# dlwns147/amq

Hardware: AMD Instinct MI355X
Metric: decode tokens/s, Llama-2-7B AMQ mixed 2/3/4-bit avg-3-bit, batch 1 (higher is better)
Workload: dtype f16; 1 GPU; Llama-2-7B shapes, synthesized avg-3.0-bit per-layer arch (bits_usage 2.982), batch 1 decode after a 64-token prefill, one stream per GPU; parallelism=replicas x1, prompt=64, group_size=128

## Files before the change

amq_amd/_lib.py:

```python
import ctypes
import os

_HERE = os.path.dirname(os.path.abspath(__file__))
LIB_PATH = os.path.join(_HERE, "libamq_hip.so")
AB_LIB_PATH = os.path.join(_HERE, "libamq_hip_ab.so")

AMQ_OK = 0
MODE_HQQ, MODE_FMA, MODE_FMA1 = 0, 1, 2
PRO_NONE, PRO_RMSNORM, PRO_SILU_MUL = 0, 1, 2
MAX_SEGMENTS = 4
MATH_DEFAULT, MATH_LINEAR, MATH_GROUPSCALE, MATH_EXACT = 0, 1, 2, 3
FEWROW_AUTO, FEWROW_TILE, FEWROW_STREAM = 0, 1, 2
ABI_VERSION = 521
GEMM_AUTO, GEMM_TILED, GEMM_SKINNY, GEMM_RING, GEMM_RING128, GEMM_WS, GEMM_DEQ = 0, 1, 2, 3, 4, 5, 6

_vp, _i, _f, _sz = ctypes.c_void_p, ctypes.c_int, ctypes.c_float, ctypes.c_size_t


class Segment(ctypes.Structure):
    _fields_ = [("qweight_native", _vp), ("meta_native", _vp), ("bias", _vp), ("residual", _vp),
                ("y", _vp), ("N", _i), ("bits", _i), ("mode", _i), ("y_stride", _i)]


class EngineLinear(ctypes.Structure):
    _fields_ = [("qweight_native", _vp), ("meta_native", _vp), ("N", _i), ("bits", _i), ("mode", _i), ("reserved", _i)]


class EngineBlock(ctypes.Structure):
    _fields_ = [("lin", EngineLinear * 7), ("ln1", _vp), ("ln2", _vp), ("kcache", _vp), ("vcache", _vp)]


class GemvOpts(ctypes.Structure):
    _fields_ = [("math", _i), ("waves", _i), ("depth", _i), ("rpt", _i), ("dot", _i)]


SIGNATURES = {
    "amq_version": (_i, []),
    "amq_default_gemv_math": (_i, []),
    "amq_last_error": (ctypes.c_char_p, []),
    "amq_query": (_i, [_i, ctypes.POINTER(_i), _i]),
    "amq_native_qweight_bytes": (_sz, [_i, _i, _i]),
    "amq_fma1_scale_bound": (ctypes.c_float, [_i]),
    "amq_native_meta_bytes": (_sz, [_i, _i, _i]),
    "amq_repack_from_hqq": (_i, [_i, _vp, _vp, _vp, _i, _i, _i, _vp, _vp, _vp]),
    "amq_repack_from_gptq": (_i, [_i, _vp, _vp, _vp, _i, _i, _i, _vp, _vp, _vp]),
    "amq_repack_from_awq": (_i, [_vp, _vp, _vp, _i, _i, _i, _vp, _vp, _vp]),
    "amq_dequantize_f16": (_i, [_i, _i, _vp, _vp, _i, _i, _i, _vp, _vp]),
    "amq_dequantize_hqq_f16": (_i, [_i, _vp, _vp, _vp, _i, _i, _i, _vp, _vp]),
    "amq_dequantize_bf16": (_i, [_i, _vp, _vp, _i, _i, _i, _vp, _vp]),
    "amq_dequantize_hqq_bf16": (_i, [_i, _vp, _vp, _vp, _i, _i, _i, _vp, _vp]),
    "amq_gemv_bf16": (_i, [_i, _vp, _vp, _vp, _vp, _vp, _vp, _i, _i, _i, _i, _i, _i, _vp]),
    "amq_gemm_bf16_workspace_bytes": (_sz, [_i, _i, _i]),
    "amq_gemm_bf16": (_i, [_i, _vp, _vp, _vp, _vp, _vp, _vp, _i, _i, _i, _i, _i, _i, _vp, _sz, _vp]),
    "amq_gemv_f16": (_i, [_i, _i, _vp, _vp, _vp, _vp, _vp, _i, _i, _i, _i, _i, _i, _vp]),
    "amq_gemm_f16": (_i, [_i, _i, _vp, _vp, _vp, _vp, _vp, _i, _i, _i, _i, _i, _i, _vp]),
    "amq_linear_f16": (_i, [_i, _i, _vp, _vp, _vp, _vp, _vp, _i, _i, _i, _i, _vp]),
    "amq_gemm_splitk_workspace_bytes": (_sz, [_i, _i, _i]),
    "amq_gemm_splitk_f16": (_i, [_i, _i, _vp, _vp, _vp, _vp, _vp, _i, _i, _i, _i, _i, _i, _vp, _sz, _vp]),
    "amq_compat_workspace_bytes": (_sz, [_i, _i, _i, _i]),
    "amq_vecquantmatmul_faster_old": (_i, [_i, _vp, _vp, _vp, _vp, _vp, _i, _i, _i, _i, _i, _vp, _sz, _i, _vp]),
    "amq_gemv_4bit": (_i, [_vp, _vp, _vp, _vp, _vp, _i, _i, _i, _i, _vp, _sz, _i, _vp]),
    "amq_gemm_4bit": (_i, [_vp, _vp, _vp, _vp, _vp, _i, _i, _i, _i, _vp, _sz, _i, _vp]),
    "amq_rmsnorm_f16": (_i, [_vp, _vp, _vp, _i, _i, _f, _vp]),
    "amq_gemv_f16w": (_i, [_vp, _vp, _vp, _vp, _vp, _f, _i, _i, _vp]),
    "amq_attn_decode_f16": (_i, [_vp, _vp, _vp, _vp, _vp, _vp, _vp, _i, _i, _i, _i, _i, _i, _f, _vp, _vp]),
    "amq_rope_table_f16": (_i, [_vp, _i, _f, _vp]),
    "amq_rope_table_freqs_f16": (_i, [_vp, _i, _vp, _f, _vp]),
    "amq_decode_tail_f16": (_i, [_vp, _i, _vp, _i, _vp, _vp, _vp, _vp, _vp, _i, _vp]),
    "amq_attn_decode_cur_f16": (_i, [_vp, _vp, _vp, _vp, _vp, _vp, _vp, _i, _i, _i, _i, _i, _vp]),
    "amq_gemm_res_f16": (_i, [_i, _i, _vp, _vp, _vp, _vp, _vp, _vp, _i, _i, _i, _i, _i, _i, _vp, _sz, _vp]),
    "amq_xfrag_bytes": (_sz, [_i, _i]),
    "amq_xfrag_f16": (_i, [_vp, _vp, _i, _i, ctypes.c_longlong, ctypes.c_longlong, _vp]),
    "amq_rmsnorm_xfrag_f16": (_i, [_vp, _vp, _vp, _i, _i, _f, _vp]),
    "amq_gemm_xfrag_f16": (_i, [_i, _i, _vp, _vp, _vp, _vp, _vp, _vp, _vp, _i, _i, _i, _i, _i, _vp]),
    "amq_gemm_gated_fused": (_i, [_i, _i, _i, _i, _i]),
    "amq_gemm_gated_fused_g": (_i, [_i, _i, _i, _i, _i, _i]),
    "amq_gemm_gated_f16": (_i, [_i, _i, _i, _vp, _vp, _vp, _vp, _vp, _vp, _i, _i, _i, _i, _i, _vp, _sz, _vp]),
    "amq_attn_decode_split_workspace_bytes": (_sz, [_i, _i, _i]),
    "amq_attn_decode_split_f16": (_i, [_vp, _vp, _vp, _vp, _vp, _vp, _vp, _vp, _i, _i, _i, _i, _i, _i, _f, _vp, _i, _vp, _sz, _vp, _vp]),
    "amq_gemm_xfrag_grouped_f16": (_i, [ctypes.POINTER(Segment), _i, _vp, _i, _i, _i, _vp]),
    "amq_gemm_xfrag_grouped_form_f16": (_i, [ctypes.POINTER(Segment), _i, _vp, _i, _i, _i, _i, _i, _vp]),
    "amq_attn_prefill_xfrag_f16": (_i, [_vp, _vp, _vp, _vp, _i, _i, _i, _i, _i] + [ctypes.c_longlong] * 5 + [_vp]),
    "amq_gemv_f16w_rows": (_i, [_vp, _vp, _vp, _vp, _vp, _f, _i, _i, _i, _vp]),
    "amq_decode_tail_batch_f16": (_i, [_vp, _i, _vp, _i, _vp, _vp, _vp, _vp, _vp, _i, _i, _vp]),
    "amq_decode_tail_suppress_f16": (_i, [_vp, _i, _vp, _i, _vp, _vp, _vp, _vp, _vp, _i, _i, _vp, _vp]),
    "amq_set_token_f16": (_i, [_vp, _i, _vp, _i, _i, _vp, _vp, _vp, _vp, _vp, _i, _i, _vp]),
    "amq_attn_prefill_f16": (_i, [_vp, _vp, _vp, _vp, _i, _i, _i, _i, _i, _i] + [ctypes.c_longlong] * 10 + [_vp]),
    "amq_rope_cache_f16": (_i, [_vp, _vp, _vp, _vp, _vp, _vp, _i, _i, _i, _i, _i, _i, _i, _vp]),
    "amq_rope_cache_batch_f16": (_i, [_vp, _vp, _vp, _vp, _vp, _vp, _i, _i, _i, _i, _i, _i, _i, _i, _vp]),
    "amq_rope_rows_f16": (_i, [_vp, _vp, _vp, _i, _i, _i, _i, _i, _i, _i, _vp]),
    "amq_silu_mul_f16": (_i, [_vp, _vp, _vp, _sz, _vp]),
    "amq_gemv_grouped_f16": (_i, [ctypes.POINTER(Segment), _i, _vp, _vp, _vp, _f, _i, _i, _i, _i, _i, ctypes.POINTER(GemvOpts), _vp]),
    "amq_gemv_grouped_sums_f16": (_i, [ctypes.POINTER(Segment), _i, _vp, _vp, _f, _vp, _vp, _i, _i, _i, _vp]),
    "amq_gemm_f16w_f16": (_i, [_vp, _vp, _vp, _vp, _vp, _vp, _i, _i, _i, _i, _i, _vp]),
    "amq_gemm_route_workspace_bytes": (_sz, [_i, _i, _i, _i]),
    "amq_gemm_route_workspace_bytes_g": (_sz, [_i, _i, _i, _i, _i]),
    "amq_gemm_res_norm_xfrag_f16": (_i, [_i, _i, _vp, _vp, _vp, _vp, _vp, _vp, _i, _i, _i, _i, _i, _vp, _sz, _vp, _f, _vp, _vp]),
    "amq_gemm_route_f16": (_i, [_i, _i, _i, _vp, _vp, _vp, _vp, _vp, _vp, _i, _i, _i, _i, _i, _i, _vp, _sz, _vp]),
}

AB_SIGNATURES = {
    "amq_gemv_qkv_attn_f16": (_i, [ctypes.POINTER(Segment), _vp, _vp, _f, _i, _i, _vp, _vp, _vp, _vp, _i, _i, _i, _i, _vp, _vp]),
    "amq_decode_engine_image_bytes": (_sz, [_i]),
    "amq_decode_engine_scratch_bytes": (_sz, [_i, _i, _i]),
    "amq_decode_engine_sync_bytes": (_sz, []),
    "amq_decode_engine_image": (_i, [ctypes.POINTER(EngineBlock), _i, _i, _i, _i, _i, _i, _i, _vp]),
    "amq_decode_engine_f16": (_i, [_vp, _i, _i, _i, _i, _i, _i, _i, _f, _vp, _vp, _sz, _vp, _vp, _sz, _i, _vp]),
}

_lib = None
_ab_lib = None


class AmqError(RuntimeError):
    pass


def load():
    global _lib
    if _lib is not None:
        return _lib
    if not os.path.exists(LIB_PATH):
        raise AmqError(
            f"{LIB_PATH} not found: the HIP extension is not built. "
            "Run `python -c 'import __graft_entry__ as g; g.build()'` (or `make -C amq_amd/csrc`). "
            "There is no CPU fallback.")
    import torch
    lib = ctypes.CDLL(LIB_PATH)
    for name, (res, args) in SIGNATURES.items():
        fn = getattr(lib, name)
        fn.restype, fn.argtypes = res, args
    if lib.amq_version() != ABI_VERSION:
        raise AmqError(f"{LIB_PATH} reports ABI version {lib.amq_version()}, these bindings were written against {ABI_VERSION} "
                       "(include/amq_hip.h AMQ_VERSION): rebuild with `make -C amq_amd/csrc`")
    _lib = lib
    return lib


def load_ab():
    global _ab_lib
    if _ab_lib is not None:
        return _ab_lib
    if not os.path.exists(AB_LIB_PATH):
        raise AmqError(f"{AB_LIB_PATH} not found: the A/B routes (decode engine, fused q/k/v + attention) live in their own library -- "
                       "`make -C amq_amd/csrc ab` (or __graft_entry__.build()).  They are slower than the product step and not needed for it.")
    import torch
    lib = ctypes.CDLL(AB_LIB_PATH)
    for name, (res, args) in AB_SIGNATURES.items():
        fn = getattr(lib, name)
        fn.restype, fn.argtypes = res, args
    lib.amq_last_error.restype = ctypes.c_char_p
    _ab_lib = lib
    return lib


def check_ab(rc):
    if rc != AMQ_OK:
        raise AmqError(f"libamq_hip_ab error {rc}: {load_ab().amq_last_error().decode('utf-8', 'replace')}")


def use_library(path):
    global LIB_PATH
    global AB_LIB_PATH
    if _lib is not None or _ab_lib is not None:
        raise AmqError("use_library() must be called before the library is first loaded")
    LIB_PATH = os.path.abspath(path)
    AB_LIB_PATH = LIB_PATH


SAFE_LIB_PATH = os.path.join(_HERE, "libamq_hip_safe.so")


def open_twin(path=None):
    path = SAFE_LIB_PATH if path is None else os.path.abspath(path)
    if not os.path.exists(path):
        raise AmqError(f"{path} not found: `make -C amq_amd/csrc safe` (or __graft_entry__.build())")
    import torch
    lib = ctypes.CDLL(path)
    for name, (res, args) in SIGNATURES.items():
        fn = getattr(lib, name)
        fn.restype, fn.argtypes = res, args
    if lib.amq_version() != ABI_VERSION:
        raise AmqError(f"{path} reports ABI version {lib.amq_version()}, expected {ABI_VERSION}")
    return lib


class routed_to:

    def __init__(self, lib):
        self.lib = lib

    def __enter__(self):
        global _lib
        load()
        self.prev, _lib = _lib, self.lib
        return self.lib

    def __exit__(self, *exc):
        global _lib
        _lib = self.prev
        return False


def check(rc):
    if rc != AMQ_OK:
        msg = load().amq_last_error().decode("utf-8", "replace")
        raise AmqError(f"libamq_hip error {rc}: {msg}")


def current_stream():
    import torch
    try:
        return ctypes.c_void_p(torch._C._cuda_getCurrentRawStream(torch.cuda.current_device()))
    except AttributeError:
        return ctypes.c_void_p(torch.cuda.current_stream().cuda_stream)


def stream_of(device):
    import torch
    idx = device if isinstance(device, int) else (device.index if device.index is not None else torch.cuda.current_device())
    try:
        return ctypes.c_void_p(torch._C._cuda_getCurrentRawStream(idx))
    except AttributeError:
        return ctypes.c_void_p(torch.cuda.current_stream(idx).cuda_stream)


def ptr(t):
    if t is None:
        return None
    return ctypes.c_void_p(t.data_ptr())
```

amq_amd/csrc/amq_capi.hip:

```cpp
#include "../../include/amq_hip.h"
#ifdef AMQ_AB_ROUTES
#include "../../include/amq_hip_ab.h"
#endif
#include "amq_common.cuh"
#include "amq_kernels.h"

#include <stdarg.h>
#include <stdio.h>
#include <vector>

namespace {

thread_local char g_err[512] = "";

int fail(int code, const char* fmt, ...) {
    va_list ap;
    va_start(ap, fmt);
    vsnprintf(g_err, sizeof(g_err), fmt, ap);
    va_end(ap);
    return code;
}

int check_hip(hipError_t e, const char* what) {
    if (e == hipSuccess) return AMQ_OK;
// ... 25 lines not shown

constexpr size_t LDS_LIMIT = 160 * 1024;

}

extern "C" {

int amq_version(void) { return AMQ_VERSION; }
const char* amq_last_error(void) { return g_err; }

int amq_query(int K, int* out, int cap) {
    int vals[6];
    int maxm = 0, maxm_plain = 0, maxm_plain_nonorm = 0;
    for (int m = 1; m <= amq::GEMV_MAX_M; ++m) {
        if (amq::gemv_min_lds_bytes(m, K, false) <= LDS_LIMIT) maxm = m;
        if (amq::gemv_min_lds_bytes(m, K, true, true) <= LDS_LIMIT) maxm_plain = m;
        if (amq::gemv_min_lds_bytes(m, K, true, false) <= LDS_LIMIT) maxm_plain_nonorm = m;
    }
    vals[0] = maxm;
    vals[1] = (int)LDS_LIMIT;
    vals[2] = amq::TILE_N;
    vals[3] = amq::TILE_K;
    vals[4] = maxm_plain;
    vals[5] = maxm_plain_nonorm;
    int n = cap < 6 ? cap : 6;
    for (int i = 0; i < n; ++i) out[i] = vals[i];
    return n;
}

size_t amq_native_qweight_bytes(int bits, int N, int K) { return amq::native_qweight_bytes(bits, N, K); }
float amq_fma1_scale_bound(int bits) { return (bits == 2 || bits == 3 || bits == 4) ? amq::fma1_scale_bound(bits) : 0.0f; }
size_t amq_native_meta_bytes(int N, int K, int group) { return amq::native_meta_bytes(N, K, group > 0 ? amq::meta_pairs(group) : 1); }

int amq_repack_from_hqq(int bits, const void* W_q, const void* scale, const void* zero, int N, int K, int group,
                        void* qn, void* mn, void* stream) {
    if (int rc = check_shape(bits, N, K, group)) return rc;
    if (!W_q || !scale || !zero || !qn || !mn) return fail(AMQ_EINVAL, "null pointer");
    return check_hip(amq::launch_repack(amq::FMT_HQQ, bits, W_q, scale, zero, N, K, qn, mn, (hipStream_t)stream, group), "repack_from_hqq");
}

int amq_repack_from_gptq(int bits, const void* qweight, const void* scales, const void* zeros, int N, int K, int group,
                         void* qn, void* mn, void* stream) {
    if (int rc = check_shape(bits, N, K, group)) return rc;
    if (!qweight || !scales || !zeros || !qn || !mn) return fail(AMQ_EINVAL, "null pointer");
    return check_hip(amq::launch_repack(amq::FMT_GPTQ, bits, qweight, scales, zeros, N, K, qn, mn, (hipStream_t)stream, group), "repack_from_gptq");
}

int amq_repack_from_awq(const void* qweight, const void* scales, const void* scaled_zeros, int N, int K, int group,
                        void* qn, void* mn, void* stream) {
    if (int rc = check_shape(4, N, K, group)) return rc;
    if (!qweight || !scales || !scaled_zeros || !qn || !mn) return fail(AMQ_EINVAL, "null pointer");
    return check_hip(amq::launch_repack(amq::FMT_AWQ, 4, qweight, scales, scaled_zeros, N, K, qn, mn, (hipStream_t)stream, group), "repack_from_awq");
}

int amq_dequantize_f16(int bits, int mode, const void* qn, const void* mn, int N, int K, int group, void* W, void* stream) {
    if (int rc = check_shape(bits, N, K, group)) return rc;
    if (int rc = check_mode(mode)) return rc;
    mode = kernel_mode(mode);
    if (!qn || !mn || !W) return fail(AMQ_EINVAL, "null pointer");
    return check_hip(amq::launch_dequantize(bits, mode, qn, mn, N, K, W, (hipStream_t)stream, amq::meta_pairs(group)), "dequantize");
}

int amq_dequantize_hqq_f16(int bits, const void* W_q, const void* scale, const void* zero, int N, int K, int group,
                           void* W, void* stream) {
    if (int rc = check_shape(bits, N, K, group)) return rc;
    if (!W_q || !scale || !zero || !W) return fail(AMQ_EINVAL, "null pointer");
    return check_hip(amq::launch_dequantize_hqq(bits, W_q, scale, zero, N, K, W, (hipStream_t)stream, group), "dequantize_hqq");
}

#ifndef AMQ_GEMV_DEFAULT_MATH
#define AMQ_GEMV_DEFAULT_MATH AMQ_MATH_EXACT
#endif
int amq_default_gemv_math(void) { return AMQ_GEMV_DEFAULT_MATH; }

int amq_gemv_grouped_f16(const amq_segment* segs, int nseg, const void* x, const void* x2, const void* gamma,
                         float eps, int prologue, int M, int K, int group, int x_stride, const amq_gemv_opts* opts,
                         void* stream) {
    if (!segs || nseg < 1 || nseg > AMQ_MAX_SEGMENTS) return fail(AMQ_EINVAL, "nseg must be 1..%d (got %d)", AMQ_MAX_SEGMENTS, nseg);
    if (!x) return fail(AMQ_EINVAL, "null x");
    if (prologue < AMQ_PRO_NONE || prologue > AMQ_PRO_SILU_MUL) return fail(AMQ_EINVAL, "unknown prologue %d", prologue);
    if (prologue == AMQ_PRO_RMSNORM && !gamma) return fail(AMQ_EINVAL, "RMSNorm prologue needs gamma");
    if (prologue == AMQ_PRO_SILU_MUL && !x2) return fail(AMQ_EINVAL, "SiLU*mul prologue needs x2");
    if (M < 1) return fail(AMQ_ESHAPE, "M must be >= 1 (got %d)", M);
    amq_gemv_opts o{};
    if (opts) o = *opts;
    if (o.math < AMQ_MATH_DEFAULT || o.math > AMQ_MATH_EXACT)
        return fail(AMQ_EINVAL, "opts.math must be AMQ_MATH_DEFAULT, AMQ_MATH_EXACT, AMQ_MATH_GROUPSCALE or AMQ_MATH_LINEAR");
    if (o.math == AMQ_MATH_DEFAULT) o.math = amq_default_gemv_math();
    if (o.waves != 0 && o.waves != 4 && o.waves != 8 && o.waves != 16) return fail(AMQ_EINVAL, "opts.waves must be 0, 4, 8 or 16");
    if (o.depth != 0 && o.depth != 2 && o.depth != 4) return fail(AMQ_EINVAL, "opts.depth must be 0, 2 or 4");
    if (o.rpt < 0 || o.rpt > 64) return fail(AMQ_EINVAL, "opts.rpt (row-tiles per workgroup) must be 0..64");
    const bool plain_form = !o.dot && o.math != AMQ_MATH_LINEAR && o.depth != 4 && amq::meta_pairs(group) == 1 && o.waves != 4;
    const bool whole_rows = prologue == AMQ_PRO_RMSNORM || (x_stride != 0 && x_stride != K);
    if (M > amq::GEMV_MAX_M || amq::gemv_min_lds_bytes(M, K, plain_form && o.waves == 0 && o.rpt == 0, whole_rows) > LDS_LIMIT)
        return fail(AMQ_ESHAPE, "M=%d rows of K=%d%s do not fit LDS for the GEMV path; use amq_gemm_f16", M, K, (x_stride != 0 && x_stride != K) ? " (strided x)" : "");
    amq::GemvArgs a{};
    for (int i = 0; i < nseg; ++i) {
        const amq_segment& s = segs[i];
        if (int rc = check_shape(s.bits, s.N, K, group)) return rc;
        if (int rc = check_mode(s.mode)) return rc;
        if (!s.qweight_native || !s.meta_native || !s.y) return fail(AMQ_EINVAL, "segment %d: null pointer", i);
        amq::GemvSeg& d = a.seg[i];
        d.qweight = s.qweight_native; d.meta = s.meta_native; d.bias = s.bias; d.residual = s.residual; d.y = s.y;
        d.N = s.N; d.bits = s.bits; d.mode = s.mode;
        d.y_stride = s.y_stride ? s.y_stride : s.N;
    }
    a.nseg = nseg; a.M = M; a.K = K; a.x_stride = x_stride ? x_stride : K;
    a.x = x; a.x2 = x2; a.gamma = gamma; a.eps = eps; a.prologue = prologue;
    a.flags = (o.dot ? amq::GEMV_FLAG_DOT : 0) | (o.math == AMQ_MATH_LINEAR ? amq::GEMV_FLAG_LINEAR : 0) |
              (o.math == AMQ_MATH_GROUPSCALE ? amq::GEMV_FLAG_GS : 0);
    a.force_waves = o.waves;
    a.force_depth = o.depth;
    a.force_rpt = o.rpt;
    a.gp = amq::meta_pairs(group);
    if (a.gp > 1 && (o.dot || o.math == AMQ_MATH_LINEAR || o.depth == 4))
        return fail(AMQ_EINVAL, "groups of %d: the GEMV kernel's default form only (opts.math = AMQ_MATH_EXACT, opts.dot = 0, opts.depth = 0 / 2)", group);
    return check_hip(amq::launch_gemv(a, (hipStream_t)stream), "gemv");
}

int amq_gemv_grouped_sums_f16(const amq_segment* segs, int nseg, const void* x, const void* gamma, float eps, const float* sums_in,
                              float* sums_out, int M, int K, int group, void* stream) {
    if (!segs || nseg < 1 || nseg > AMQ_MAX_SEGMENTS) return fail(AMQ_EINVAL, "nseg must be 1..%d (got %d)", AMQ_MAX_SEGMENTS, nseg);
    if (!x) return fail(AMQ_EINVAL, "null x");
    if ((sums_in != nullptr) != (gamma != nullptr)) return fail(AMQ_EINVAL, "sums_in (the partial sums of squares of x) and gamma go together");
    if (M < 2 || M > 8) return fail(AMQ_ESHAPE, "the partial-sum forms live in the 2 .. 8-row kernels (got M=%d); one row: amq_gemv_grouped_f16 with AMQ_PRO_RMSNORM", M);
    if (amq::meta_pairs(group) != 1) return fail(AMQ_ESHAPE, "groups of 128 (and multiples) only (got %d)", group);
    if (K < 2048) return fail(AMQ_ESHAPE, "K >= 2048 (the 2 .. 8-row kernels run 8 or 16 waves per workgroup; got K=%d)", K);
    if (sums_out && nseg != 1) return fail(AMQ_EINVAL, "sums_out describes ONE output: nseg must be 1");
    if (sums_out && sums_in) return fail(AMQ_EINVAL, "sums_out is written by launches without a prologue (o_proj, down_proj): not together with sums_in");
    if (sums_in && K > 8192) return fail(AMQ_ESHAPE, "sums_in: K <= 8192 (K / 16 <= 512 partials per row; got K=%d)", K);
    const bool phased = amq::gemv_rows_phased(M, K, true, sums_in != nullptr);
    if (sums_in && phased) return fail(AMQ_ESHAPE, "M=%d rows of K=%d are staged in two K phases: no fused norm there", M, K);
    if (amq::gemv_min_lds_bytes(M, K, true, sums_in != nullptr) > LDS_LIMIT)
        return fail(AMQ_ESHAPE, "M=%d rows of K=%d do not fit LDS for the GEMV path", M, K);
    amq::GemvArgs a{};
    for (int i = 0; i < nseg; ++i) {
        const amq_segment& s = segs[i];
        if (int rc = check_shape(s.bits, s.N, K, group)) return rc;
        if (int rc = check_mode(s.mode)) return rc;
        if (!s.qweight_native || !s.meta_native || !s.y) return fail(AMQ_EINVAL, "segment %d: null pointer", i);
        amq::GemvSeg& d = a.seg[i];
        d.qweight = s.qweight_native; d.meta = s.meta_native; d.bias = s.bias; d.residual = s.residual; d.y = s.y;
        d.N = s.N; d.bits = s.bits; d.mode = s.mode;
        d.y_stride = s.y_stride ? s.y_stride : s.N;
    }
    a.nseg = nseg; a.M = M; a.K = K; a.x_stride = K;
    a.x = x; a.x2 = nullptr; a.gamma = gamma; a.eps = eps;
    a.prologue = sums_in ? amq::PRO_RMSNORM_SUMS : amq::PRO_NONE;
    a.sums_in = sums_in; a.sums_out = sums_out;
    a.gp = 1;
    return check_hip(amq::launch_gemv(a, (hipStream_t)stream), "gemv_sums");
}

int amq_gemv_f16(int bits, int mode, const void* x, const void* qn, const void* mn, const void* bias, void* y,
                 int M, int N, int K, int group, int x_stride, int y_stride, void* stream) {
    amq_segment s{};
    s.qweight_native = qn; s.meta_native = mn; s.bias = bias; s.residual = nullptr; s.y = y;
    s.N = N; s.bits = bits; s.mode = mode; s.y_stride = y_stride;
    return amq_gemv_grouped_f16(&s, 1, x, nullptr, nullptr, 0.f, AMQ_PRO_NONE, M, K, group, x_stride, nullptr, stream);
}

int amq_gemm_f16(int bits, int mode, const void* x, const void* qn, const void* mn, const void* bias, void* y,
                 int M, int N, int K, int group, int x_stride, int y_stride, void* stream) {
    if (int rc = check_shape(bits, N, K, group)) return rc;
    if (int rc = check_mode(mode)) return rc;
    mode = kernel_mode(mode);
    if (!x || !qn || !mn || !y) return fail(AMQ_EINVAL, "null pointer");
    if (M < 1) return fail(AMQ_ESHAPE, "M must be >= 1 (got %d)", M);
    amq::GemmArgs a{x, qn, mn, bias, y, M, N, K, bits, mode, x_stride ? x_stride : K, y_stride ? y_stride : N, nullptr, 1,
                    nullptr, nullptr, nullptr, amq::meta_pairs(group)};
    return check_hip(amq::launch_gemm(a, (hipStream_t)stream), "gemm");
}

size_t amq_gemm_splitk_workspace_bytes(int M, int N, int K) {
    if (M < 1 || N < 1 || K < 128) return 0;
    const int s = amq::gemm_pick_splits(M, N, K);
    return s > 1 ? (size_t)s * (size_t)M * (size_t)N * sizeof(float) : 0;
}

int amq_gemm_splitk_f16(int bits, int mode, const void* x, const void* qn, const void* mn, const void* bias, void* y,
                        int M, int N, int K, int group, int x_stride, int y_stride, void* workspace, size_t workspace_bytes,
                        void* stream) {
    const size_t need = amq_gemm_splitk_workspace_bytes(M, N, K);
    if (need == 0) return amq_gemm_f16(bits, mode, x, qn, mn, bias, y, M, N, K, group, x_stride, y_stride, stream);
    if (int rc = check_shape(bits, N, K, group)) return rc;
    if (int rc = check_mode(mode)) return rc;
    mode = kernel_mode(mode);
    if (!x || !qn || !mn || !y) return fail(AMQ_EINVAL, "null pointer");
    if (!workspace || workspace_bytes < need) return fail(AMQ_EINVAL, "split-K workspace too small: need %zu bytes, got %zu", need, workspace_bytes);
    amq::GemmArgs a{x, qn, mn, bias, y, M, N, K, bits, mode, x_stride ? x_stride : K, y_stride ? y_stride : N,
                    (float*)workspace, amq::gemm_pick_splits(M, N, K), nullptr, nullptr, nullptr, amq::meta_pairs(group)};
    return check_hip(amq::launch_gemm(a, (hipStream_t)stream), "gemm_splitk");
}

static bool route_is_deq(int route, int M, int N, int K, int group = 128) {
    if (group == 64 || group == 32)
        return route == AMQ_GEMM_DEQ || (route == AMQ_GEMM_AUTO && amq::gemm_fine_takes_deq(M, N, K));
    return route == AMQ_GEMM_DEQ || (route == AMQ_GEMM_AUTO && amq::gemm_takes_deq(M, N, K));
}

size_t amq_gemm_route_workspace_bytes_g(int route, int M, int N, int K, int group) {
    if (M < 1 || N < 1 || K < 128 || route < AMQ_GEMM_AUTO || route > AMQ_GEMM_DEQ) return 0;
    if (route_is_deq(route, M, N, K, group)) return (size_t)N * (size_t)K * 2;
    if ((group == 64 || group == 32) && amq::gemm_fine_takes_skinny(M)) return 0;
    const int s = amq::gemm_pick_splits(M, N, K, (group == 64 || group == 32) && route == AMQ_GEMM_AUTO ? (int)AMQ_GEMM_TILED : route);
    return s > 1 ? (size_t)s * (size_t)M * (size_t)N * sizeof(float) : 0;
}
size_t amq_gemm_route_workspace_bytes(int route, int M, int N, int K) { return amq_gemm_route_workspace_bytes_g(route, M, N, K, 128); }

static int check_fine_route(int route, int group, int M, int N, int K, const void* workspace) {
    if (group != 64 && group != 32) return AMQ_OK;
    if (route == AMQ_GEMM_RING || route == AMQ_GEMM_RING128 || route == AMQ_GEMM_WS)
        return fail(AMQ_EINVAL, "groups of %d: the ring / wave-specialised kernels read one (scale, zero) per 128 columns (use AMQ_GEMM_AUTO, _SKINNY, _TILED or the dequantize-once route _DEQ)", group);
    if (route == AMQ_GEMM_DEQ && !workspace) return fail(AMQ_EINVAL, "AMQ_GEMM_DEQ needs a workspace of N * K * 2 bytes for the fp16 weights");
    (void)M; (void)N; (void)K;
    return AMQ_OK;
}

static int gemm_route_impl(int route, int bits, int mode, const void* x, const void* qn, const void* mn, const void* bias,
                           const void* residual, void* y, int M, int N, int K, int group, int x_stride, int y_stride,
                           void* workspace, size_t workspace_bytes, void* stream, amq::GemmNorm* norm) {
    if (route < AMQ_GEMM_AUTO || route > AMQ_GEMM_DEQ) return fail(AMQ_EINVAL, "unknown GEMM route %d", route);
    if (int rc = check_shape(bits, N, K, group)) return rc;
    if (int rc = check_mode(mode)) return rc;
    mode = kernel_mode(mode);
    if (!x || !qn || !mn || !y) return fail(AMQ_EINVAL, "null pointer");
    if (M < 1) return fail(AMQ_ESHAPE, "M must be >= 1 (got %d)", M);
    if (route == AMQ_GEMM_SKINNY && M > 64 && !((group == 64 || group == 32) && amq::gemm_fine_takes_skinny(M)))
        return fail(AMQ_ESHAPE, "the few-row kernel takes at most 64 rows (got %d)", M);
    if (int rc = check_fine_route(route, group, M, N, K, workspace)) return rc;
    const bool fine = group == 64 || group == 32;
    const size_t need = amq_gemm_route_workspace_bytes_g(route, M, N, K, group);
    const bool deq = route_is_deq(route, M, N, K, group);
    if (route == AMQ_GEMM_DEQ && !workspace) return fail(AMQ_EINVAL, "AMQ_GEMM_DEQ needs a workspace of N * K * 2 bytes for the fp16 weights");
    const bool use_ws = need != 0 && workspace != nullptr;
    if (use_ws && workspace_bytes < need)
        return fail(AMQ_EINVAL, "workspace too small: need %zu bytes, got %zu", need, workspace_bytes);
    const bool split = use_ws && !deq;
    const int sroute = fine && route == AMQ_GEMM_AUTO ? (int)AMQ_GEMM_TILED : route;
    amq::GemmArgs a{x, qn, mn, bias, y, M, N, K, bits, mode, x_stride ? x_stride : K, y_stride ? y_stride : N,
                    split ? (float*)workspace : nullptr, split ? amq::gemm_pick_splits(M, N, K, sroute) : 1, residual, nullptr,
                    use_ws && deq ? workspace : nullptr, amq::meta_pairs(group)};
    if ((route == AMQ_GEMM_DEQ || (fine && deq)) && !amq::gemm_f16w_ok(M, N, K, a.x_stride, a.y_stride))
        return fail(AMQ_ESHAPE, "AMQ_GEMM_DEQ: strides must be multiples of 8 (x) / 4 (y) halves and x, W must each span < 4 GiB");
    return check_hip(amq::launch_gemm(a, (hipStream_t)stream, route, norm), "gemm");
}

int amq_gemm_route_f16(int route, int bits, int mode, const void* x, const void* qn, const void* mn, const void* bias,
                       const void* residual, void* y, int M, int N, int K, int group, int x_stride, int y_stride,
                       void* workspace, size_t workspace_bytes, void* stream) {
    return gemm_route_impl(route, bits, mode, x, qn, mn, bias, residual, y, M, N, K, group, x_stride, y_stride, workspace, workspace_bytes, stream, nullptr);
}

int amq_gemm_res_norm_xfrag_f16(int bits, int mode, const void* x, const void* qn, const void* mn, const void* bias, const void* residual,
                                void* y, int M, int N, int K, int group, int x_stride, void* workspace, size_t workspace_bytes,
                                const void* gamma, float eps, void* xf, void* stream) {
    if (!gamma || !xf) return fail(AMQ_EINVAL, "null pointer");
    if (N < 128 || (N % 128) != 0) return fail(AMQ_ESHAPE, "the normed rows are handed on in fragment order: N %% 128 == 0 (got N=%d)", N);
    amq::GemmNorm norm{gamma, eps, xf, false};
    return gemm_route_impl(AMQ_GEMM_AUTO, bits, mode, x, qn, mn, bias, residual, y, M, N, K, group, x_stride, 0, workspace, workspace_bytes, stream, &norm);
}

int amq_gemm_gated_fused_g(int route, int M, int N, int K, int use_workspace, int group) {
    if (M < 1 || N < 16 || K < 128 || route < AMQ_GEMM_AUTO || route > AMQ_GEMM_DEQ) return 0;
    const bool fine = group == 64 || group == 32;
    const bool deq = route_is_deq(route, M, N, K, group);
    const int sroute = fine && route == AMQ_GEMM_AUTO ? (int)AMQ_GEMM_TILED : route;
    amq::GemmArgs a{nullptr, nullptr, nullptr, nullptr, nullptr, M, N, K, 4, AMQ_MODE_HQQ, K, N, nullptr,
                    use_workspace && !deq ? amq::gemm_pick_splits(M, N, K, sroute) : 1, nullptr, nullptr,
                    use_workspace && deq ? (void*)&a : nullptr,
                    amq::meta_pairs(group > 0 ? group : 128)};
    return amq::gemm_gate_fused(a, route) ? 1 : 0;
}
int amq_gemm_gated_fused(int route, int M, int N, int K, int use_workspace) { return amq_gemm_gated_fused_g(route, M, N, K, use_workspace, 128); }

int amq_gemm_gated_f16(int route, int bits, int mode, const void* x, const void* qn, const void* mn, const void* bias,
                       const void* gate, void* y, int M, int N, int K, int group, int x_stride, void* workspace,
                       size_t workspace_bytes, void* stream) {
    if (route < AMQ_GEMM_AUTO || route > AMQ_GEMM_DEQ) return fail(AMQ_EINVAL, "unknown GEMM route %d", route);
    if (int rc = check_shape(bits, N, K, group)) return rc;
    if (int rc = check_mode(mode)) return rc;
    mode = kernel_mode(mode);
    if (!x || !qn || !mn || !y || !gate) return fail(AMQ_EINVAL, "null pointer");
    if (M < 1) return fail(AMQ_ESHAPE, "M must be >= 1 (got %d)", M);
    if (N % 8) return fail(AMQ_ESHAPE, "the gated product needs N %% 8 == 0 (got %d)", N);
    if (route == AMQ_GEMM_SKINNY && M > 64 && !((group == 64 || group == 32) && amq::gemm_fine_takes_skinny(M)))
        return fail(AMQ_ESHAPE, "the few-row kernel takes at most 64 rows (got %d)", M);
    if (int rc = check_fine_route(route, group, M, N, K, workspace)) return rc;
    const size_t need = amq_gemm_route_workspace_bytes_g(route, M, N, K, group);
    const bool deq = route_is_deq(route, M, N, K, group);
    if (route == AMQ_GEMM_DEQ && !workspace) return fail(AMQ_EINVAL, "AMQ_GEMM_DEQ needs a workspace of N * K * 2 bytes for the fp16 weights");
    const bool use_ws = need != 0 && workspace != nullptr;
    if (use_ws && workspace_bytes < need)
        return fail(AMQ_EINVAL, "workspace too small: need %zu bytes, got %zu", need, workspace_bytes);
    const bool split = use_ws && !deq;
    const int sroute = (group == 64 || group == 32) && route == AMQ_GEMM_AUTO ? (int)AMQ_GEMM_TILED : route;
    amq::GemmArgs a{x, qn, mn, bias, y, M, N, K, bits, mode, x_stride ? x_stride : K, N,
                    split ? (float*)workspace : nullptr, split ? amq::gemm_pick_splits(M, N, K, sroute) : 1, nullptr, gate,
                    use_ws && deq ? workspace : nullptr, amq::meta_pairs(group)};
    if ((group == 64 || group == 32) && deq && !amq::gemm_f16w_ok(M, N, K, a.x_stride, a.y_stride))
        return fail(AMQ_ESHAPE, "groups of %d (dequantize-once route): x_stride must be a multiple of 8 halves, N of 4, x and W must each span < 4 GiB", group);
    if (gate == y && !amq::gemm_gate_fused(a, route))
        return fail(AMQ_EINVAL, "gate may alias y only where the kernel applies it in its epilogue (amq_gemm_gated_fused)");
    return check_hip(amq::launch_gemm(a, (hipStream_t)stream, route), "gemm_gated");
}

// ... 502 lines not shown
```

amq_amd/csrc/amq_gemv.hip:

```cpp
#include "amq_gemv_body.cuh"

namespace amq {


#ifdef AMQ_STAMP
unsigned long long* g_stamp_ptr = nullptr;
extern "C" int amq_debug_set_stamps(void* p) { g_stamp_ptr = (unsigned long long*)p; return 0; }
#endif

size_t gemv_lds_bytes(int M, int K, int nw) {
    const size_t xbytes = (((size_t)M * (K + XPAD) * 2) + 15) & ~(size_t)15;
    const size_t xg = (size_t)(K >> 7) * 64;
    const size_t red = (size_t)2 * (nw > 1 ? nw : 16) * 16 * 16 * 4;
    return xbytes + xg + red;
}

size_t gemv_lds_bytes_rows(int M, int K, int nw) {
    const size_t xbytes = (((size_t)M * (K + XPAD) * 2) + 15) & ~(size_t)15;
    return xbytes + (size_t)2 * nw * (M <= 4 ? 64 : 128) * 4;
}
bool gemv_rows_phased(int M, int K, bool plain, bool norm) {
    const int G = K >> 7;
    return plain && !norm && M > 4 && M <= 8 && (G & 1) == 0 && G / 2 >= 2 * 16 && (K / 2 >> 3) <= 1024 &&
           gemv_lds_bytes_rows(M, K, 16) > 160 * 1024 && gemv_lds_bytes_rows(M, K / 2, 16) <= 160 * 1024;
}
size_t gemv_min_lds_bytes(int M, int K, bool plain, bool norm) {
    if (gemv_rows_phased(M, K, plain, norm)) return gemv_lds_bytes_rows(M, K / 2, 16);
    if (plain && M > 1 && M <= 8) return gemv_lds_bytes_rows(M, K, 16);
    return gemv_lds_bytes(M, K, 1);
}

int gemv_pick_waves(int total_rt, int K) {
    const int G = K >> 7;
    if (G < 16) return 4;
    if (G > 32) return 16;
    return 8;
}

#define AMQ_GEMV_EXTERN(PRO_)                                                                                                  \
    extern template hipError_t launch_pro<PRO_>(const GemvKArgs&, int, int, int, int, size_t, hipStream_t);                     \
    extern template hipError_t launch_pro_g<PRO_, 2>(const GemvKArgs&, int, int, size_t, hipStream_t);                          \
    extern template hipError_t launch_pro_g<PRO_, 4>(const GemvKArgs&, int, int, size_t, hipStream_t);
AMQ_GEMV_EXTERN(PRO_NONE)
AMQ_GEMV_EXTERN(PRO_RMSNORM)
AMQ_GEMV_EXTERN(PRO_SILU_MUL)
#undef AMQ_GEMV_EXTERN
hipError_t launch_pro_sums_entry(const GemvKArgs&, int nw, int rs, int, size_t, hipStream_t);

#ifndef AMQ_RS128_THREE
#define AMQ_RS128_THREE 1
#endif
hipError_t launch_gemv(GemvArgs& a, hipStream_t st) {
    StreamDevice sd_(st);
    int total_rt = 0;
    for (int i = 0; i < a.nseg; ++i) { a.seg[i].n_rt = a.seg[i].N / 16; total_rt += a.seg[i].n_rt; }
    int nw = a.force_waves ? a.force_waves : gemv_pick_waves(total_rt, a.K);
    const int gp = a.gp > 1 ? a.gp : 1;
    if (gp != 1 && gp != 2 && gp != 4) return hipErrorInvalidValue;
    if (gp > 1 && ((a.flags & (GEMV_FLAG_DOT | GEMV_FLAG_LINEAR)) || a.force_depth == 4)) return hipErrorInvalidValue;
    bool rs128 = false, rs64 = false;
    const bool plain = !(a.flags & (GEMV_FLAG_DOT | GEMV_FLAG_LINEAR)) && a.force_depth != 4 && gp == 1;
    const bool ph2 = !a.force_waves && a.force_rpt <= 0 && gemv_rows_phased(a.M, a.K, plain, a.prologue == PRO_RMSNORM || a.x_stride != a.K);
    if (ph2) {
        rs128 = true;
        nw = 16;
    } else if (a.M > 1 && a.M <= 8 && plain && nw != 4) {
        rs128 = a.M > 4;
        rs64 = !rs128;
        if (!a.force_waves && nw == 8 && 2 * gemv_lds_bytes_rows(a.M, a.K, 8) > 160 * 1024) nw = 16;
    } else if (!a.force_waves && a.M > 1 && nw == 8 && 3 * gemv_lds_bytes(a.M, a.K, 8) > 160 * 1024) {
        nw = 16;
    }
    const bool mid_k = gp == 1 && !a.force_waves && nw == 16 && a.M == 1 && (a.K >> 3) > 512 && (a.K >> 3) <= 1024 &&
                       !(a.flags & (GEMV_FLAG_DOT | GEMV_FLAG_LINEAR)) && a.force_depth != 4;
    if (mid_k) nw = 8;
    int rpt = ph2 ? 1 : a.force_rpt;
    const bool two_per_cu = nw == 8 && ((rs128 && (a.prologue == PRO_RMSNORM || a.prologue == PRO_RMSNORM_SUMS || !AMQ_RS128_THREE)) || ((rs64 || rs128) && 3 * gemv_lds_bytes_rows(a.M, a.K, 8) > 160 * 1024));
    const int target = (mid_k || two_per_cu) ? 512 : nw == 16 ? 256 : 256 * 24 / nw;
    if (rpt <= 0) {
        rpt = (total_rt + target - 1) / target;
        if (rpt < 1) rpt = 1;
    }
#ifndef AMQ_DEAL_SCOPE
#define AMQ_DEAL_SCOPE 1
#endif
    const bool deal = a.force_rpt <= 0 && !ph2 && total_rt > target &&
                      ((rs128 && nw == 8) || (AMQ_DEAL_SCOPE >= 1 && mid_k) || AMQ_DEAL_SCOPE >= 2);
    int wg = 0, mask = 0;
    for (int i = 0; i < a.nseg; ++i) {
        a.seg[i].wg_begin = wg;
        a.seg[i].wg_count = (a.seg[i].n_rt + rpt - 1) / rpt;
        if (deal) {
            const int share = (int)((long long)target * a.seg[i].n_rt / total_rt);
            a.seg[i].wg_count = share < 1 ? 1 : share > a.seg[i].n_rt ? a.seg[i].n_rt : share;
        }
        if (a.seg[i].n_rt / a.seg[i].wg_count > GEMV_SPLIT_BASE_MASK || a.seg[i].wg_count >= (1 << 19)) return hipErrorInvalidValue;
        wg += a.seg[i].wg_count;
        mask |= 1 << a.seg[i].bits;
    }
    const bool lin = (a.flags & GEMV_FLAG_LINEAR) && !((a.flags & GEMV_FLAG_DOT) && a.M == 1);
    (void)lin; (void)mask;
    const size_t lds = ph2 ? gemv_lds_bytes_rows(a.M, a.K / 2, 16) : (rs128 || rs64) ? gemv_lds_bytes_rows(a.M, a.K, nw) : gemv_lds_bytes(a.M, a.K, a.M > 1 ? nw : 16);
    if ((a.prologue == PRO_RMSNORM_SUMS || a.sums_out) && !(rs128 || rs64)) return hipErrorInvalidValue;
    if (a.prologue == PRO_RMSNORM_SUMS && (ph2 || !a.sums_in || (a.K >> 4) > 64 * SUMS_PER_LANE || a.x_stride != a.K)) return hipErrorInvalidValue;
    if (a.sums_out && (a.nseg != 1 || a.prologue != PRO_NONE)) return hipErrorInvalidValue;
    GemvKArgs k{};
    k.x = a.x; k.x2 = a.prologue == PRO_RMSNORM_SUMS ? a.sums_in : a.x2; k.gamma = a.gamma;
    k.sums_out = (float*)a.sums_out; k.sums_stride = a.seg[0].n_rt;
    k.M = a.M; k.K = a.K; k.x_stride = a.x_stride; k.nseg = a.nseg;
    k.eps = a.eps; k.rpt = rpt;
    for (int i = 0; i < a.nseg; ++i) {
        const GemvSeg& s = a.seg[i];
        const bool has_fma1 = gp == 1 && !(a.flags & (GEMV_FLAG_DOT | GEMV_FLAG_LINEAR));
        k.wg_begin[i] = s.wg_begin; k.n_rt[i] = gemv_split(s.n_rt, s.wg_count); k.key[i] = s.bits * 4 + (s.mode == MODE_FMA1 && !has_fma1 ? (int)MODE_FMA : s.mode);
        k.qweight[i] = s.qweight; k.meta[i] = s.meta;
        k.bias[i] = s.bias; k.residual[i] = s.residual; k.y[i] = s.y; k.y_stride[i] = s.y_stride;
    }
#ifdef AMQ_STAMP
    k.stamps = g_stamp_ptr;
#endif
    if (gp == 2) {
        switch (a.prologue) {
            case PRO_NONE: return launch_pro_g<PRO_NONE, 2>(k, nw, wg, lds, st);
            case PRO_RMSNORM: return launch_pro_g<PRO_RMSNORM, 2>(k, nw, wg, lds, st);
            default: return launch_pro_g<PRO_SILU_MUL, 2>(k, nw, wg, lds, st);
        }
    }
    if (gp == 4) {
        switch (a.prologue) {
            case PRO_NONE: return launch_pro_g<PRO_NONE, 4>(k, nw, wg, lds, st);
            case PRO_RMSNORM: return launch_pro_g<PRO_RMSNORM, 4>(k, nw, wg, lds, st);
            default: return launch_pro_g<PRO_SILU_MUL, 4>(k, nw, wg, lds, st);
        }
    }
    if (a.prologue == PRO_RMSNORM_SUMS) return launch_pro_sums_entry(k, nw, rs64 ? 64 : 128, wg, lds, st);
    switch (a.prologue) {
        case PRO_NONE: return launch_pro<PRO_NONE>(k, a.flags | (rs128 ? GEMV_FLAG_RS128 : 0) | (rs64 ? GEMV_FLAG_RS64 : 0) | (ph2 ? GEMV_FLAG_PH2 : 0), a.force_depth, nw, wg, lds, st);
        case PRO_RMSNORM: return launch_pro<PRO_RMSNORM>(k, a.flags | (rs128 ? GEMV_FLAG_RS128 : 0) | (rs64 ? GEMV_FLAG_RS64 : 0) | (ph2 ? GEMV_FLAG_PH2 : 0), a.force_depth, nw, wg, lds, st);
        default: return launch_pro<PRO_SILU_MUL>(k, a.flags | (rs128 ? GEMV_FLAG_RS128 : 0) | (rs64 ? GEMV_FLAG_RS64 : 0) | (ph2 ? GEMV_FLAG_PH2 : 0), a.force_depth, nw, wg, lds, st);
    }
}

}
```

amq_amd/csrc/amq_gemv_body.cuh:

```cuda
#pragma once
#include "amq_common.cuh"
#include "amq_kernels.h"

namespace amq {

constexpr int XPAD = 8;

struct GemvKArgs {
    const void* x; const void* x2; const void* gamma;
    int M, K, x_stride, nseg;
    float eps; int rpt, pad0_, pad1_;
    int wg_begin[GEMV_MAX_SEG];
    int n_rt[GEMV_MAX_SEG];
    int key[GEMV_MAX_SEG];
    const void* qweight[GEMV_MAX_SEG];
    const void* meta[GEMV_MAX_SEG];
    const void* bias[GEMV_MAX_SEG];
    const void* residual[GEMV_MAX_SEG];
    void* y[GEMV_MAX_SEG];
    int y_stride[GEMV_MAX_SEG];
    float* sums_out;
    int sums_stride;
#ifdef AMQ_STAMP
    unsigned long long* stamps;
#endif
};

struct SegOut { const _Float16* bias; const _Float16* residual; _Float16* y; int y_stride; float* sums; int sums_stride; };

__device__ __forceinline__ float row16_total(float v) {
    v += __builtin_bit_cast(float, __builtin_amdgcn_update_dpp(0, __builtin_bit_cast(int, v), 0xB1, 0xF, 0xF, false));
    v += __builtin_bit_cast(float, __builtin_amdgcn_update_dpp(0, __builtin_bit_cast(int, v), 0x4E, 0xF, 0xF, false));
    v += __builtin_bit_cast(float, __builtin_amdgcn_update_dpp(0, __builtin_bit_cast(int, v), 0x141, 0xF, 0xF, false));
    v += __builtin_bit_cast(float, __builtin_amdgcn_update_dpp(0, __builtin_bit_cast(int, v), 0x140, 0xF, 0xF, false));
    return v;
}

struct GemvHot {
    const void* x; const void* x2; const void* gamma;
    int M, K, x_stride, rpt;
    float eps;
};

#ifdef AMQ_STAMP
#define AMQ_STAMP_AT(a_, slot_)                                                                  \
    do {                                                                                         \
        if ((a_).stamps && (threadIdx.x & 63) == 0)                                              \
            (a_).stamps[(size_t)blockIdx.x * 128 + (slot_)] = __builtin_amdgcn_s_memrealtime();   \
    } while (0)
#else
#define AMQ_STAMP_AT(a_, slot_) do { } while (0)
#endif
enum { MATH_EXACT = 0, MATH_DOT = 1, MATH_LINEAR = 2, MATH_GS = 3 };
#ifndef AMQ_SD_E9
#define AMQ_SD_E9 0
#endif

__device__ __forceinline__ float wave_sum(float v) {
    v += __builtin_bit_cast(float, __builtin_amdgcn_update_dpp(0, __builtin_bit_cast(int, v), 0xB1, 0xF, 0xF, false));
    v += __builtin_bit_cast(float, __builtin_amdgcn_update_dpp(0, __builtin_bit_cast(int, v), 0x4E, 0xF, 0xF, false));
    v += __builtin_bit_cast(float, __builtin_amdgcn_update_dpp(0, __builtin_bit_cast(int, v), 0x141, 0xF, 0xF, false));
    v += __builtin_bit_cast(float, __builtin_amdgcn_update_dpp(0, __builtin_bit_cast(int, v), 0x140, 0xF, 0xF, false));
    return (__builtin_bit_cast(float, __builtin_amdgcn_readlane(__builtin_bit_cast(int, v), 0)) +
            __builtin_bit_cast(float, __builtin_amdgcn_readlane(__builtin_bit_cast(int, v), 16))) +
           (__builtin_bit_cast(float, __builtin_amdgcn_readlane(__builtin_bit_cast(int, v), 32)) +
            __builtin_bit_cast(float, __builtin_amdgcn_readlane(__builtin_bit_cast(int, v), 48)));
}

__device__ __forceinline__ float silu_f(float g) { return g / (1.0f + __expf(-g)); }

struct MeanDiv {
    float inv; bool pow2; float k;
    __device__ __forceinline__ explicit MeanDiv(int K)
        : inv(__builtin_bit_cast(float, (127 - __builtin_ctz((unsigned)K)) << 23)), pow2((K & (K - 1)) == 0), k((float)K) {}
    __device__ __forceinline__ float operator()(float tot) const { return pow2 ? tot * inv : tot / k; }
};

template <int PRO, int NW, bool LIN>
__device__ __forceinline__ void stage_x(const GemvHot& a, _Float16* xl, float* xg, float* red, int xs) {
    constexpr int THREADS = NW * 64;
    const int tid = threadIdx.x;
    const int K = a.K;
    const int chunks = K >> 3;
    if (!LIN) {
        const int lane = tid & 63, wave = tid >> 6;
        int wpr = 1;
        while (wpr * 2 * a.M <= NW) wpr *= 2;
        const int rows_per_round = NW / wpr, sub = wave % wpr, stride = wpr * 64;
        for (int m0 = 0; m0 < a.M; m0 += rows_per_round) {
            const int m = m0 + wave / wpr;
            const bool on = m < a.M;
            const _Float16* xrow = (const _Float16*)a.x + (size_t)(on ? m : 0) * a.x_stride;
            _Float16* lrow = xl + (size_t)(on ? m : 0) * xs;
            float rstd = 1.0f;
            if (PRO == PRO_RMSNORM) {
                float ss = 0.f;
                if (on)
                    for (int c = sub * 64 + lane; c < chunks; c += stride) {
                        h8 v = *(const h8*)(xrow + 8 * c);
#pragma unroll
                        for (int i = 0; i < 8; ++i) { float f = (float)v[i]; ss += f * f; }
                    }
                ss = wave_sum(ss);
                if (m0) __syncthreads();
                if (lane == 0) red[wave] = ss;
                __syncthreads();
                float tot = 0.f;
                for (int i = 0; i < wpr; ++i) tot += red[wave - sub + i];
                rstd = rsqrtf(MeanDiv(K)(tot) + a.eps);
            }
            if (on)
                for (int c = sub * 64 + lane; c < chunks; c += stride) {
                    h8 v = *(const h8*)(xrow + 8 * c);
                    h8 r;
                    if (PRO == PRO_NONE) {
                        r = v;
                    } else if (PRO == PRO_SILU_MUL) {
                        const h8 u = *(const h8*)((const _Float16*)a.x2 + (size_t)m * a.x_stride + 8 * c);
#pragma unroll
                        for (int i = 0; i < 8; ++i) { _Float16 s = (_Float16)silu_f((float)v[i]); r[i] = s * u[i]; }
                    } else {
                        const h8 gm = *(const h8*)((const _Float16*)a.gamma + 8 * c);
#pragma unroll
                        for (int i = 0; i < 8; ++i) { _Float16 nrm = (_Float16)((float)v[i] * rstd); r[i] = gm[i] * nrm; }
                    }
                    *(h8*)(lrow + 8 * c) = r;
                }
        }
        return;
    }
    if (LIN)
        for (int i = tid; i < (K >> 7) * 16; i += THREADS) xg[i] = 0.f;
    if (LIN) __syncthreads();
    for (int m = 0; m < a.M; ++m) {
        const _Float16* xrow = (const _Float16*)a.x + (size_t)m * a.x_stride;
        _Float16* lrow = xl + (size_t)m * xs;
        float rstd = 1.0f;
        if (PRO == PRO_RMSNORM) {
            float ss = 0.f;
            for (int c = tid; c < chunks; c += THREADS) {
                h8 v = *(const h8*)(xrow + 8 * c);
#pragma unroll
                for (int i = 0; i < 8; ++i) { float f = (float)v[i]; ss += f * f; }
            }
            ss = wave_sum(ss);
            __syncthreads();
            if ((tid & 63) == 0) red[tid >> 6] = ss;
            __syncthreads();
            float tot = 0.f;
#pragma unroll
            for (int w = 0; w < NW; ++w) tot += red[w];
            rstd = rsqrtf(MeanDiv(K)(tot) + a.eps);
        }
        for (int c = tid; c < chunks; c += THREADS) {
            h8 v = *(const h8*)(xrow + 8 * c);
            h8 r;
            if (PRO == PRO_NONE) {
                r = v;
            } else if (PRO == PRO_SILU_MUL) {
                const h8 u = *(const h8*)((const _Float16*)a.x2 + (size_t)m * a.x_stride + 8 * c);
#pragma unroll
                for (int i = 0; i < 8; ++i) { _Float16 s = (_Float16)silu_f((float)v[i]); r[i] = s * u[i]; }
            } else {
                const h8 gm = *(const h8*)((const _Float16*)a.gamma + 8 * c);
#pragma unroll
                for (int i = 0; i < 8; ++i) { _Float16 nrm = (_Float16)((float)v[i] * rstd); r[i] = gm[i] * nrm; }
            }
            *(h8*)(lrow + 8 * c) = r;
            if (LIN) {
                float cs = 0.f;
#pragma unroll
                for (int i = 0; i < 8; ++i) cs += (float)r[i];
                cs += __shfl_xor(cs, 1); cs += __shfl_xor(cs, 2); cs += __shfl_xor(cs, 4); cs += __shfl_xor(cs, 8);
                if ((tid & 15) == 0) xg[(size_t)(c >> 4) * 16 + m] = cs;
            }
        }
    }
}

constexpr int XC_MAX = 4;
constexpr int SUMS_PER_LANE = 8;
struct XRegs { union { h8 v[XC_MAX]; float f[4 * XC_MAX]; }; h8 w[XC_MAX]; };
template <int NW> struct XCfg { static constexpr int XC = NW == 16 ? 2 : 1; };

template <int PRO, int NW, int XCH>
__device__ __forceinline__ void x_issue(const GemvHot& a, XRegs& xr) {
    constexpr int THREADS = NW * 64;
    const int last = (a.K >> 3) - 1;
#pragma unroll
    for (int i = 0; i < XCH; ++i) {
        int c = (int)threadIdx.x + i * THREADS;
        c = c < last ? c : last;
        xr.v[i] = *(const h8*)((const _Float16*)a.x + 8 * c);
        if (PRO == PRO_SILU_MUL) xr.w[i] = *(const h8*)((const _Float16*)a.x2 + 8 * c);
        if (PRO == PRO_RMSNORM) xr.w[i] = *(const h8*)((const _Float16*)a.gamma + 8 * c);
    }
}

template <int PRO, int NW, int XCH, bool LIN>
__device__ __forceinline__ void x_finish(const GemvHot& a, const XRegs& xr, _Float16* xl, float* xg, float* red) {
    constexpr int THREADS = NW * 64;
    const int tid = threadIdx.x;
    const int chunks = a.K >> 3;
    float rstd = 1.0f;
    if (PRO == PRO_RMSNORM) {
        float ss = 0.f;
#pragma unroll
        for (int i = 0; i < XCH; ++i) {
            if (tid + i * THREADS < chunks) {
#pragma unroll
                for (int e = 0; e < 8; ++e) { float f = (float)xr.v[i][e]; ss += f * f; }
            }
        }
        ss = wave_sum(ss);
        if ((tid & 63) == 0) red[tid >> 6] = ss;
        __syncthreads();
        float tot = 0.f;
#pragma unroll
        for (int w = 0; w < NW; ++w) tot += red[w];
        rstd = rsqrtf(MeanDiv(a.K)(tot) + a.eps);
    }
#pragma unroll
    for (int i = 0; i < XCH; ++i) {
        const int c = tid + i * THREADS;
        float cs = 0.f;
        if (c < chunks) {
            h8 r;
            if (PRO == PRO_NONE) {
                r = xr.v[i];
            } else if (PRO == PRO_SILU_MUL) {
#pragma unroll
                for (int e = 0; e < 8; ++e) { _Float16 sg = (_Float16)silu_f((float)xr.v[i][e]); r[e] = sg * xr.w[i][e]; }
            } else {
#pragma unroll
                for (int e = 0; e < 8; ++e) { _Float16 nrm = (_Float16)((float)xr.v[i][e] * rstd); r[e] = xr.w[i][e] * nrm; }
            }
            *(h8*)(xl + 8 * c) = r;
            if (LIN) {
#pragma unroll
                for (int e = 0; e < 8; ++e) cs += (float)r[e];
            }
        }
        if (LIN) {
            cs += __builtin_bit_cast(float, __builtin_amdgcn_update_dpp(0, __builtin_bit_cast(int, cs), 0xB1, 0xF, 0xF, false));
            cs += __builtin_bit_cast(float, __builtin_amdgcn_update_dpp(0, __builtin_bit_cast(int, cs), 0x4E, 0xF, 0xF, false));
            cs += __builtin_bit_cast(float, __builtin_amdgcn_update_dpp(0, __builtin_bit_cast(int, cs), 0x141, 0xF, 0xF, false));
            cs += __builtin_bit_cast(float, __builtin_amdgcn_update_dpp(0, __builtin_bit_cast(int, cs), 0x140, 0xF, 0xF, false));
            if ((tid & 15) == 0 && c < chunks) xg[(size_t)(c >> 4) * 16] = cs;
        }
    }
}

template <int RS> struct RowsCfg { static constexpr int MRMAX = RS == 64 ? 4 : RS == 128 ? 8 : 1; };

__device__ __forceinline__ void gv_glds16(const void* sbase, unsigned voff, unsigned lds_dst) {
    asm volatile("s_mov_b32 m0, %2\n\ts_nop 0\n\tglobal_load_lds_dwordx4 %0, %1" AMQ_MARK("gemv.xdma") :: "v"(voff), "s"(sbase), "s"(lds_dst) : "memory", "m0");
}

template <int PRO, int NW, int XCH>
__device__ __forceinline__ void x_dma_rows(const GemvHot& a, _Float16* xl, int xs, XRegs& xr, int k0, int Ks) {
    constexpr int THREADS = NW * 64;
    const int chunks = Ks >> 3;
    const int wave = __builtin_amdgcn_readfirstlane((int)threadIdx.x >> 6);
    const unsigned lds0 = (unsigned)(size_t)(__attribute__((address_space(3))) _Float16*)xl;
    for (int m = 0; m < a.M; ++m) {
        const _Float16* row = (const _Float16*)a.x + (size_t)m * a.x_stride + k0;
#pragma unroll
        for (int i = 0; i < XCH; ++i) {
            const int c = (int)threadIdx.x + i * THREADS;
            if (c < chunks) gv_glds16(row, 16u * (unsigned)c, lds0 + (unsigned)(m * xs) * 2u + (unsigned)(i * THREADS + wave * 64) * 16u);
        }
    }
    if (PRO == PRO_RMSNORM || PRO == PRO_RMSNORM_SUMS) {
        const int last = chunks - 1;
#pragma unroll
        for (int i = 0; i < XCH; ++i) {
            int c = (int)threadIdx.x + i * THREADS;
            c = c < last ? c : last;
            xr.w[i] = *(const h8*)((const _Float16*)a.gamma + 8 * c);
        }
    }
    if (PRO == PRO_RMSNORM_SUMS) {
        const int P = a.K >> 4;
        const float* ss = (const float*)a.x2 + (size_t)(wave < a.M ? wave : a.M - 1) * P;
        const int lane = (int)threadIdx.x & 63;
#pragma unroll
        for (int j = 0; j < SUMS_PER_LANE; ++j) {
            const int idx = lane + 64 * j;
            xr.f[j] = ss[idx < P ? idx : P - 1];
        }
    }
}

template <int PRO, int NW, int XCH, int NRING, int MR>
__device__ __forceinline__ void x_finish_dma(const GemvHot& a, const XRegs& xr, _Float16* xl, float* red, int xs, int k0, int Ks) {
    constexpr int THREADS = NW * 64;
    static_assert(NRING >= 0 && NRING <= 63, "counted wait (vmcnt is six bits on gfx9)");
    const int tid = threadIdx.x;
    const int chunks = Ks >> 3;
    AMQ_WAIT_VM("gemv.xrows", NRING, "from=gemv.xdma:>=%0");
    if (PRO == PRO_NONE) return;
    if (PRO == PRO_RMSNORM) {
        h8 v[MR * XCH];
        float ss[MR];
#pragma unroll
        for (int m = 0; m < MR; ++m) {
            ss[m] = 0.f;
            if (m < a.M) {
#pragma unroll
                for (int i = 0; i < XCH; ++i) {
                    const int c = tid + i * THREADS;
                    if (c < chunks) v[m * XCH + i] = *(const h8*)(xl + (size_t)m * xs + 8 * c);
                }
            }
        }
#pragma unroll
        for (int m = 0; m < MR; ++m) {
            if (m < a.M) {
#pragma unroll
                for (int i = 0; i < XCH; ++i) {
                    if (tid + i * THREADS < chunks) {
#pragma unroll
                        for (int e = 0; e < 8; ++e) { float f = (float)v[m * XCH + i][e]; ss[m] += f * f; }
                    }
                }
            }
        }
#pragma unroll
        for (int m = 0; m < MR; ++m) {
            if (m < a.M) {
                ss[m] = wave_sum(ss[m]);
                if ((tid & 63) == 0) red[m * NW + (tid >> 6)] = ss[m];
            }
        }
        __syncthreads();
        const MeanDiv mean(a.K);
#pragma unroll
        for (int m = 0; m < MR; ++m) {
            if (m < a.M) {
                float tot = 0.f;
#pragma unroll
                for (int w = 0; w < NW; ++w) tot += red[m * NW + w];
                const float rstd = rsqrtf(mean(tot) + a.eps);
#pragma unroll
                for (int i = 0; i < XCH; ++i) {
                    const int c = tid + i * THREADS;
                    if (c < chunks) {
                        h8 r;
#pragma unroll
                        for (int e = 0; e < 8; ++e) { _Float16 nrm = (_Float16)((float)v[m * XCH + i][e] * rstd); r[e] = xr.w[i][e] * nrm; }
                        *(h8*)(xl + (size_t)m * xs + 8 * c) = r;
                    }
                }
            }
        }
        return;
    }
    if (PRO == PRO_RMSNORM_SUMS) {
        const int P = a.K >> 4, lane = tid & 63, wave = tid >> 6;
        float s = 0.f;
#pragma unroll
        for (int j = 0; j < SUMS_PER_LANE; ++j) s += (lane + 64 * j < P) ? xr.f[j] : 0.f;
        s = wave_sum(s);
        if (lane == 0) red[wave] = rsqrtf(MeanDiv(a.K)(s) + a.eps);
        __syncthreads();
#pragma unroll
        for (int m = 0; m < MR; ++m) {
            if (m < a.M) {
                const float rstd = red[m];
#pragma unroll
                for (int i = 0; i < XCH; ++i) {
                    const int c = tid + i * THREADS;
                    if (c < chunks) {
                        _Float16* p = xl + (size_t)m * xs + 8 * c;
                        const h8 v = *(const h8*)p;
                        h8 r;
#pragma unroll
// ... 14 lines not shown
#pragma unroll
            for (int i = 0; i < XCH; ++i) {
                int c = tid + i * THREADS;
                c = c < last ? c : last;
                up[j * XCH + i] = *(const h8*)((const _Float16*)a.x2 + (size_t)mm * a.x_stride + k0 + 8 * c);
            }
        }
#pragma unroll
        for (int j = 0; j < 4; ++j) {
            if (m0 + j < a.M) {
#pragma unroll
                for (int i = 0; i < XCH; ++i) {
                    const int c = tid + i * THREADS;
                    if (c < chunks) {
                        _Float16* p = xl + (size_t)(m0 + j) * xs + 8 * c;
                        const h8 g = *(const h8*)p;
                        h8 r;
#pragma unroll
                        for (int e = 0; e < 8; ++e) { _Float16 sg = (_Float16)silu_f((float)g[e]); r[e] = sg * up[j * XCH + i][e]; }
                        *(h8*)p = r;
                    }
                }
            }
        }
    }
}

__device__ __forceinline__ void store_out(const SegOut& s, int m, int n, float acc) {
    _Float16 y = (_Float16)acc;
    if (s.bias) y = y + s.bias[n];
    if (s.residual) y = s.residual[(size_t)m * s.y_stride + n] + y;
    s.y[(size_t)m * s.y_stride + n] = y;
}

template <int BITS> struct LinCfg;
template <> struct LinCfg<4> { static constexpr int SH = 6; };
template <> struct LinCfg<3> { static constexpr int SH = 7; };
template <> struct LinCfg<2> { static constexpr int SH = 8; };

template <int BITS>
__device__ __forceinline__ void unpack_lane_sub(const uint32_t* w, h2* out) {
    constexpr int SH = LinCfg<BITS>::SH;
    constexpr uint32_t fm = (1u << BITS) - 1u;
    constexpr uint32_t msk = (fm << SH) | ((fm << SH) << 16);
    if (BITS == 4) {
#pragma unroll
        for (int t = 0; t < 4; ++t) {
            const uint32_t u = w[t];
            out[4 * t + 0] = as_h2((u << 6) & msk);
            out[4 * t + 1] = as_h2((u << 2) & msk);
            out[4 * t + 2] = as_h2((u >> 2) & msk);
            out[4 * t + 3] = as_h2((u >> 6) & msk);
        }
    } else if (BITS == 2) {
#pragma unroll
        for (int d = 0; d < 2; ++d) {
            const uint32_t u = w[d];
            out[8 * d + 0] = as_h2((u << 8) & msk);
            out[8 * d + 1] = as_h2((u << 6) & msk);
            out[8 * d + 2] = as_h2((u << 4) & msk);
            out[8 * d + 3] = as_h2((u << 2) & msk);
            out[8 * d + 4] = as_h2(u & msk);
            out[8 * d + 5] = as_h2((u >> 2) & msk);
            out[8 * d + 6] = as_h2((u >> 4) & msk);
            out[8 * d + 7] = as_h2((u >> 6) & msk);
        }
    } else {
#pragma unroll
        for (int d = 0; d < 3; ++d) {
            const uint32_t u = w[d];
            out[5 * d + 0] = as_h2((u << 7) & msk);
            out[5 * d + 1] = as_h2((u << 4) & msk);
            out[5 * d + 2] = as_h2((u << 1) & msk);
            out[5 * d + 3] = as_h2((u >> 2) & msk);
            out[5 * d + 4] = as_h2((u >> 5) & msk);
        }
        out[15] = as_h2(((w[0] >> 8) & 0x00800080u) | ((w[1] >> 7) & 0x01000100u) | ((w[2] >> 6) & 0x02000200u));
    }
}

template <int BITS, int MODE, int PRO, int NW, int U, int MATH, int XCH, int RS = 256, bool SC1 = false, int GP = 1, int PH = 1>
__device__ __forceinline__ void gemv_body(const GemvHot& a, const GemvKArgs& blk, int sidx, const void* qweight, const void* meta_base,
                                          int seg_split, int local, _Float16* lds_x, const _Float16* xl, float* xg,
                                          float* red, int xs, int xmode, const XRegs& xr) {
    const int lane = threadIdx.x & 63;
    const int wave = __builtin_amdgcn_readfirstlane(threadIdx.x >> 6);
    const int G = a.K >> 7;
    const int r = lane & 15, o = lane >> 4;
    static_assert(PH == 1 || (RS != 256 && PRO != PRO_RMSNORM && PRO != PRO_RMSNORM_SUMS && MATH != MATH_LINEAR && MATH != MATH_DOT), "K phases: the row kernels, no full-row statistic");
    static_assert(PRO != PRO_RMSNORM_SUMS || (RS != 256 && MATH == MATH_EXACT && GP == 1), "partial-sum RMSNorm: the 2 .. 8-row kernels");
    const int Gp = G / PH;
    const int nt = (Gp - wave + NW - 1) / NW;
    const int sp_base = seg_split & GEMV_SPLIT_BASE_MASK, sp_rem = seg_split >> GEMV_SPLIT_BASE_BITS;
    const int rt0 = local * sp_base + (local < sp_rem ? local : sp_rem);
    const int n_my = sp_base + (local < sp_rem ? 1 : 0);
    const int total = n_my * PH * nt;
    const uint32_t* qw = (const uint32_t*)qweight;
    static_assert(GP == 1 || MATH == MATH_EXACT || MATH == MATH_GS, "groups finer than 128: exact math only");
    constexpr bool GS = MATH == MATH_GS && MODE == MODE_HQQ && GP == 1;
    const h2* mt = (const h2*)meta_base + r * GP;

#ifdef AMQ_ABL_NOMETA
#define AMQ_META_LOAD(slot, tile_) meta[slot] = as_h2(0x40003c00u + (uint32_t)(tile_ & 1))
#else
#define AMQ_META_LOAD(slot, tile_)                                                               \
    do {                                                                                         \
        if constexpr (GP == 1) meta[slot] = as_h2(AMQ_STREAM_LOAD((const uint32_t*)(mt + (tile_) * 16)));   \
        else metag[slot] = load_meta_g<GP>(mt + (tile_) * (16 * GP));                            \
    } while (0)
#endif
#ifdef AMQ_ABL_NOXLDS
#define AMQ_XREAD(p) ((h8){(_Float16)1, (_Float16)2, (_Float16)-1, (_Float16)0.5f, (_Float16)1, (_Float16)-2, (_Float16)1, (_Float16)3} + (h8)(_Float16)(float)(kbase & 1))
#else
#define AMQ_XREAD(p) (*(const h8*)(p))
#endif
    LanePayload<BITS> pay[U];
    h2 meta[U];
    [[maybe_unused]] MetaG<GP> metag[U];
    int ii = 0, ij = 0;
#ifdef AMQ_ABL_NOLOAD
#define AMQ_ISSUE(slot)                                                                          \
    do {                                                                                         \
        _Pragma("unroll") for (int d_ = 0; d_ < BITS; ++d_) asm volatile("" : "+v"(pay[slot].w[d_]));   \
        asm volatile("" : "+v"(meta[slot]));                                                     \
        if (++ii == nt) { ii = 0; ++ij; }                                                        \
    } while (0)
#else
#define AMQ_ISSUE_AT(slot, clamp_)                                                               \
    do {                                                                                         \
        size_t tile_ = (size_t)(rt0 + ij / PH) * G + (ij % PH) * Gp + (wave + ii * NW);           \
        if (clamp_) tile_ = tile_ < last_tile ? tile_ : last_tile;                               \
        pay[slot] = load_payload<BITS>(qw + tile_ * (64 * BITS), lane);                           \
        AMQ_META_LOAD(slot, tile_);                                                              \
        if (++ii == nt) { ii = 0; ++ij; }                                                        \
    } while (0)
#define AMQ_ISSUE(slot) AMQ_ISSUE_AT(slot, false)
#endif

    const size_t last_tile = (size_t)(rt0 + n_my) * G - 1;
#ifdef AMQ_ABL_NOLOAD
#pragma unroll
    for (int u = 0; u < U; ++u) AMQ_ISSUE(u);
#else
#pragma unroll
    for (int u = 0; u < U; ++u) AMQ_ISSUE_AT(u, true);
#endif
    if (wave == 0) AMQ_STAMP_AT(blk, 1);

    SegOut so;
    so.bias = (const _Float16*)blk.bias[sidx];
    so.residual = (const _Float16*)blk.residual[sidx];
    so.y = (_Float16*)blk.y[sidx];
    so.y_stride = blk.y_stride[sidx];
    so.sums = (RS != 256 && PRO == PRO_NONE) ? blk.sums_out : nullptr;
    so.sums_stride = blk.sums_stride;
#ifndef AMQ_ABL_NOSTAGE
    if (xmode == 1) x_finish<PRO, NW, XCH, MATH == MATH_LINEAR>(a, xr, lds_x, xg, red);
    else if (RS != 256 && xmode == 2) {
#ifdef AMQ_ABL_NOLOAD
        x_finish_dma<PRO, NW, XCH, 0, RowsCfg<RS>::MRMAX>(a, xr, lds_x, red, xs, 0, a.K / PH);
#else
        if constexpr (U * 2 <= 63) x_finish_dma<PRO, NW, XCH, U * 2, RowsCfg<RS>::MRMAX>(a, xr, lds_x, red, xs, 0, a.K / PH);
#endif
    }
    else stage_x<PRO, NW, MATH == MATH_LINEAR>(a, lds_x, xg, red, xs);
#endif
    __syncthreads();
    if (wave == 0) AMQ_STAMP_AT(blk, 2);

    _Float16 pf_bias = (_Float16)0.f, pf_res = (_Float16)0.f;
    const int e_m = (int)threadIdx.x >> 4, e_c = (int)threadIdx.x & 15;
    const bool e_on = (int)threadIdx.x < a.M * 16;
#define AMQ_EPI_PREFETCH(rt_)                                                                    \
    do {                                                                                         \
        if (e_on) {                                                                              \
            if (so.bias) pf_bias = so.bias[(rt_) * 16 + e_c];                                    \
            if (so.residual) pf_res = so.residual[(size_t)e_m * so.y_stride + (rt_) * 16 + e_c]; \
        }                                                                                        \
    } while (0)
    AMQ_EPI_PREFETCH(rt0);

    float acc1[4] = {0.f, 0.f, 0.f, 0.f};
    f4 accm = (f4){0.f, 0.f, 0.f, 0.f};
    const int mrow = r < a.M ? r : a.M - 1;
    const _Float16* xrow = xl + (size_t)mrow * xs + 8 * o;
    int ci = 0, cj = 0, par = 0;

    int plevel_ = 3;
#define AMQ_SETPRIO_LEVEL()                                                                      \
    do {                                                                                         \
        if (plevel_ == 3) __builtin_amdgcn_s_setprio(3);                                         \
        else if (plevel_ == 2) __builtin_amdgcn_s_setprio(2);                                    \
        else if (plevel_ == 1) __builtin_amdgcn_s_setprio(1);                                    \
        else __builtin_amdgcn_s_setprio(0);                                                      \
    } while (0)
#define AMQ_FINISH()                                                                             \
    do {                                                                                         \
        float* rp_ = red + par * (NW * RS);                                                      \
        if (MATH == MATH_DOT) {                                                                  \
            float v_ = (acc1[0] + acc1[1]) + (acc1[2] + acc1[3]);                                \
            v_ += __shfl_xor(v_, 16);                                                            \
            v_ += __shfl_xor(v_, 32);                                                            \
            if (lane < 16) rp_[wave * RS + lane] = v_;                                           \
            acc1[0] = acc1[1] = acc1[2] = acc1[3] = 0.f;                                         \
        } else {                                                                                 \
            _Pragma("unroll") for (int i_ = 0; i_ < 4; ++i_)                                     \
                if (4 * o + i_ < a.M) rp_[wave * RS + (4 * o + i_) * 16 + r] = accm[i_];         \
            accm = (f4){0.f, 0.f, 0.f, 0.f};                                                     \
        }                                                                                        \
        __syncthreads();                                                                         \
        const int rt_ = rt0 + cj / PH;                                                           \
        if (e_on) {                                                \
            float tot_ = 0.f;                                                                    \
            _Pragma("unroll") for (int w_ = 0; w_ < NW; ++w_) tot_ += rp_[w_ * RS + threadIdx.x];  \
            _Float16 y_ = (_Float16)tot_;                                      \
            if (so.bias) y_ = y_ + pf_bias;                      \
            if (so.residual) y_ = pf_res + y_;                               \
            if (SC1) __hip_atomic_store((unsigned short*)(so.y + (size_t)e_m * so.y_stride + rt_ * 16 + e_c),          \
                                        __builtin_bit_cast(unsigned short, y_), __ATOMIC_RELAXED, __HIP_MEMORY_SCOPE_AGENT); \
            else so.y[(size_t)e_m * so.y_stride + rt_ * 16 + e_c] = y_;                          \
            if constexpr (RS != 256 && PRO == PRO_NONE) {      \
                if (so.sums) {                                                                   \
                    const float q_ = row16_total((float)y_ * (float)y_);                         \
                    if (e_c == 0) so.sums[(size_t)e_m * so.sums_stride + rt_] = q_;              \
                }                                                                                \
            }                                                                                    \
        }                                                                                        \
        if (cj / PH + 1 < n_my) AMQ_EPI_PREFETCH(rt_ + 1);                                       \
        par ^= 1;                                                                                \
    } while (0)

#ifdef AMQ_ABL_NOCOMPUTE
#define AMQ_COMPUTE(slot)                                                                        \
    do {                                                                                         \
        uint32_t x_ = 0;                                                                         \
        _Pragma("unroll") for (int d_ = 0; d_ < BITS; ++d_) x_ ^= pay[slot].w[d_];               \
        accm[0] += (float)(x_ & 1u) + (float)meta[slot].x;                                       \
    } while (0)
#else
#define AMQ_COMPUTE(slot)                                                                        \
    do {                                                                                         \
        const int g_ = wave + ci * NW;                                                           \
        const int kbase = g_ << 7;                                                               \
        h2 wv[16];                                                                               \
        if (MATH == MATH_LINEAR) unpack_lane_sub<BITS>(pay[slot].w, wv);                         \
        else if constexpr (GS) dequant_lane_gs<BITS>(pay[slot].w, gs_zero(meta[slot]), wv);       \
        else if constexpr (GP == 1 && MODE == MODE_FMA1) dequant_lane_fma1<BITS>(pay[slot].w, meta[slot], wv);    \
        else if constexpr (GP == 1 && MODE == MODE_HQQ && AMQ_SD_E9) {                            \
            dequant_lane_gs<BITS>(pay[slot].w, gs_zero(meta[slot]), wv);                         \
            const h2 sc9_ = bcast(meta[slot].x) * bcast((_Float16)512.0f);                       \
            _Pragma("unroll") for (int p_ = 0; p_ < 16; ++p_) wv[p_] = wv[p_] * sc9_;            \
        }                                                                                        \
        else if constexpr (GP == 1) dequant_lane_sd<BITS, MODE>(pay[slot].w, meta[slot], wv);    \
        else dequant_lane_sd_g<BITS, MODE, GP>(pay[slot].w, metag[slot], wv);                    \
        if (MATH == MATH_DOT) {                                                                  \
            _Pragma("unroll") for (int t = 0; t < 4; ++t) {                                      \
                const h8 xv = *(const h8*)(xl + kbase + 8 * o + 32 * t);                         \
                _Pragma("unroll") for (int p = 0; p < 4; ++p) {                                  \
                    h2 xp = {xv[2 * p], xv[2 * p + 1]};                                          \
                    acc1[t] = __builtin_amdgcn_fdot2(wv[4 * t + p], xp, acc1[t], false);         \
                }                                                                                \
            }                                                                                    \
        } else {                                                                                 \
            f4 c_ = (MATH == MATH_LINEAR || GS) ? (f4){0.f, 0.f, 0.f, 0.f} : accm;               \
            _Pragma("unroll") for (int t = 0; t < 4; ++t) {                                      \
                h8 b;                                                                            \
                _Pragma("unroll") for (int p = 0; p < 4; ++p) {                                  \
                    b[2 * p] = wv[4 * t + p].x; b[2 * p + 1] = wv[4 * t + p].y;                  \
                }                                                                                \
                const h8 av = AMQ_XREAD(xrow + kbase + 32 * t);                                  \
                c_ = __builtin_amdgcn_mfma_f32_16x16x32_f16(av, b, c_, 0, 0, 0);                 \
            }                                                                                    \
            if (MATH == MATH_LINEAR) {                                                           \
                 \
                 \
                const float sf = (float)meta[slot].x, zf = (float)meta[slot].y;                  \
                const float s24 = sf * (float)(1 << (24 - LinCfg<BITS>::SH));                    \
                const float zx = (MODE == MODE_HQQ) ? -(sf * zf) : zf;                           \
                const f4 xs4 = *(const f4*)(xg + g_ * 16 + 4 * o);                               \
                _Pragma("unroll") for (int i_ = 0; i_ < 4; ++i_)                                 \
                    accm[i_] = __builtin_fmaf(s24, c_[i_], __builtin_fmaf(zx, xs4[i_], accm[i_])); \
            } else if constexpr (GS) {                                                           \
                 \
                const float sg_ = gs_scale(meta[slot]);                                          \
                _Pragma("unroll") for (int i_ = 0; i_ < 4; ++i_) accm[i_] = __builtin_fmaf(sg_, c_[i_], accm[i_]); \
            } else {                                                                             \
                accm = c_;                                                                       \
            }                                                                                    \
        }                                                                                        \
    } while (0)
#endif
#ifdef AMQ_ABL_NOFINISH
#define AMQ_ROWEND() do { if (++ci == nt) { ci = 0; ++cj; } } while (0)
#else
#define AMQ_ROWEND()                                                                             \
    do {                                                                                         \
        if (++ci == nt) {                                                                        \
            if (PH == 1 || cj % PH == PH - 1) AMQ_FINISH();                                      \
            if constexpr (PH > 1) { if (cj + 1 < n_my * PH) AMQ_RESTAGE((cj + 1) % PH); }        \
            ci = 0; ++cj;                                                                        \
        }                                                                                        \
    } while (0)
#endif
#define AMQ_RESTAGE_NRING 0
#define AMQ_RESTAGE(ph_)                                                                         \
    do {                                                                                         \
        __syncthreads();                                       \
        x_dma_rows<PRO, NW, XCH>(a, lds_x, xs, const_cast<XRegs&>(xr), (ph_) * (a.K / PH), a.K / PH);          \
        x_finish_dma<PRO, NW, XCH, AMQ_RESTAGE_NRING, RowsCfg<RS>::MRMAX>(a, xr, lds_x, red, xs, (ph_) * (a.K / PH), a.K / PH); \
        __syncthreads();                                                                         \
    } while (0)

    if (nt == 0) {
        for (int j = 0; j < n_my; ++j) { AMQ_FINISH(); cj += PH; }
        return;
    }

    int idx = 0;
#ifdef AMQ_STAMP
    unsigned long long c_wait = 0, c_math = 0, c_row = 0;
    constexpr int OPS_PER_TILE = 2;
#define AMQ_T() __builtin_amdgcn_s_memtime()
    AMQ_STAMP_AT(blk, 96 + wave);
    bool first_ = true;
    for (; idx + 2 * U <= total; idx += U) {
#pragma unroll
        for (int u = 0; u < U; ++u) {
            const unsigned long long t0 = AMQ_T();
            AMQ_WAIT_VM("gemv.stamp", (U - 1) * OPS_PER_TILE, "");
            if (first_) { AMQ_STAMP_AT(blk, 112 + wave); first_ = false; }
            const unsigned long long t1 = AMQ_T();
            AMQ_COMPUTE(u);
            __builtin_amdgcn_sched_barrier(0);
            AMQ_ISSUE(u);
            __builtin_amdgcn_sched_barrier(0);
            const unsigned long long t2 = AMQ_T();
            AMQ_ROWEND();
            const unsigned long long t3 = AMQ_T();
            c_wait += t1 - t0; c_math += t2 - t1; c_row += t3 - t2;
        }
    }
    if (blk.stamps && lane == 0) {
        blk.stamps[(size_t)blockIdx.x * 128 + 32 + wave * 4 + 0] = c_wait;
        blk.stamps[(size_t)blockIdx.x * 128 + 32 + wave * 4 + 1] = c_math;
        blk.stamps[(size_t)blockIdx.x * 128 + 32 + wave * 4 + 2] = c_row;
        blk.stamps[(size_t)blockIdx.x * 128 + 32 + wave * 4 + 3] = (unsigned long long)idx;
    }
#else
#ifndef AMQ_NO_PRIO_PROGRESS
    const int q1_ = total >> 2, q2_ = total >> 1, q3_ = q1_ + q2_;
#endif
    for (; idx + 2 * U <= total; idx += U) {
#pragma unroll
        for (int u = 0; u < U; ++u) {
            AMQ_COMPUTE(u);
            __builtin_amdgcn_sched_barrier(0);
            AMQ_ISSUE(u);
            __builtin_amdgcn_sched_barrier(0);
            AMQ_ROWEND();
        }
#ifndef AMQ_NO_PRIO_PROGRESS
        plevel_ = idx + U >= q3_ ? 0 : idx + U >= q2_ ? 1 : idx + U >= q1_ ? 2 : 3;
        AMQ_SETPRIO_LEVEL();
#endif
    }
#endif
#pragma unroll
    for (int u = 0; u < U; ++u) {
        if (idx + u < total) {
            AMQ_COMPUTE(u);
            __builtin_amdgcn_sched_barrier(0);
            if (idx + u + U < total) AMQ_ISSUE(u);
            AMQ_ROWEND();
        }
    }
    idx += U;
#pragma unroll
    for (int u = 0; u < U; ++u)
        if (idx + u < total) { AMQ_COMPUTE(u); AMQ_ROWEND(); }
#ifdef AMQ_ABL_NOFINISH
    cj = 0;
    AMQ_FINISH();
#endif
    AMQ_STAMP_AT(blk, 8 + wave);
#undef AMQ_ISSUE
#undef AMQ_ISSUE_AT
#undef AMQ_COMPUTE
#undef AMQ_ROWEND
#undef AMQ_RESTAGE
#undef AMQ_RESTAGE_NRING
#undef AMQ_EPI_PREFETCH
#undef AMQ_SETPRIO_LEVEL
#undef AMQ_FINISH
}

#ifndef AMQ_LB_WAVES
#define AMQ_LB_WAVES(NW_) 1
#endif
struct GemvPre {
    const void* x; const void* xw; const void* qw0; const void* mt0;
    int K, m_nseg, rpt, n_rt0, key0; float eps;
};

#ifndef AMQ_LB_WAVES_G
#define AMQ_LB_WAVES_G(NW_, GP_) (((GP_) == 2 && (NW_) == 8) ? 6 : AMQ_LB_WAVES(NW_))
#endif
#ifndef AMQ_LB_WAVES_M
#define AMQ_LB_WAVES_M(NW_, GP_, MATH_, XCH_) (((MATH_) == MATH_GS && (NW_) == 8 && (GP_) == 1 && (XCH_) == 1) ? 6 : AMQ_LB_WAVES_G(NW_, GP_))
#endif
#ifndef AMQ_RS64_WAVES
#define AMQ_RS64_WAVES 6
#endif
#ifndef AMQ_LB_WAVES_R
#define AMQ_LB_WAVES_R(NW_, GP_, MATH_, XCH_, RS_) (((RS_) == 64 && (NW_) == 8) ? AMQ_RS64_WAVES : ((RS_) == 128 && (NW_) == 8) ? 4 : (RS_) == 128 ? 1 : AMQ_LB_WAVES_M(NW_, GP_, MATH_, XCH_))
#endif
template <int PRO, int NW, int U, int MATH, int XCH, int RS = 256, int GP = 1, int PH = 1>
__global__ __launch_bounds__(NW * 64, AMQ_LB_WAVES_R(NW, GP, MATH, XCH, RS)) void gemv_kernel(const void* p_x, const void* p_xw, const void* p_qw0,
                                                                     const void* p_mt0, int p_K, int p_m_nseg, int p_rpt,
                                                                     int p_n_rt0, int p_key0, float p_eps, GemvKArgs blk) {
    extern __shared__ __attribute__((aligned(16))) unsigned char smem[];
#ifndef AMQ_NO_PRIO_PROGRESS
    __builtin_amdgcn_s_setprio(3);
#endif
    GemvHot a;
    a.x = p_x; a.x2 = p_xw; a.gamma = p_xw;
    if (PRO == PRO_RMSNORM_SUMS) a.x2 = blk.x2;
    a.K = p_K; a.M = p_m_nseg & 0xFF; a.rpt = p_rpt; a.eps = p_eps;
    const int nseg = p_m_nseg >> 16;
    const bool dense = (p_m_nseg >> 8) & 1;
    const int Kst = a.K / PH;
    const bool fits = (Kst >> 3) <= XCH * NW * 64;
    int xmode = (a.M == 1 && fits && PH == 1) ? 1 : 0;
    if (RS != 256 && MATH != MATH_LINEAR && fits && dense && a.M >= 2 && a.M <= RowsCfg<RS>::MRMAX) xmode = 2;
    if (PH > 1 && xmode != 2) return;
    if (PRO == PRO_RMSNORM_SUMS && xmode != 2) return;
    const bool slow_x = xmode == 0;
    a.x_stride = slow_x ? blk.x_stride : a.K;
    const int xs = Kst + XPAD;
    _Float16* xl = (_Float16*)smem;
    const size_t xbytes = ((size_t)a.M * xs * 2 + 15) & ~(size_t)15;
    float* xg = (float*)(smem + xbytes);
    const size_t xgbytes = (MATH == MATH_LINEAR) ? (size_t)(a.K >> 7) * 64 : 0;
    float* red = (float*)(smem + xbytes + xgbytes);

    XRegs xr;
    if (xmode == 1) x_issue<PRO, NW, XCH>(a, xr);
    else if (RS != 256 && xmode == 2) x_dma_rows<PRO, NW, XCH>(a, xl, xs, xr, 0, Kst);

    const int bid = (int)blockIdx.x;
    int sidx = 0;
    int wgb = 0, nrt = p_n_rt0, key = p_key0;
    const void* qwp = p_qw0;
    const void* mtp = p_mt0;
    if (nseg > 1) {
        asm volatile("" ::"s"(blk.wg_begin[1]), "s"(blk.wg_begin[2]), "s"(blk.wg_begin[3]), "s"(blk.n_rt[1]),
                     "s"(blk.n_rt[2]), "s"(blk.n_rt[3]), "s"(blk.key[1]), "s"(blk.key[2]), "s"(blk.key[3]),
                     "s"(blk.qweight[1]), "s"(blk.qweight[2]), "s"(blk.qweight[3]), "s"(blk.meta[1]), "s"(blk.meta[2]),
                     "s"(blk.meta[3]));
#pragma unroll
        for (int i = 1; i < GEMV_MAX_SEG; ++i) {
            const bool take = i < nseg && bid >= blk.wg_begin[i];
            sidx = take ? i : sidx;
            wgb = take ? blk.wg_begin[i] : wgb;
            nrt = take ? blk.n_rt[i] : nrt;
            key = take ? blk.key[i] : key;
            qwp = take ? blk.qweight[i] : qwp;
            mtp = take ? blk.meta[i] : mtp;
        }
    }
    const int local = bid - wgb;
#ifdef AMQ_STAMP
    if (threadIdx.x == 0 && blk.stamps) {
        blk.stamps[(size_t)blockIdx.x * 128 + 0] = __builtin_amdgcn_s_memrealtime();
        blk.stamps[(size_t)blockIdx.x * 128 + 5] = __builtin_amdgcn_s_memtime();
        blk.stamps[(size_t)blockIdx.x * 128 + 3] = ((unsigned long long)__builtin_amdgcn_s_getreg((31 << 11) | 20) << 32) |
                                                (unsigned)__builtin_amdgcn_s_getreg((31 << 11) | 4);
    }
#endif

    const _Float16* xuse = xl;
    constexpr bool HAS_FMA1 = (MATH == MATH_EXACT || MATH == MATH_GS) && GP == 1;
    bool done = false;
    if constexpr (HAS_FMA1) {
        if (key == 4 * 4 + MODE_FMA1) { gemv_body<4, MODE_FMA1, PRO, NW, U, MATH, XCH, RS, false, GP, PH>(a, blk, sidx, qwp, mtp, nrt, local, xl, xuse, xg, red, xs, xmode, xr); done = true; }
        else if (key == 3 * 4 + MODE_FMA1) { gemv_body<3, MODE_FMA1, PRO, NW, U, MATH, XCH, RS, false, GP, PH>(a, blk, sidx, qwp, mtp, nrt, local, xl, xuse, xg, red, xs, xmode, xr); done = true; }
        else if (key == 2 * 4 + MODE_FMA1) { gemv_body<2, MODE_FMA1, PRO, NW, U, MATH, XCH, RS, false, GP, PH>(a, blk, sidx, qwp, mtp, nrt, local, xl, xuse, xg, red, xs, xmode, xr); done = true; }
    }
    if (!done) switch (key) {
        case 4 * 4 + MODE_HQQ: gemv_body<4, MODE_HQQ, PRO, NW, U, MATH, XCH, RS, false, GP, PH>(a, blk, sidx, qwp, mtp, nrt, local, xl, xuse, xg, red, xs, xmode, xr); break;
        case 3 * 4 + MODE_HQQ: gemv_body<3, MODE_HQQ, PRO, NW, U, MATH, XCH, RS, false, GP, PH>(a, blk, sidx, qwp, mtp, nrt, local, xl, xuse, xg, red, xs, xmode, xr); break;
        case 2 * 4 + MODE_HQQ: gemv_body<2, MODE_HQQ, PRO, NW, U, MATH, XCH, RS, false, GP, PH>(a, blk, sidx, qwp, mtp, nrt, local, xl, xuse, xg, red, xs, xmode, xr); break;
        case 4 * 4 + MODE_FMA: gemv_body<4, MODE_FMA, PRO, NW, U, MATH, XCH, RS, false, GP, PH>(a, blk, sidx, qwp, mtp, nrt, local, xl, xuse, xg, red, xs, xmode, xr); break;
        case 3 * 4 + MODE_FMA: gemv_body<3, MODE_FMA, PRO, NW, U, MATH, XCH, RS, false, GP, PH>(a, blk, sidx, qwp, mtp, nrt, local, xl, xuse, xg, red, xs, xmode, xr); break;
        default:               gemv_body<2, MODE_FMA, PRO, NW, U, MATH, XCH, RS, false, GP, PH>(a, blk, sidx, qwp, mtp, nrt, local, xl, xuse, xg, red, xs, xmode, xr); break;
    }
    if (threadIdx.x < 64) AMQ_STAMP_AT(blk, 4);
#ifdef AMQ_STAMP
    if (threadIdx.x == 0 && blk.stamps) blk.stamps[(size_t)blockIdx.x * 128 + 6] = __builtin_amdgcn_s_memtime();
#endif
}


template <int PRO, int NW, int U, int MATH, int XCH = XCfg<NW>::XC, int RS = 256, int GP = 1, int PH = 1>
inline hipError_t launch_one(const GemvKArgs& a, int total_wg, size_t lds, hipStream_t st) {
    auto kern = gemv_kernel<PRO, NW, U, MATH, XCH, RS, GP, PH>;
    if (lds > 64 * 1024) {
        hipError_t e = hipFuncSetAttribute((const void*)kern, hipFuncAttributeMaxDynamicSharedMemorySize, (int)lds);
        if (e != hipSuccess) return e;
    }
    const void* xw = PRO == PRO_SILU_MUL ? a.x2 : a.gamma;
    hipLaunchKernelGGL(kern, dim3(total_wg), dim3(NW * 64), lds, st, a.x, xw, a.qweight[0], a.meta[0], a.K,
                       a.M | ((a.x_stride == a.K ? 1 : 0) << 8) | (a.nseg << 16), a.rpt, a.n_rt[0], a.key[0], a.eps, a);
    return hipGetLastError();
}

template <int PRO, int NW, int MATH>
inline hipError_t launch_std(const GemvKArgs& a, int flags, int total_wg, size_t lds, hipStream_t st) {
    if (NW == 8 && (flags & GEMV_FLAG_RS64)) return launch_one<PRO, 8, 2, MATH, XCfg<8>::XC, 64>(a, total_wg, lds, st);
    if (NW == 8 && (flags & GEMV_FLAG_RS128)) return launch_one<PRO, 8, 2, MATH, XCfg<8>::XC, 128>(a, total_wg, lds, st);
    if (NW == 16 && (flags & GEMV_FLAG_RS64)) return launch_one<PRO, 16, 2, MATH, XCfg<16>::XC, 64>(a, total_wg, lds, st);
    if constexpr (NW == 16 && PRO != PRO_RMSNORM) {
        if (flags & GEMV_FLAG_PH2) return launch_one<PRO, 16, 2, MATH, 1, 128, 1, 2>(a, total_wg, lds, st);
    }
    if (NW == 16 && (flags & GEMV_FLAG_RS128)) return launch_one<PRO, 16, 2, MATH, XCfg<16>::XC, 128>(a, total_wg, lds, st);
    if (NW == 16 && a.M == 1 && (a.K >> 3) > XCfg<16>::XC * 1024 && (a.K >> 3) <= 4 * 1024)
        return launch_one<PRO, 16, 2, MATH, 4>(a, total_wg, lds, st);
    if (NW == 8 && a.M == 1 && (a.K >> 3) > 512 && (a.K >> 3) <= 1024)
        return launch_one<PRO, 8, 2, MATH, 2>(a, total_wg, lds, st);
    return launch_one<PRO, NW, 2, MATH>(a, total_wg, lds, st);
}

template <int PRO, int NW>
inline hipError_t launch_nw(const GemvKArgs& a, int flags, int depth, int total_wg, size_t lds, hipStream_t st) {
    const int u = depth ? depth : 2;
    if ((flags & GEMV_FLAG_DOT) && a.M == 1) return launch_one<PRO, NW, 2, MATH_DOT>(a, total_wg, lds, st);
    if (flags & GEMV_FLAG_LINEAR) {
        if (u == 4) return launch_one<PRO, NW, 4, MATH_LINEAR>(a, total_wg, lds, st);
        return launch_one<PRO, NW, 2, MATH_LINEAR>(a, total_wg, lds, st);
    }
    if (u == 4) return launch_one<PRO, NW, 4, MATH_EXACT>(a, total_wg, lds, st);
    if (flags & GEMV_FLAG_GS) return launch_std<PRO, NW, MATH_GS>(a, flags, total_wg, lds, st);
    return launch_std<PRO, NW, MATH_EXACT>(a, flags, total_wg, lds, st);
}


template <int PRO, int GP>
hipError_t launch_pro_g(const GemvKArgs& a, int nw, int total_wg, size_t lds, hipStream_t st) {
    if (nw == 4) return launch_one<PRO, 4, 2, MATH_EXACT, XCfg<4>::XC, 256, GP>(a, total_wg, lds, st);
    if (nw == 16) return launch_one<PRO, 16, 2, MATH_EXACT, XCfg<16>::XC, 256, GP>(a, total_wg, lds, st);
    return launch_one<PRO, 8, 2, MATH_EXACT, XCfg<8>::XC, 256, GP>(a, total_wg, lds, st);
}

template <int PRO>
hipError_t launch_pro(const GemvKArgs& a, int flags, int depth, int nw, int total_wg, size_t lds, hipStream_t st) {
    if (nw == 4) return launch_nw<PRO, 4>(a, flags, depth, total_wg, lds, st);
    if (nw == 16) return launch_nw<PRO, 16>(a, flags, depth, total_wg, lds, st);
    return launch_nw<PRO, 8>(a, flags, depth, total_wg, lds, st);
}


}
```

amq_amd/csrc/amq_gemv_pro3.hip:

```cpp
#include "amq_gemv_body.cuh"
namespace amq {
hipError_t launch_pro_sums_entry(const GemvKArgs& a, int nw, int rs, int total_wg, size_t lds, hipStream_t st) {
    if (rs == 64) {
        if (nw == 16) return launch_one<PRO_RMSNORM_SUMS, 16, 2, MATH_EXACT, XCfg<16>::XC, 64>(a, total_wg, lds, st);
        return launch_one<PRO_RMSNORM_SUMS, 8, 2, MATH_EXACT, XCfg<8>::XC, 64>(a, total_wg, lds, st);
    }
    if (nw == 16) return launch_one<PRO_RMSNORM_SUMS, 16, 2, MATH_EXACT, XCfg<16>::XC, 128>(a, total_wg, lds, st);
    return launch_one<PRO_RMSNORM_SUMS, 8, 2, MATH_EXACT, XCfg<8>::XC, 128>(a, total_wg, lds, st);
}
}
```

amq_amd/csrc/amq_gemv_qkvattn.hip:

```cpp
#include "amq_gemv_body.cuh"

namespace amq {

struct AttnTail { void* kc; void* vc; const void* state; void* out; int* tickets; int n_heads, n_kv_heads, max_seq; };
constexpr int QA_PF = 4;
constexpr int QA_GROUPS = 32;
constexpr unsigned QA_SPIN_LIMIT = 1u << 20;

__device__ __forceinline__ float qa_row16_sum(float v) {
    v += __builtin_bit_cast(float, __builtin_amdgcn_update_dpp(0, __builtin_bit_cast(int, v), 0xB1, 0xF, 0xF, false));
    v += __builtin_bit_cast(float, __builtin_amdgcn_update_dpp(0, __builtin_bit_cast(int, v), 0x4E, 0xF, 0xF, false));
    v += __builtin_bit_cast(float, __builtin_amdgcn_update_dpp(0, __builtin_bit_cast(int, v), 0x141, 0xF, 0xF, false));
    v += __builtin_bit_cast(float, __builtin_amdgcn_update_dpp(0, __builtin_bit_cast(int, v), 0x140, 0xF, 0xF, false));
    return v;
}
__device__ __forceinline__ float qa_row16_max(float v) {
    v = fmaxf(v, __builtin_bit_cast(float, __builtin_amdgcn_update_dpp(__builtin_bit_cast(int, v), __builtin_bit_cast(int, v), 0xB1, 0xF, 0xF, false)));
    v = fmaxf(v, __builtin_bit_cast(float, __builtin_amdgcn_update_dpp(__builtin_bit_cast(int, v), __builtin_bit_cast(int, v), 0x4E, 0xF, 0xF, false)));
    v = fmaxf(v, __builtin_bit_cast(float, __builtin_amdgcn_update_dpp(__builtin_bit_cast(int, v), __builtin_bit_cast(int, v), 0x141, 0xF, 0xF, false)));
    v = fmaxf(v, __builtin_bit_cast(float, __builtin_amdgcn_update_dpp(__builtin_bit_cast(int, v), __builtin_bit_cast(int, v), 0x140, 0xF, 0xF, false)));
    return v;
}
__device__ __forceinline__ float qa_wave4(float v, bool mx) {
    const float a = __builtin_bit_cast(float, __builtin_amdgcn_readlane(__builtin_bit_cast(int, v), 0));
// ... 48 lines not shown
        }
    }
    if (tid == 0) {
        int bad = 0;
        unsigned spins = 0;
        while (__hip_atomic_load(at.tickets + h, __ATOMIC_RELAXED, __HIP_MEMORY_SCOPE_AGENT) != 24) {
            if (++spins > QA_SPIN_LIMIT) { bad = 1; break; }
            __builtin_amdgcn_s_sleep(1);
        }
        if (!bad) __hip_atomic_store(at.tickets + h, 0, __ATOMIC_RELAXED, __HIP_MEMORY_SCOPE_AGENT);
        if (bad || !pos_ok) *(int*)((char*)const_cast<void*>(at.state) + 260) = 1;
        *flag = bad;
    }
    __syncthreads();
    if (*flag || !pos_ok) return;

    _Float16 q0 = 0, q1 = 0, k0 = 0, k1 = 0, v0 = 0, v1 = 0;
    h2 cs = {(_Float16)1.f, (_Float16)0.f};
    if (tid < 64) {
        q0 = qa_ldh(q + tid); q1 = qa_ldh(q + tid + 64);
        k0 = qa_ldh(kn + tid); k1 = qa_ldh(kn + tid + 64);
        cs = ((const h2*)at.state)[tid];
        v0 = qa_ldh(vn + tid); v1 = qa_ldh(vn + tid + 64);
        const _Float16 c16 = cs.x, s16 = cs.y;
        const int i = tid;
        qs[i] = q0 * c16 + (-q1) * s16;
        qs[i + 64] = q1 * c16 + q0 * s16;
        const _Float16 r0 = k0 * c16 + (-k1) * s16, r1 = k1 * c16 + k0 * s16;
        ks[i] = r0;
        ks[i + 64] = r1;
        vs[i] = v0;
        vs[i + 64] = v1;
        if (h % group == 0) {
            kc[(size_t)pos * D + i] = r0;
            kc[(size_t)pos * D + i + 64] = r1;
            vc[(size_t)pos * D + i] = v0;
            vc[(size_t)pos * D + i + 64] = v1;
        }
    }
    __syncthreads();
    const float scale = rsqrtf((float)D);
    {
        const h8 qv = *(const h8*)(qs + 8 * l16);
        const h8 knew = *(const h8*)(ks + 8 * l16);
        auto score = [&](const h8& kv) {
            float s = 0.f;
#pragma unroll
            for (int e = 0; e < 4; ++e)
                s = __builtin_amdgcn_fdot2((h2){qv[2 * e], qv[2 * e + 1]}, (h2){kv[2 * e], kv[2 * e + 1]}, s, false);
            s = qa_row16_sum(s);
            return (float)(_Float16)((float)(_Float16)s * scale);
        };
#pragma unroll
        for (int i = 0; i < QA_PF; ++i) {
            if (QA_GROUPS * i < T) {
                const int t = grp + QA_GROUPS * i;
                const float sv = score(t == pos ? knew : krow[i]);
                if (t < T && l16 == 0) sc[t] = sv;
            }
        }
        for (int t = grp + QA_GROUPS * QA_PF; t < T; t += QA_GROUPS) {
            const h8 kv = (t == pos) ? knew : *(const h8*)(kc + (size_t)t * D + 8 * l16);
            const float sv = score(kv);
            if (l16 == 0) sc[t] = sv;
        }
    }
    __syncthreads();
    float lmax = -INFINITY;
    for (int t = tid; t < T; t += THREADS) lmax = fmaxf(lmax, sc[t]);
    lmax = qa_wave4(qa_row16_max(lmax), true);
    if ((tid & 63) == 0) red[tid >> 6] = lmax;
    __syncthreads();
    float gmax = red[0];
#pragma unroll
    for (int w = 1; w < THREADS / 64; ++w) gmax = fmaxf(gmax, red[w]);
    float lsum = 0.f;
    for (int t = tid; t < T; t += THREADS) {
        const float e = __expf(sc[t] - gmax);
        sc[t] = e;
        lsum += e;
    }
    lsum = qa_wave4(qa_row16_sum(lsum), false);
    if ((tid & 63) == 0) red[THREADS / 64 + (tid >> 6)] = lsum;
    __syncthreads();
    float tot = 0.f;
#pragma unroll
    for (int w = 0; w < THREADS / 64; ++w) tot += red[THREADS / 64 + w];
    const float inv = 1.0f / tot;
    float o[8] = {0, 0, 0, 0, 0, 0, 0, 0};
    const h8 vnew = *(const h8*)(vs + 8 * l16);
#pragma unroll
    for (int i = 0; i < QA_PF; ++i) {
        const int t = grp + QA_GROUPS * i;
        if (QA_GROUPS * i < T && t < T) {
            const _Float16 p16 = (_Float16)(sc[t] * inv);
            const h8 vv = (t == pos) ? vnew : vrow[i];
#pragma unroll
            for (int e = 0; e < 8; ++e) o[e] += (float)p16 * (float)vv[e];
        }
    }
    for (int t = grp + QA_GROUPS * QA_PF; t < T; t += QA_GROUPS) {
        const _Float16 p16 = (_Float16)(sc[t] * inv);
        const h8 vv = (t == pos) ? vnew : *(const h8*)(vc + (size_t)t * D + 8 * l16);
#pragma unroll
        for (int e = 0; e < 8; ++e) o[e] += (float)p16 * (float)vv[e];
    }
#pragma unroll
    for (int e = 0; e < 8; ++e) part[grp * D + 8 * l16 + e] = o[e];
    __syncthreads();
    if (tid < D) {
        float acc = 0.f;
#pragma unroll
        for (int g = 0; g < QA_GROUPS; ++g) acc += part[g * D + tid];
        ((_Float16*)at.out)[(size_t)h * D + tid] = (_Float16)acc;
    }
}

template <int U, int XCH>
__global__ __launch_bounds__(512, 6) void gemv_qkv_attn_kernel(const void* p_x, const void* p_xw, const void* p_qw0, const void* p_mt0, int p_K,
                                                            int p_m_nseg, int p_rpt, int p_n_rt0, int p_key0, float p_eps, GemvKArgs blk,
                                                            AttnTail at) {
    constexpr int NW = 8, PRO = PRO_RMSNORM, MATH = MATH_EXACT;
    extern __shared__ __attribute__((aligned(16))) unsigned char smem[];
#ifndef AMQ_NO_PRIO_PROGRESS
    __builtin_amdgcn_s_setprio(3);
#endif
    GemvHot a;
    a.x = p_x; a.x2 = p_xw; a.gamma = p_xw;
    a.K = p_K; a.M = 1; a.rpt = p_rpt; a.eps = p_eps;
    a.x_stride = a.K;
    const int xs = a.K + XPAD;
    _Float16* xl = (_Float16*)smem;
    const size_t xbytes = ((size_t)xs * 2 + 15) & ~(size_t)15;
    float* xg = (float*)(smem + xbytes);
    float* red = (float*)(smem + xbytes);
    const int bid = (int)blockIdx.x;
    int sidx = 0, wgb = 0, nrt = p_n_rt0, key = p_key0;
    const void* qwp = p_qw0;
    const void* mtp = p_mt0;
    asm volatile("" ::"s"(blk.wg_begin[1]), "s"(blk.wg_begin[2]), "s"(blk.n_rt[1]), "s"(blk.n_rt[2]), "s"(blk.key[1]), "s"(blk.key[2]),
                 "s"(blk.qweight[1]), "s"(blk.qweight[2]), "s"(blk.meta[1]), "s"(blk.meta[2]));
#pragma unroll
    for (int i = 1; i < 3; ++i) {
        const bool take = bid >= blk.wg_begin[i];
        sidx = take ? i : sidx;
        wgb = take ? blk.wg_begin[i] : wgb;
        nrt = take ? blk.n_rt[i] : nrt;
        key = take ? blk.key[i] : key;
        qwp = take ? blk.qweight[i] : qwp;
        mtp = take ? blk.meta[i] : mtp;
    }
    const int local = bid - wgb;
    XRegs xr;
    x_issue<PRO, NW, XCH>(a, xr);
    switch (key) {
        case 4 * 4 + MODE_HQQ: gemv_body<4, MODE_HQQ, PRO, NW, U, MATH, XCH, 256, true>(a, blk, sidx, qwp, mtp, nrt, local, xl, xl, xg, red, xs, 1, xr); break;
        case 3 * 4 + MODE_HQQ: gemv_body<3, MODE_HQQ, PRO, NW, U, MATH, XCH, 256, true>(a, blk, sidx, qwp, mtp, nrt, local, xl, xl, xg, red, xs, 1, xr); break;
        case 2 * 4 + MODE_HQQ: gemv_body<2, MODE_HQQ, PRO, NW, U, MATH, XCH, 256, true>(a, blk, sidx, qwp, mtp, nrt, local, xl, xl, xg, red, xs, 1, xr); break;
        case 4 * 4 + MODE_FMA: gemv_body<4, MODE_FMA, PRO, NW, U, MATH, XCH, 256, true>(a, blk, sidx, qwp, mtp, nrt, local, xl, xl, xg, red, xs, 1, xr); break;
        case 3 * 4 + MODE_FMA: gemv_body<3, MODE_FMA, PRO, NW, U, MATH, XCH, 256, true>(a, blk, sidx, qwp, mtp, nrt, local, xl, xl, xg, red, xs, 1, xr); break;
        default:               gemv_body<2, MODE_FMA, PRO, NW, U, MATH, XCH, 256, true>(a, blk, sidx, qwp, mtp, nrt, local, xl, xl, xg, red, xs, 1, xr); break;
    }
    asm volatile("s_waitcnt vmcnt(0)" ::: "memory");
    __syncthreads();
    const int sp_base = nrt & GEMV_SPLIT_BASE_MASK, sp_rem = nrt >> GEMV_SPLIT_BASE_BITS;
    const int rt0 = local * sp_base + (local < sp_rem ? local : sp_rem);
    const int n_my = sp_base + (local < sp_rem ? 1 : 0);
    const int group = at.n_heads / at.n_kv_heads;
    if (threadIdx.x == 0) {
        for (int rt = rt0; rt < rt0 + n_my; ++rt) {
            if (sidx == 0) {
                __hip_atomic_fetch_add(at.tickets + (rt >> 3), 1, __ATOMIC_RELAXED, __HIP_MEMORY_SCOPE_AGENT);
            } else {
                for (int j = 0; j < group; ++j)
                    __hip_atomic_fetch_add(at.tickets + (rt >> 3) * group + j, 1, __ATOMIC_RELAXED, __HIP_MEMORY_SCOPE_AGENT);
            }
        }
    }
    if (sidx == 0) {
        for (int h = (rt0 + 7) >> 3; 8 * h < rt0 + n_my && h < at.n_heads; ++h) {
            __syncthreads();
            qkv_attention(at, h, (const _Float16*)blk.y[0], (const _Float16*)blk.y[1], (const _Float16*)blk.y[2], smem);
        }
    }
}

size_t gemv_qkv_attn_lds_bytes(int K, int max_seq) {
    const size_t g = gemv_lds_bytes(1, K, 16);
    const size_t t = 6 * 128 + 64 + (size_t)QA_GROUPS * 128 * 4 + (size_t)max_seq * 4;
    return g > t ? g : t;
}

hipError_t launch_gemv_qkv_attn(GemvArgs& a, const AttnArgs& t, int* tickets, hipStream_t st) {
    StreamDevice sd_(st);
    int total_rt = 0;
    for (int i = 0; i < 3; ++i) { a.seg[i].n_rt = a.seg[i].N / 16; total_rt += a.seg[i].n_rt; }
    const int chunks = a.K >> 3;
    if (chunks > 1024) return hipErrorInvalidValue;
    const bool two = chunks > 512;
    const int target = two ? 512 : 768;
    int rpt = (total_rt + target - 1) / target;
    if (rpt < 1) rpt = 1;
    int wg = 0;
    for (int i = 0; i < 3; ++i) {
        a.seg[i].wg_begin = wg;
        a.seg[i].wg_count = (a.seg[i].n_rt + rpt - 1) / rpt;
        wg += a.seg[i].wg_count;
    }
    GemvKArgs k{};
    k.x = a.x; k.x2 = nullptr; k.gamma = a.gamma;
    k.M = 1; k.K = a.K; k.x_stride = a.K; k.nseg = 3; k.eps = a.eps; k.rpt = rpt;
    for (int i = 0; i < 3; ++i) {
        const GemvSeg& s = a.seg[i];
        k.wg_begin[i] = s.wg_begin; k.n_rt[i] = gemv_split(s.n_rt, s.wg_count); k.key[i] = s.bits * 4 + (s.mode == MODE_FMA1 ? (int)MODE_FMA : s.mode);
        k.qweight[i] = s.qweight; k.meta[i] = s.meta; k.bias[i] = nullptr; k.residual[i] = nullptr; k.y[i] = s.y; k.y_stride[i] = s.N;
    }
    k.wg_begin[3] = 0x7fffffff;
#ifdef AMQ_STAMP
    k.stamps = nullptr;
#endif
    AttnTail at{t.kcache, t.vcache, t.rope_cur, t.out, tickets, t.n_heads, t.n_kv_heads, t.max_seq};
    const size_t lds = gemv_qkv_attn_lds_bytes(a.K, t.max_seq);
    static unsigned long long attr2_done = 0, attr1_done = 0;
    if (two) {
        auto kern = gemv_qkv_attn_kernel<2, 2>;
        if (lds > 64 * 1024) { hipError_t e = ensure_dyn_lds(attr2_done, (const void*)kern, 160 * 1024); if (e != hipSuccess) return e; }
        hipLaunchKernelGGL(kern, dim3(wg), dim3(512), lds, st, k.x, k.gamma, k.qweight[0], k.meta[0], k.K, 1 | (3 << 16), rpt, k.n_rt[0], k.key[0], k.eps, k, at);
    } else {
        auto kern = gemv_qkv_attn_kernel<2, 1>;
        if (lds > 64 * 1024) { hipError_t e = ensure_dyn_lds(attr1_done, (const void*)kern, 160 * 1024); if (e != hipSuccess) return e; }
        hipLaunchKernelGGL(kern, dim3(wg), dim3(512), lds, st, k.x, k.gamma, k.qweight[0], k.meta[0], k.K, 1 | (3 << 16), rpt, k.n_rt[0], k.key[0], k.eps, k, at);
    }
    return hipGetLastError();
}


}
```

amq_amd/csrc/amq_kernels.h:

```cpp
#pragma once
#include <hip/hip_runtime.h>
#include <stddef.h>
#include <stdint.h>

namespace amq {

inline hipError_t ensure_dyn_lds(unsigned long long& done_mask, const void* fn, int bytes) {
    int dev = 0;
    hipError_t e = hipGetDevice(&dev);
    if (e != hipSuccess) return e;
    const unsigned long long bit = 1ull << (dev & 63);
    if (__atomic_load_n(&done_mask, __ATOMIC_RELAXED) & bit) return hipSuccess;
    e = hipFuncSetAttribute(fn, hipFuncAttributeMaxDynamicSharedMemorySize, bytes);
    if (e == hipSuccess) __atomic_fetch_or(&done_mask, bit, __ATOMIC_RELAXED);
    return e;
}

struct StreamDevice {
    int prev = -1;
    bool switched = false;
    explicit StreamDevice(hipStream_t st) {
        hipDevice_t dev = 0;
        if (st == nullptr || hipGetDevice(&prev) != hipSuccess || hipStreamGetDevice(st, &dev) != hipSuccess) return;
        if ((int)dev != prev && hipSetDevice((int)dev) == hipSuccess) switched = true;
    }
    ~StreamDevice() { if (switched) (void)hipSetDevice(prev); }
    StreamDevice(const StreamDevice&) = delete;
    StreamDevice& operator=(const StreamDevice&) = delete;
};

enum { PRO_NONE = 0, PRO_RMSNORM = 1, PRO_SILU_MUL = 2,
       PRO_RMSNORM_SUMS = 3  };
enum { FMT_HQQ = 0, FMT_GPTQ = 1, FMT_AWQ = 2 };
constexpr int GEMV_MAX_SEG = 4;

struct GemvSeg {
    const void* qweight;
    const void* meta;
    const void* bias;
    const void* residual;
    void* y;
    int N;
    int bits;
    int mode;
    int wg_begin;
    int wg_count;
    int n_rt;
    int y_stride;
};

struct GemvArgs {
    GemvSeg seg[GEMV_MAX_SEG];
    int nseg;
    int M, K;
    int x_stride;
    const void* x;
    const void* x2;
    const void* gamma;
    float eps;
    int prologue;
    int flags;
    int force_waves;
    int force_depth;
    int force_rpt;
    int gp;
    const void* sums_in;
    void* sums_out;
};
constexpr int GEMV_SPLIT_BASE_BITS = 12, GEMV_SPLIT_BASE_MASK = (1 << GEMV_SPLIT_BASE_BITS) - 1;
inline int gemv_split(int n_rt, int wg_count) { return (n_rt / wg_count) | ((n_rt % wg_count) << GEMV_SPLIT_BASE_BITS); }
enum { GEMV_FLAG_DOT = 1, GEMV_FLAG_LINEAR = 2, GEMV_FLAG_RS128 = 4 ,
       GEMV_FLAG_GS = 8 ,
       GEMV_FLAG_RS64 = 16 ,
       GEMV_FLAG_PH2 = 32  };
constexpr int GEMV_MAX_M = 16;

size_t gemv_lds_bytes(int M, int K, int copies);
size_t gemv_lds_bytes_rows(int M, int K, int nw);
size_t gemv_min_lds_bytes(int M, int K, bool plain, bool norm = true);
bool gemv_rows_phased(int M, int K, bool plain, bool norm);
hipError_t launch_gemv(GemvArgs& a, hipStream_t st);

struct GemmArgs {
    const void* x; const void* qweight; const void* meta; const void* bias; void* y;
    int M, N, K, bits, mode, x_stride, y_stride;
    float* ws;
    int splits;
    const void* residual;
    const void* gate;
    void* w16;
    int gp;
};
enum { GEMM_ROUTE_AUTO = 0, GEMM_ROUTE_TILED = 1, GEMM_ROUTE_SKINNY = 2, GEMM_ROUTE_RING = 3, GEMM_ROUTE_RING128 = 4, GEMM_ROUTE_WS = 5,
       GEMM_ROUTE_DEQ = 6  };
struct GemmNorm { const void* gamma; float eps; void* xf; bool done; };
hipError_t launch_gemm(const GemmArgs& a, hipStream_t st, int route = GEMM_ROUTE_AUTO, GemmNorm* norm = nullptr);
bool gemm_gate_fused(const GemmArgs& a, int route);
hipError_t launch_gemm_ring(const GemmArgs& a, hipStream_t st, int bm = 0);
bool gemm_ring_ok(const GemmArgs& a);
hipError_t launch_gemm_ws(const GemmArgs& a, hipStream_t st);
int gemm_ring_rows(int M, int N);
int gemm_many_rows_plan(int M, int N);
bool gemm_takes_ring(int M, int N, int K);
hipError_t launch_gemm_xfrag(const GemmArgs& a, hipStream_t st);
hipError_t launch_xfrag(const void* src, void* xf, int M, int K, long stride_m, long stride_kt, hipStream_t st);
hipError_t launch_gemm_xfrag_grouped(const void* xf, int M, int K, const GemvSeg* segs, int nseg, hipStream_t st, int form = 0, int nsub_forced = 0);
hipError_t launch_gemm_fewrow_stream_grouped(const void* xf, int M, int K, const GemvSeg* segs, int nseg, hipStream_t st, int nsub_forced = 0);
int fewrow_stream_nsub(const int* seg_blocks, int nseg, int row_groups, int cus);
int gemm_pick_splits(int M, int N, int K, int route = GEMM_ROUTE_AUTO);
bool gemm_f16w_ok(int M, int N, int K, int x_stride, int y_stride);
bool gemm_fine_takes_deq(int M, int N, int K);
bool gemm_fine_takes_skinny(int M);
bool gemm_takes_deq(int M, int N, int K);
hipError_t launch_gemm_f16w(const void* x, const void* w, const void* bias, const void* residual, const void* gate, void* y,
                            int M, int N, int K, int x_stride, int y_stride, hipStream_t st);

struct AttnArgs {
    const void* q;
    const void* k;
    const void* v;
    void* kcache;
    void* vcache;
    void* out;
    const int* pos_dev;
    int pos;
    int n_heads, n_kv_heads, max_seq;
    float rope_theta;
    const void* rope_table;
    const void* rope_cur;
};
hipError_t launch_rope_table(void* tab, int max_seq, float theta, hipStream_t st);
hipError_t launch_rope_table_freqs(void* tab, int max_seq, const void* inv_freq, float scale, hipStream_t st);
hipError_t launch_attn_decode(const AttnArgs& a, int batch, hipStream_t st);
#ifndef AMQ_ATT_MIN_CHUNK
#define AMQ_ATT_MIN_CHUNK 256
#endif
constexpr int ATT_MIN_CHUNK = AMQ_ATT_MIN_CHUNK;
hipError_t launch_attn_decode_split(const AttnArgs& a, int batch, int n_splits, void* ws, void* tickets, hipStream_t st);
#ifndef AMQ_ATT_GQA
#define AMQ_ATT_GQA 1
#endif
bool attn_decode_takes_gqa(int n_heads, int n_kv_heads, int max_seq, int n_splits);
int attn_decode_gqa_iters(int max_seq, int n_splits);
hipError_t launch_attn_decode_gqa(const AttnArgs& a, int batch, int n_splits, void* ws, void* tickets, hipStream_t st);
hipError_t launch_rmsnorm(const void* x, const void* gamma, void* y, int M, int K, float eps, hipStream_t st);
hipError_t launch_rmsnorm_xfrag(const void* x, const void* gamma, void* xf, int M, int K, float eps, hipStream_t st);
struct AttnPrefillArgs {
    const void* q; const void* k; const void* v; void* out;
    int S;
    int pos0;
    int n_heads, n_kv_heads, batch;
    long q_rstride, q_bstride, k_rstride, k_bstride, k_hstride, v_rstride, v_bstride, v_hstride, o_rstride, o_bstride;
    int out_xfrag;
};
hipError_t launch_attn_prefill(const AttnPrefillArgs& a, hipStream_t st);
hipError_t launch_rope_cache(void* q, const void* k, const void* v, void* kcache, void* vcache, const void* rope_table,
                             int rope_rows, int pos0, int S, int n_heads, int n_kv_heads, int max_seq, hipStream_t st,
                             int batch = 1);
hipError_t launch_rope_rows(void* q, void* k, const void* rope_table, int rope_rows, int pos0, int rows, int seq_len, int n_heads,
                            int n_kv_heads, hipStream_t st);
hipError_t launch_silu_mul(const void* gate, const void* up, void* out, long n, hipStream_t st);
hipError_t launch_decode_tail(const void* logits, int vocab, const void* embed, int hidden, void* token, void* pos, void* x,
                              const void* rope_table, void* rope_cur, int rope_rows, hipStream_t st, int batch = 1, const void* suppress = nullptr);
hipError_t launch_set_token(const void* token_in, int n_in, const void* embed, int vocab, int hidden, void* token, const void* pos, void* x,
                            const void* rope_table, void* rope_cur, int rope_rows, int batch, hipStream_t st);
hipError_t launch_gemv_f16w(const void* x, const void* W, const void* bias, void* y, const void* gamma, float eps,
                            int N, int K, hipStream_t st, int M = 1);

hipError_t launch_gemv_qkv_attn(GemvArgs& a, const AttnArgs& t, int* tickets, hipStream_t st);
size_t gemv_qkv_attn_lds_bytes(int K, int max_seq);

struct EngineDesc {
    const void* blocks_dev;
    int n_block;
    int H, I, n_heads, n_kv_heads, max_seq;
    float eps;
    void* x;
    void* scratch;
    const void* state;
    void* sync;
    int grid;
    int depth;
};
struct EngineLinearH { const void* qweight; const void* meta; int N; int bits; int mode; };
size_t engine_image_bytes(int n_block);
// ... 23 lines not shown
```

amq_amd/llama.py:

```python
import math

import torch

from . import ops
from .arch import MODEL_CONFIGS, arch_bits, rope_inv_freq, uniform_arch
from .hqq_format import HQQWeights

EPS = 1e-5
ROPE_THETA = 10000.0


class _Lin:
    __slots__ = ("qn", "mn", "bits", "mode", "N", "K", "bias")

    def __init__(self, qn, mn, bits, mode, N, K, bias=None):
        self.qn, self.mn, self.bits, self.mode, self.N, self.K, self.bias = qn, mn, bits, mode, N, K, bias

    def seg(self, y, residual=None):
        return dict(qn=self.qn, mn=self.mn, bits=self.bits, mode=self.mode, N=self.N, y=y, residual=residual, bias=self.bias)

    def nbytes(self):
        return self.qn.numel() * 4 + self.mn.numel() * 2 + (0 if self.bias is None else self.bias.numel() * 2)


def _synthetic_linear(n, k, bits, gen, device, group=128):
    qb, mb = ops.native_sizes(bits, n, k, group)
    qn = torch.randint(-2 ** 31, 2 ** 31 - 1, (qb // 4,), dtype=torch.int32, device=device, generator=gen)
    std_q = math.sqrt((4.0 ** bits - 1.0) / 12.0)
    s0 = 0.5 / (math.sqrt(k) * std_q)
    r = torch.rand(mb // 4, 2, device=device, generator=gen)
    meta = torch.empty(mb // 4, 2, dtype=torch.float16, device=device)
    meta[:, 0] = (s0 * (0.75 + 0.5 * r[:, 0])).to(torch.float16)
    meta[:, 1] = ((2 ** bits - 1) / 2.0 + (r[:, 1] - 0.5)).to(torch.float16)
    return _Lin(qn, meta.reshape(-1).contiguous(), bits, ops.MODE_HQQ, n, k)


_GRAPH_STATE_PRIMED = set()


class _no_gc:

    def __enter__(self):
        import gc
        self.was = gc.isenabled()
        gc.collect()
        gc.disable()

    def __exit__(self, *exc):
        import gc
        if self.was:
            gc.enable()
        return False


def _prime_graph_state(dev):
    key = (dev.type, dev.index)
    if key in _GRAPH_STATE_PRIMED or dev.type != "cuda":
        return
    with torch.inference_mode(False):
        side = torch.cuda.Stream(device=dev)
        with torch.cuda.stream(side):
            g = torch.cuda.CUDAGraph()
            keep = torch.zeros(1, device=dev)
            with torch.cuda.graph(g, stream=side, capture_error_mode="thread_local"):
                keep += 1
        side.synchronize()
    _GRAPH_STATE_PRIMED.add(key)


class QuantLlama:
    ENGINE_MAX_SEQ = 512
    DOWN_FUSED_ROWS = 1
    NORM_FUSED_ROWS = 4
    NORM_SUMS = True
    FUSE_QKV_ATTN = False
    ENGINE_DEFAULT = False
    all_logits = False
    fine = False

    def __init__(self, config, arch_linear=None, device="cuda:0", max_seq=256, seed=0, synthetic=True,
                 hqq_layers=None, dense=None, batch=1, engine=None, prebuilt=None, group=128, rope=None):
        if isinstance(config, str):
            config = MODEL_CONFIGS[config]
        if not 1 <= int(batch) <= 8:
            raise ValueError("batch must be 1..8")
        self.B = int(batch)
        self.cfg = config
        self.dev = torch.device(device)
        _prime_graph_state(self.dev)
        self.H = config["hidden_size"]
        self.I = config["intermediate_size"]
        self.nh, self.nkv = config["num_heads"], config["num_kv_heads"]
        if config["head_dim"] != 128:
            raise ValueError("head_dim must be 128")
        self.kvd = self.nkv * 128
        self.nb = config["n_block"]
        self.vocab = config["vocab_size"]
        self.max_seq = max_seq
        self.eps = float(config.get("rms_norm_eps", EPS))
        self.theta = float(config.get("rope_theta", ROPE_THETA))
        arch_linear = arch_linear or uniform_arch(config, 4)["linear"]
        self.arch_linear = arch_linear
        gen = torch.Generator(device=self.dev).manual_seed(seed)
        dev = self.dev

        def lin(block, name):
            n, k = config["linear_shape"][name]
            bits = arch_bits(arch_linear, name, block)
            if prebuilt is not None:
                l = prebuilt[(block, name)]
                assert l.bits == bits and (l.N, l.K) == (n, k) and l.qn.device == dev
                return l
            if hqq_layers is not None:
                h: HQQWeights = hqq_layers[(block, name)].to(dev)
                assert h.nbits == bits and tuple(h.shape) == (n, k)
                qn, mn = ops.repack_from_hqq(h.W_q.contiguous(), h.scale.reshape(-1).contiguous(),
                                             h.zero.reshape(-1).contiguous(), bits, n, k, group=h.group_size)
                return _Lin(qn, mn, bits, ops.MODE_HQQ, n, k, None if h.bias is None else h.bias.to(dev, torch.float16).contiguous())
            if not synthetic:
                raise ValueError("no weights given")
            l = _synthetic_linear(n, k, bits, gen, dev, group)
            if config.get("qkv_bias") and name in ("self_attn.q_proj", "self_attn.k_proj", "self_attn.v_proj"):
                l.bias = (0.1 * torch.randn(n, device=dev, generator=gen)).to(torch.float16)
            return l

        self.blocks = []
        for b in range(self.nb):
            blk = {name: lin(b, name) for name in config["linear"]}
            if dense is not None:
                blk["ln1"], blk["ln2"] = dense["ln1"][b].to(dev), dense["ln2"][b].to(dev)
            else:
                blk["ln1"] = (1.0 + 0.05 * torch.randn(self.H, device=dev, generator=gen)).to(torch.float16)
                blk["ln2"] = (1.0 + 0.05 * torch.randn(self.H, device=dev, generator=gen)).to(torch.float16)
            blk["kc"] = torch.zeros(self.B, self.nkv, max_seq, 128, dtype=torch.float16, device=dev)
            blk["vc"] = torch.zeros(self.B, self.nkv, max_seq, 128, dtype=torch.float16, device=dev)
            self.blocks.append(blk)
        if dense is not None:
            self.embed, self.lm_head, self.norm = dense["embed"].to(dev), dense["lm_head"].to(dev), dense["norm"].to(dev)
        else:
            self.embed = (torch.randn(self.vocab, self.H, device=dev, generator=gen)).to(torch.float16)
            self.lm_head = (torch.randn(self.vocab, self.H, device=dev, generator=gen) / math.sqrt(self.H)).to(torch.float16)
            self.norm = (1.0 + 0.05 * torch.randn(self.H, device=dev, generator=gen)).to(torch.float16)

        self.fine = any(blk[n].mn.numel() != ops.native_sizes(blk[n].bits, blk[n].N, blk[n].K)[1] // 2 for blk in self.blocks for n in config["linear"])
        if self.fine and engine:
            raise ValueError("the decode engine serves groups of 128")
        for bi, blk in enumerate(self.blocks):
            for sibs in (("self_attn.q_proj", "self_attn.k_proj", "self_attn.v_proj"), ("mlp.gate_proj", "mlp.up_proj")):
                pairs = {blk[n].mn.numel() * 128 // (2 * blk[n].N * blk[n].K) for n in sibs}
                if len(pairs) != 1:
                    raise ValueError(f"block {bi}: {', '.join(sibs)} mix group sizes ({sorted(128 // p for p in pairs)}); the runner issues them as "
                                     "one grouped launch, which needs one group size per sibling set")

        f16 = dict(dtype=torch.float16, device=dev)
        B = self.B
        self.x = torch.zeros(B, self.H, **f16)
        self.xn = torch.zeros(B, self.H, **f16)
        self.q = torch.zeros(B, self.H, **f16)
        self.k = torch.zeros(B, self.kvd, **f16)
        self.v = torch.zeros(B, self.kvd, **f16)
        self.att = torch.zeros(B, self.H, **f16)
        self.gate = torch.zeros(B, self.I, **f16)
        self.up = torch.zeros(B, self.I, **f16)
        self.logits = torch.zeros(self.vocab, **f16) if B == 1 else torch.zeros(B, self.vocab, **f16)
        self.token = torch.zeros(B, dtype=torch.int64, device=dev)
        self.pos = torch.zeros(1, dtype=torch.int32, device=dev)
        self.inv_freq, self.rope_scale = rope if rope is not None else rope_inv_freq(config)
        self.rope_tab = ops.rope_table(max_seq, self.theta, dev, inv_freq=self.inv_freq, scale=self.rope_scale)
        self.rope_cur, self.pos, self.step_err = ops.new_step_state(dev)
        self.rope_cur.copy_(self.rope_tab.view(max_seq, 128)[0])
        self.graph = None
        self.host_pos = 0
        self.suppress = torch.full((8,), -1, dtype=torch.int32, device=dev)
        self.has_bias = any(blk[n].bias is not None for blk in self.blocks for n in config["linear"])
        self._down_rows_fit = self.B <= min(ops.gemv_max_rows(self.I, plain=not self.fine), self.DOWN_FUSED_ROWS)
        self._down_rows_phased = not self._down_rows_fit and self.B <= ops.gemv_max_rows(self.I, plain=not self.fine, norm=False)
        self.can_fuse_qkv_attn = self.B == 1 and max_seq <= ops.ATTN_SPLIT_FROM and self.H <= 8192 and not self.fine and not self.has_bias
        self.fuse_qkv_attn = self.FUSE_QKV_ATTN and self.can_fuse_qkv_attn
        self._tickets = torch.zeros(max(self.nh, 64), dtype=torch.int32, device=dev)
        self._norm_sums = (self.NORM_SUMS and 2 <= self.B <= 8 and not self.fine and 2048 <= self.H <= 8192 and self.I >= 2048
                           and self.B <= ops.gemv_max_rows(self.H, plain=True))
        self.ss = torch.zeros(self.B, self.H // 16, dtype=torch.float32, device=dev) if self._norm_sums else None
        eligible = self.B == 1 and max_seq <= self.ENGINE_MAX_SEQ and self.H == self.nh * 128 and not self.fine and not self.has_bias
        if engine and not eligible:
            raise ValueError("the decode engine needs batch 1 and max_seq <= %d" % self.ENGINE_MAX_SEQ)
        self.engine = None
        if engine is None:
            engine = self.ENGINE_DEFAULT
        if eligible and engine:
            self.engine = ops.DecodeEngine(
                [dict({n: dict(qn=blk[n].qn, mn=blk[n].mn, bits=blk[n].bits, mode=blk[n].mode, N=blk[n].N) for n in ops.ENGINE_LINEARS},
                      ln1=blk["ln1"], ln2=blk["ln2"], kc=blk["kc"], vc=blk["vc"]) for blk in self.blocks],
                self.H, self.I, self.nh, self.nkv, max_seq, self.eps, self.x.view(-1), self.rope_cur)

    HF_MODEL_TYPES = ("llama", "mistral", "qwen2")

    @classmethod
    def check_hf(cls, model, max_seq=None):
        from .checkpoint import runner_config
        hf = model.config.to_dict()
        mt = hf.get("model_type", "llama")
        if mt not in cls.HF_MODEL_TYPES:
            raise ValueError(f"from_hf: model_type '{mt}' is not one of {cls.HF_MODEL_TYPES} (a Llama-shaped decoder is required)")
        if hf.get("hidden_act", "silu") != "silu":
            raise ValueError("from_hf: a SiLU-gated MLP is required")
        attn0 = model.model.layers[0].self_attn
        if any(hasattr(attn0, n) for n in ("q_norm", "k_norm")):
            raise ValueError("from_hf: per-head q / k norms are not part of the runner's block")
        from .quant_linear import HIPQuantLinear
        if not isinstance(getattr(attn0, "q_proj", None), HIPQuantLinear):
            raise ValueError("from_hf: the decoder linears are not HIPQuantLinear modules: run prepare_for_inference(model, backend='hip') first")
        rp = hf.get("rope_parameters") or {}
        if hf.get("rope_theta") is None:
            hf["rope_theta"] = rp.get("rope_theta", 10000.0)
        rot = getattr(model.model, "rotary_emb", None)
        kind = getattr(rot, "rope_type", None) or rp.get("rope_type") or (hf.get("rope_scaling") or {}).get("rope_type", "default")
        rope = None
        if kind != "default":
            if kind not in ("llama3", "linear", "yarn") or rot is None or getattr(rot, "inv_freq", None) is None:
                raise ValueError(f"from_hf: rope type '{kind}' is not served (default, linear, llama3, yarn: the static ones)")
            rope = (rot.inv_freq.detach().to(torch.float32), float(getattr(rot, "attention_scaling", 1.0)))
            if rope[0].numel() != 64:
                raise ValueError("from_hf: head_dim must be 128")
        sw = hf.get("sliding_window")
        sliding = sw is not None and hf.get("use_sliding_window", True) is not False and \
            (not hf.get("layer_types") or any(t == "sliding_attention" for t in hf["layer_types"]))
        if sliding and max_seq is not None and max_seq > int(sw):
            raise ValueError(f"from_hf: max_seq {max_seq} exceeds the model's sliding window ({sw}): the runner attends the whole cache")
        cfg = runner_config(hf)
        return cfg, rope

    @classmethod
    def from_hf(cls, model, max_seq=256, batch=1, engine=None):
        from .quant_linear import HIPQuantLinear
        cfg, rope = cls.check_hf(model, max_seq)
        layers = model.model.layers
        pre, arch_linear = {}, {name: [] for name in cfg["linear"]}
        dev = None
        f16 = lambda t: t.detach() if t.dtype is torch.float16 else t.detach().to(torch.float16)
        for b, layer in enumerate(layers):
            for name in cfg["linear"]:
                parent, attr = name.split(".")
                m = getattr(getattr(layer, parent), attr)
                if not isinstance(m, HIPQuantLinear) or not m.qweight.is_cuda:
                    raise ValueError(f"model.layers.{b}.{name}: expected a HIPQuantLinear on the GPU (run prepare_for_inference first)")
                if m.is_bf16:
                    raise ValueError(f"model.layers.{b}.{name}: a bfloat16 module -- the decode runner is fp16 (the reference's kernels are, ft.py:62); "
                                     "bf16 models run through the modules' own forward")
                dev = dev or m.qweight.device
                pre[(b, name)] = _Lin(m.qweight, m.meta, m.bits, m.mode, m.outfeatures, m.infeatures, None if m.bias is None else f16(m.bias))
                arch_linear[name].append(m.bits)
        dense = {"embed": f16(model.model.embed_tokens.weight), "lm_head": f16(model.lm_head.weight), "norm": f16(model.model.norm.weight),
                 "ln1": [f16(l.input_layernorm.weight) for l in layers], "ln2": [f16(l.post_attention_layernorm.weight) for l in layers]}
        return cls(cfg, arch_linear, device=dev, max_seq=max_seq, dense=dense, batch=batch, engine=engine, prebuilt=pre, synthetic=False, rope=rope)

    def linear_bytes_per_token(self):
        return sum(blk[name].nbytes() for blk in self.blocks for name in self.cfg["linear"])

    def total_bytes_per_token(self, context):
        kv = 2 * self.nb * self.nkv * 128 * 2 * context
        return self.linear_bytes_per_token() + self.lm_head.numel() * 2 + kv

    def _step(self):
        H = self.H
        if self.engine is not None:
            self.engine.step()
            ops.gemv_f16w(self.x.reshape(-1), self.lm_head, gamma=self.norm, eps=self.eps, out=self.logits)
            ops.decode_tail(self.logits, self.embed, self.token, self.pos, self.x, table=self.rope_tab, cur=self.rope_cur, suppress=self.suppress)
            return
        have_sums = False
        for blk in self.blocks:
            if self.fuse_qkv_attn:
                ops.gemv_qkv_attn(self.x, [blk["self_attn.q_proj"].seg(self.q.view(-1)), blk["self_attn.k_proj"].seg(self.k.view(-1)),
                                           blk["self_attn.v_proj"].seg(self.v.view(-1))], H, blk["ln1"], self.eps, blk["kc"], blk["vc"],
                                  self.att.view(-1), self.rope_cur, self.nh, self.nkv, self._tickets)
            else:
                qkv = [blk["self_attn.q_proj"].seg(self.q), blk["self_attn.k_proj"].seg(self.k), blk["self_attn.v_proj"].seg(self.v)]
                if self._norm_sums and have_sums:
                    ops.gemv_grouped_sums(self.x, qkv, H, gamma=blk["ln1"], eps=self.eps, sums_in=self.ss)
                elif self.B > self.NORM_FUSED_ROWS:
                    ops.gemv_grouped(ops.rmsnorm(self.x, blk["ln1"], self.eps, out=self.xn), qkv, H)
                else:
                    ops.gemv_grouped(self.x, qkv, H, prologue=ops.PRO_RMSNORM, gamma=blk["ln1"], eps=self.eps)
                ops.attn_decode(self.q, self.k, self.v, blk["kc"], blk["vc"], self.att, self.pos, self.nh, self.nkv, self.theta,
                                cur=self.rope_cur)
            if self._norm_sums:
                ops.gemv_grouped_sums(self.att, [blk["self_attn.o_proj"].seg(self.x, residual=self.x)], H, sums_out=self.ss)
                ops.gemv_grouped_sums(self.x, [blk["mlp.gate_proj"].seg(self.gate), blk["mlp.up_proj"].seg(self.up)], H,
                                      gamma=blk["ln2"], eps=self.eps, sums_in=self.ss)
            else:
                ops.gemv_grouped(self.att, [blk["self_attn.o_proj"].seg(self.x, residual=self.x)], H)
            if self._norm_sums:
                pass
            elif self.B > self.NORM_FUSED_ROWS:
                ops.gemv_grouped(ops.rmsnorm(self.x, blk["ln2"], self.eps, out=self.xn), [blk["mlp.gate_proj"].seg(self.gate), blk["mlp.up_proj"].seg(self.up)], H)
            else:
                ops.gemv_grouped(self.x, [blk["mlp.gate_proj"].seg(self.gate), blk["mlp.up_proj"].seg(self.up)], H,
                                 prologue=ops.PRO_RMSNORM, gamma=blk["ln2"], eps=self.eps)
            if self._down_rows_fit:
                ops.gemv_grouped(self.gate, [blk["mlp.down_proj"].seg(self.x, residual=self.x)], self.I,
                                 prologue=ops.PRO_SILU_MUL, x2=self.up)
            elif self._down_rows_phased and self._norm_sums:
                ops.gemv_grouped_sums(ops.silu_mul(self.gate, self.up, out=self.gate), [blk["mlp.down_proj"].seg(self.x, residual=self.x)], self.I,
                                      sums_out=self.ss)
                have_sums = True
            elif self._down_rows_phased:
                ops.gemv_grouped(ops.silu_mul(self.gate, self.up, out=self.gate), [blk["mlp.down_proj"].seg(self.x, residual=self.x)], self.I)
            else:
                d = blk["mlp.down_proj"]
                ops.gemm(ops.silu_mul(self.gate, self.up, out=self.gate), d.qn, d.mn, d.bits, d.mode, d.N, d.K, bias=d.bias, residual=self.x, out=self.x)
                have_sums = False
        ops.gemv_f16w(self.x.reshape(-1) if self.B == 1 else self.x, self.lm_head, gamma=self.norm, eps=self.eps, out=self.logits)
        ops.decode_tail(self.logits, self.embed, self.token, self.pos, self.x, table=self.rope_tab, cur=self.rope_cur, suppress=self.suppress)

    def set_suppressed(self, ids=()):
        ids = [int(i) for i in ids]
        if len(ids) > 8:
            raise ValueError("at most 8 suppressed token ids")
        self.suppress.copy_(torch.tensor(ids + [-1] * (8 - len(ids)), dtype=torch.int32))
        self._suppressed = tuple(ids)

    def _argmax(self, logits, dim, keepdim=False):
        assert dim in (-1, logits.dim() - 1)
        m = torch.zeros(self.vocab + 1, dtype=torch.float32, device=logits.device)
        m.index_fill_(0, torch.where(self.suppress >= 0, self.suppress, self.vocab).to(torch.int64), float("-inf"))
        return torch.argmax(logits.float() + m[:self.vocab], dim=dim, keepdim=keepdim)

    def set_pos(self, pos):
        pos = int(pos)
        if not 0 <= pos <= self.max_seq:
            raise ValueError(f"position {pos} outside the KV cache (max_seq={self.max_seq})")
        self.pos.fill_(pos)
        self.host_pos = pos

    def check(self):
        try:
            ops.check_step_state(self.step_err)
        except Exception:
            self._tickets.zero_()
            raise
        if self.engine is not None:
            try:
                self.engine.check()
            except Exception:
                self.graph = None
                raise

    def set_token(self, token):
        if isinstance(token, torch.Tensor) and token.is_cuda and token.dtype is torch.int64 and token.numel() in (1, self.B) and token.is_contiguous():
            return ops.set_token(token, self.embed, self.token, self.pos, self.x, table=self.rope_tab, cur=self.rope_cur)
        if isinstance(token, torch.Tensor):
            self.token.copy_(token.reshape(-1).expand(self.B) if token.numel() == 1 else token.reshape(self.B))
        else:
            self.token.fill_(int(token))
        torch.index_select(self.embed, 0, self.token, out=self.x)
        torch.index_select(self.rope_tab.view(self.max_seq, 128), 0, self.pos.to(torch.int64).clamp_(0, self.max_seq - 1),
                           out=self.rope_cur.view(1, 128))

    def capture(self):
        if self.graph is not None:
            return
        if self.host_pos >= self.max_seq:
            raise ValueError(f"cannot capture a decode step at position {self.host_pos}: the KV cache holds {self.max_seq} rows")
        side = torch.cuda.Stream(device=self.dev)
        side.wait_stream(torch.cuda.current_stream(self.dev))
        saved = (self.token.clone(), self.pos.clone())
        with torch.cuda.stream(side):
            self._step()
            side.synchronize()
            self.pos.copy_(saved[1]); self.set_token(saved[0])
            g = torch.cuda.CUDAGraph()
            with _no_gc(), torch.cuda.graph(g, stream=side, capture_error_mode="thread_local"):
                self._step()
        torch.cuda.current_stream(self.dev).wait_stream(side)
        torch.cuda.synchronize(self.dev)
        self.pos.copy_(saved[1]); self.set_token(saved[0])
        self.graph = g

    def decode_step(self, use_graph=True):
        if self.host_pos >= self.max_seq:
            raise ValueError(f"decode step at position {self.host_pos} does not fit the KV cache (max_seq={self.max_seq})")
        if use_graph and self.graph is None:
            self.capture()
        self.host_pos += 1
        if use_graph:
            self.graph.replay()
        else:
            self._step()

    def _rope(self, t, positions):
        inv = 1.0 / (self.theta ** (torch.arange(0, 128, 2, device=self.dev, dtype=torch.float32) / 128.0)) if self.inv_freq is None \
            else self.inv_freq.to(self.dev, torch.float32)
        fr = positions.to(torch.float32)[:, None] * inv[None, :]
        emb = torch.cat([fr, fr], dim=-1)
        cos, sin = (emb.cos() * self.rope_scale).to(torch.float16)[:, None, :], (emb.sin() * self.rope_scale).to(torch.float16)[:, None, :]
        t1, t2 = t[..., :64], t[..., 64:]
        rot = torch.cat([-t2, t1], dim=-1)
        return t * cos + rot * sin

    def prefill(self, ids, use_graph=True, start_pos=0):
        ids = self._ids_rows(ids)
        S = ids.shape[1]
        start_pos = int(start_pos)
        if start_pos < 0 or start_pos + S > self.max_seq:
            raise ValueError("prompt longer than the KV cache")
        if not use_graph:
            return self._prefill_rows(ids, start_pos)
        cache = self.__dict__.setdefault("_prefill_graphs", {})
        ent = cache.get((S, start_pos))
        if ent is None:
            static_ids = ids.to(self.dev).clone()
            side = torch.cuda.Stream(device=self.dev)
            side.wait_stream(torch.cuda.current_stream(self.dev))
            with torch.cuda.stream(side):
                self._prefill_rows(static_ids, start_pos)
                side.synchronize()
                g = torch.cuda.CUDAGraph()
                with _no_gc(), torch.cuda.graph(g, stream=side, capture_error_mode="thread_local"):
                    self._prefill_rows(static_ids, start_pos)
            torch.cuda.current_stream(self.dev).wait_stream(side)
            ent = cache[(S, start_pos)] = (g, static_ids, self.__dict__.get("logits_rows"))
        g, static_ids, rows = ent
        static_ids.copy_(ids)
        g.replay()
        if rows is not None:
            self.logits_rows = rows
        self.host_pos = start_pos + S
        return self.logits

    def _ids_rows(self, ids):
        ids = ids.to(self.dev)
        if ids.dim() == 1:
            ids = ids[None, :]
        if ids.dim() != 2 or ids.shape[0] != self.B:
            raise ValueError(f"expected {self.B} prompt(s) of equal length, got ids of shape {tuple(ids.shape)}")
        return ids

    def _prefill_rows(self, ids, start_pos):
        if self.B == 1:
            return self._prefill_eager(ids[0], start_pos)
        B, S = ids.shape
        last = self._rows_pass(ids, start_pos, cache=True)
        if self.all_logits:
            self.logits_rows = self._logits_of_rows(self.__dict__.pop("_rows_x"), B, S, self.logits)
        else:
            ops.gemv_f16w(last, self.lm_head, gamma=self.norm, eps=self.eps, out=self.logits)
        self.set_pos(start_pos + S)
        self.set_token(self._argmax(self.logits, 1))
        return self.logits

    def _rows_pass(self, ids, start_pos, cache):
        B, S = ids.shape
# ... 300 lines not shown
```

amq_amd/ops.py:

```python
import ctypes
import os

import torch

from . import _lib
from ._lib import (MODE_HQQ, MODE_FMA, MODE_FMA1, PRO_NONE, PRO_RMSNORM, PRO_SILU_MUL, Segment, GemvOpts, EngineBlock, EngineLinear,
                   GEMM_AUTO, GEMM_TILED, GEMM_SKINNY, GEMM_RING, GEMM_RING128, GEMM_WS, GEMM_DEQ, MATH_DEFAULT, MATH_EXACT, MATH_LINEAR, MATH_GROUPSCALE)

GROUP = 128


def _need(t, dtype, name, numel=None):
    if not isinstance(t, torch.Tensor) or not t.is_cuda:
        raise ValueError(f"{name}: expected a tensor on the GPU")
    if t.dtype != dtype:
        raise ValueError(f"{name}: expected {dtype}, got {t.dtype}")
    if not t.is_contiguous():
        raise ValueError(f"{name}: must be contiguous")
    if numel is not None and t.numel() != numel:
        raise ValueError(f"{name}: expected {numel} elements, got {t.numel()}")


FINE_GROUPS = (64, 32)

# ... 331 lines not shown

def gemm_xfrag(xf, M, qn, mn, bits, mode, N, K, bias=None, out=None, residual=None, gate=None):
    _check_shape(bits, N, K)
    _check_native(qn, mn, bits, N, K)
    _need(xf, torch.float16, "xf", _lib.load().amq_xfrag_bytes(M, K) // 2)
    if bias is not None:
        _need(bias, torch.float16, "bias", N)
    if residual is not None:
        _need(residual, torch.float16, "residual", M * N)
    if gate is not None:
        _need(gate, torch.float16, "gate", M * N)
    y = out if out is not None else torch.empty(M, N, dtype=torch.float16, device=xf.device)
    _need(y, torch.float16, "y", M * N)
    _lib.check(_lib.load().amq_gemm_xfrag_f16(bits, mode, _lib.ptr(xf), _lib.ptr(qn), _lib.ptr(mn), _lib.ptr(bias),
                                              _lib.ptr(gate), _lib.ptr(residual), _lib.ptr(y), M, N, K, GROUP, 0,
                                              _lib.current_stream()))
    return y


def gemm_xfrag_grouped(xf, M, segments, K, form=0, blocks_per_wg=0):
    if not 1 <= len(segments) <= _lib.MAX_SEGMENTS:
        raise ValueError(f"1..{_lib.MAX_SEGMENTS} segments")
    lib = _lib.load()
    _need(xf, torch.float16, "xf", lib.amq_xfrag_bytes(M, K) // 2)
    arr = (Segment * len(segments))()
    for i, s in enumerate(segments):
        _check_shape(s["bits"], s["N"], K)
        _check_native(s["qn"], s["mn"], s["bits"], s["N"], K)
        _need(s["y"], torch.float16, "y", M * s["N"])
        if s.get("bias") is not None:
            _need(s["bias"], torch.float16, "bias", s["N"])
        if s.get("residual") is not None:
            _need(s["residual"], torch.float16, "residual", M * s["N"])
        arr[i] = Segment(_lib.ptr(s["qn"]), _lib.ptr(s["mn"]), _lib.ptr(s.get("bias")), _lib.ptr(s.get("residual")),
                         _lib.ptr(s["y"]), s["N"], s["bits"], s["mode"], 0)
    _lib.check(lib.amq_gemm_xfrag_grouped_form_f16(arr, len(segments), _lib.ptr(xf), M, K, GROUP, int(form), int(blocks_per_wg), _lib.current_stream()))


def linear(x, qn, mn, bits, mode, N, K, bias=None):
    _check_shape(bits, N, K)
    group = _check_native(qn, mn, bits, N, K, fine=True)
    x2 = _prep_x(x, K)
    M = x2.shape[0]
    if bias is not None:
        _need(bias, torch.float16, "bias", N)
    if group != GROUP and M > 0:
        if M <= gemv_max_rows(K):
            return gemv(x, qn, mn, bits, mode, N, K, bias=bias)
        return gemm(x, qn, mn, bits, mode, N, K, bias=bias)
    if M > 8:
        return gemm(x, qn, mn, bits, mode, N, K, bias=bias)
    y = torch.empty(M, N, dtype=torch.float16, device=x.device)
    if M == 0:
        return y.reshape(*x.shape[:-1], N)
    _lib.check(_lib.load().amq_linear_f16(bits, mode, _lib.ptr(x2), _lib.ptr(qn), _lib.ptr(mn), _lib.ptr(bias),
                                          _lib.ptr(y), M, N, K, GROUP, _lib.current_stream()))
    return y.reshape(*x.shape[:-1], N)


_DEQ_SCRATCH_BF16 = _ScratchPool(torch.bfloat16)


def _check_native_bf16(qn, mn, bits, N, K):
    qb, mb = native_sizes(bits, N, K)
    _need(qn, torch.int32, "qweight_native", qb // 4)
    if isinstance(mn, torch.Tensor) and mn.dtype == torch.float16:
        raise ValueError("meta_native is float16: this buffer was repacked from an fp16 model -- use the fp16 entry points")
    _need(mn, torch.bfloat16, "meta_native", mb // 2)


def dequantize_bf16(qn, mn, bits, N, K, out=None):
    _check_shape(bits, N, K)
    _check_native_bf16(qn, mn, bits, N, K)
    if out is None:
        out = torch.empty(N, K, dtype=torch.bfloat16, device=qn.device)
    _need(out, torch.bfloat16, "out", N * K)
    _lib.check(_lib.load().amq_dequantize_bf16(bits, _lib.ptr(qn), _lib.ptr(mn), N, K, GROUP, _lib.ptr(out), _lib.current_stream()))
    return out


def linear_bf16(x, qn, mn, bits, N, K, bias=None, residual=None, out=None):
    _check_shape(bits, N, K)
    _check_native_bf16(qn, mn, bits, N, K)
    if x.dtype != torch.bfloat16:
        raise ValueError(f"x: expected bfloat16, got {x.dtype}")
    if x.shape[-1] != K:
        raise ValueError(f"x: last dim {x.shape[-1]} != K={K}")
    x2 = x.reshape(-1, K)
    if not x2.is_contiguous():
        x2 = x2.contiguous()
    M = x2.shape[0]
    if bias is not None:
        _need(bias, torch.bfloat16, "bias", N)
    if residual is not None:
        _need(residual, torch.bfloat16, "residual", M * N)
    y = out if out is not None else torch.empty(M, N, dtype=torch.bfloat16, device=x.device)
    _need(y, torch.bfloat16, "y", M * N)
    if M == 0:
        return y.reshape(*x.shape[:-1], N)
    lib = _lib.load()
    need = int(lib.amq_gemm_bf16_workspace_bytes(M, N, K))
    ws = _DEQ_SCRATCH_BF16.get(x.device, need // 2) if need else None
    _lib.check(lib.amq_gemm_bf16(bits, _lib.ptr(x2), _lib.ptr(qn), _lib.ptr(mn), _lib.ptr(bias), _lib.ptr(residual), _lib.ptr(y),
                                 M, N, K, GROUP, 0, 0, _lib.ptr(ws), need, _lib.current_stream()))
    return y.reshape(*x.shape[:-1], N)


DEFAULT_GEMV_OPTS = None


def default_gemv_math():
    return int(_lib.load().amq_default_gemv_math())


def gemv_max_rows(K, plain=False, norm=True):
    out = (ctypes.c_int * 6)()
    _lib.load().amq_query(int(K), out, 6)
    return int((out[4] if norm else out[5]) if plain else out[0])


def gemv_grouped(x, segments, K, prologue=PRO_NONE, x2=None, gamma=None, eps=0.0, opts=None):
    xx = _prep_x(x, K)
    M = xx.shape[0]
    if not 1 <= len(segments) <= _lib.MAX_SEGMENTS:
        raise ValueError(f"1..{_lib.MAX_SEGMENTS} segments")
    arr = (Segment * len(segments))()
    group = None
    for i, s in enumerate(segments):
        _check_shape(s["bits"], s["N"], K)
        g = _check_native(s["qn"], s["mn"], s["bits"], s["N"], K, fine=True)
        if group is not None and g != group:
            raise ValueError(f"segments of one launch must share their group size (got {group} and {g})")
        group = g
        _need(s["y"], torch.float16, "y", M * s["N"])
        if s.get("bias") is not None:
            _need(s["bias"], torch.float16, "bias", s["N"])
        if s.get("residual") is not None:
            _need(s["residual"], torch.float16, "residual", M * s["N"])
        arr[i] = Segment(_lib.ptr(s["qn"]), _lib.ptr(s["mn"]), _lib.ptr(s.get("bias")), _lib.ptr(s.get("residual")),
                         _lib.ptr(s["y"]), s["N"], s["bits"], s["mode"], 0)
    if prologue == PRO_RMSNORM:
        _need(gamma, torch.float16, "gamma", K)
    if prologue == PRO_SILU_MUL:
        x2 = _prep_x(x2, K)
        if x2.shape[0] != M:
            raise ValueError("x2 rows != x rows")
    if opts is None:
        opts = DEFAULT_GEMV_OPTS
    _lib.check(_lib.load().amq_gemv_grouped_f16(arr, len(segments), _lib.ptr(xx), _lib.ptr(x2), _lib.ptr(gamma),
                                                ctypes.c_float(eps), prologue, M, K, group, 0,
                                                ctypes.byref(opts) if opts is not None else None, _lib.current_stream()))


def gemv_grouped_sums(x, segments, K, gamma=None, eps=0.0, sums_in=None, sums_out=None):
    xx = _prep_x(x, K)
    M = xx.shape[0]
    if not 1 <= len(segments) <= _lib.MAX_SEGMENTS:
        raise ValueError(f"1..{_lib.MAX_SEGMENTS} segments")
    arr = (Segment * len(segments))()
    for i, s in enumerate(segments):
        _check_shape(s["bits"], s["N"], K)
        _check_native(s["qn"], s["mn"], s["bits"], s["N"], K)
        _need(s["y"], torch.float16, "y", M * s["N"])
        if s.get("bias") is not None:
            _need(s["bias"], torch.float16, "bias", s["N"])
        if s.get("residual") is not None:
            _need(s["residual"], torch.float16, "residual", M * s["N"])
        arr[i] = Segment(_lib.ptr(s["qn"]), _lib.ptr(s["mn"]), _lib.ptr(s.get("bias")), _lib.ptr(s.get("residual")),
                         _lib.ptr(s["y"]), s["N"], s["bits"], s["mode"], 0)
    if sums_in is not None:
        _need(gamma, torch.float16, "gamma", K)
        _need(sums_in, torch.float32, "sums_in", M * (K // 16))
    if sums_out is not None:
        _need(sums_out, torch.float32, "sums_out", M * (segments[0]["N"] // 16))
    _lib.check(_lib.load().amq_gemv_grouped_sums_f16(arr, len(segments), _lib.ptr(xx), _lib.ptr(gamma) if sums_in is not None else None,
                                                     ctypes.c_float(eps), _lib.ptr(sums_in), _lib.ptr(sums_out), M, K, GROUP, _lib.current_stream()))


def rmsnorm(x, gamma, eps, out=None):
    K = x.shape[-1]
    x2 = _prep_x(x, K)
    _need(gamma, torch.float16, "gamma", K)
    y = out if out is not None else torch.empty_like(x2)
    _need(y, torch.float16, "y", x2.numel())
    _lib.check(_lib.load().amq_rmsnorm_f16(_lib.ptr(x2), _lib.ptr(gamma), _lib.ptr(y), x2.shape[0], K,
                                           ctypes.c_float(eps), _lib.current_stream()))
    return y.reshape(x.shape)


def gemv_f16w(x, W, bias=None, gamma=None, eps=0.0, out=None):
    N, K = W.shape
    _need(W, torch.float16, "W", N * K)
    M = x.shape[0] if x.dim() == 2 else 1
    _need(x, torch.float16, "x", M * K)
    if gamma is not None:
        _need(gamma, torch.float16, "gamma", K)
    if bias is not None:
        _need(bias, torch.float16, "bias", N)
    shape = (M, N) if x.dim() == 2 else (N,)
    y = out if out is not None else torch.empty(shape, dtype=torch.float16, device=x.device)
    _need(y, torch.float16, "y", M * N)
    if M == 1:
        _lib.check(_lib.load().amq_gemv_f16w(_lib.ptr(x), _lib.ptr(W), _lib.ptr(bias), _lib.ptr(y), _lib.ptr(gamma),
                                             ctypes.c_float(eps), N, K, _lib.current_stream()))
    else:
        if M > 8:
            raise ValueError("at most 8 rows")
        _lib.check(_lib.load().amq_gemv_f16w_rows(_lib.ptr(x), _lib.ptr(W), _lib.ptr(bias), _lib.ptr(y), _lib.ptr(gamma),
                                                  ctypes.c_float(eps), M, N, K, _lib.current_stream()))
    return y


def decode_tail(logits, embed, token, pos, x, table=None, cur=None, suppress=None):
    vocab, hidden = embed.shape
    B = token.numel()
    _need(logits, torch.float16, "logits", B * vocab)
    _need(embed, torch.float16, "embed", vocab * hidden)
    _need(token, torch.int64, "token", B)
    _need(pos, torch.int32, "pos", 1)
    _need(x, torch.float16, "x", B * hidden)
    if cur is not None:
        _need(cur, torch.float16, "rope_cur", 128)
        _need(table, torch.float16, "rope table")
    tab = _lib.ptr(table) if cur is not None else None
    rows = table.numel() // 128 if cur is not None else 0
    if suppress is not None:
        _need(suppress, torch.int32, "suppress", 8)
        _lib.check(_lib.load().amq_decode_tail_suppress_f16(_lib.ptr(logits), vocab, _lib.ptr(embed), hidden, _lib.ptr(token), _lib.ptr(pos),
                                                            _lib.ptr(x), tab, _lib.ptr(cur), rows, B, _lib.ptr(suppress), _lib.current_stream()))
        return
    if B == 1:
        _lib.check(_lib.load().amq_decode_tail_f16(_lib.ptr(logits), vocab, _lib.ptr(embed), hidden, _lib.ptr(token), _lib.ptr(pos),
                                                   _lib.ptr(x), tab, _lib.ptr(cur), rows, _lib.current_stream()))
    else:
        _lib.check(_lib.load().amq_decode_tail_batch_f16(_lib.ptr(logits), vocab, _lib.ptr(embed), hidden, _lib.ptr(token),
                                                         _lib.ptr(pos), _lib.ptr(x), tab, _lib.ptr(cur), rows, B,
                                                         _lib.current_stream()))


def set_token(token_in, embed, token, pos, x, table=None, cur=None):
    vocab, hidden = embed.shape
    B = token.numel()
    n_in = token_in.numel()
    _need(token_in, torch.int64, "token_in", n_in)
    _need(embed, torch.float16, "embed", vocab * hidden)
    _need(token, torch.int64, "token", B)
    _need(pos, torch.int32, "pos", 1)
    _need(x, torch.float16, "x", B * hidden)
    if cur is not None:
        _need(cur, torch.float16, "rope_cur", 128)
        _need(table, torch.float16, "rope table")
    _lib.check(_lib.load().amq_set_token_f16(_lib.ptr(token_in), n_in, _lib.ptr(embed), vocab, hidden, _lib.ptr(token), _lib.ptr(pos), _lib.ptr(x),
                                             _lib.ptr(table) if cur is not None else None, _lib.ptr(cur), table.numel() // 128 if cur is not None else 0, B,
                                             _lib.current_stream()))


def rope_cache(q, k, v, kcache, vcache, table, pos0, n_heads, n_kv_heads):
    if kcache.dim() == 4:
        B = kcache.shape[0]
        rows = q.shape[0]
        if rows % B or kcache.shape[1] != n_kv_heads or kcache.shape[3] != 128 or vcache.shape != kcache.shape:
            raise ValueError("caches must be [B, n_kv_heads, max_seq, 128] and q rows a multiple of B")
        S = rows // B
        _need(q, torch.float16, "q", rows * n_heads * 128)
        _need(k, torch.float16, "k", rows * n_kv_heads * 128)
        _need(v, torch.float16, "v", rows * n_kv_heads * 128)
        _need(kcache, torch.float16, "kcache")
        _need(vcache, torch.float16, "vcache")
        _need(table, torch.float16, "rope table")
        _lib.check(_lib.load().amq_rope_cache_batch_f16(_lib.ptr(q), _lib.ptr(k), _lib.ptr(v), _lib.ptr(kcache), _lib.ptr(vcache),
                                                        _lib.ptr(table), table.numel() // 128, int(pos0), S, B, n_heads, n_kv_heads,
                                                        128, kcache.shape[2], _lib.current_stream()))
        return
    S = q.shape[0]
    _need(q, torch.float16, "q", S * n_heads * 128)
    _need(k, torch.float16, "k", S * n_kv_heads * 128)
    _need(v, torch.float16, "v", S * n_kv_heads * 128)
    if kcache.dim() != 3 or kcache.shape[0] != n_kv_heads or kcache.shape[2] != 128 or vcache.shape != kcache.shape:
        raise ValueError("caches must be [n_kv_heads, max_seq, 128]")
    _need(kcache, torch.float16, "kcache")
    _need(vcache, torch.float16, "vcache")
    _need(table, torch.float16, "rope table")
    _lib.check(_lib.load().amq_rope_cache_f16(_lib.ptr(q), _lib.ptr(k), _lib.ptr(v), _lib.ptr(kcache), _lib.ptr(vcache),
                                              _lib.ptr(table), table.numel() // 128, int(pos0), S, n_heads, n_kv_heads, 128,
                                              kcache.shape[1], _lib.current_stream()))


def attn_prefill(q, k, v, out, S, n_heads, n_kv_heads, batch=1, pos0=0, kv_cache=False, out_xfrag=False):
    H = n_heads * 128
    _need(q, torch.float16, "q", batch * S * H)
    if out_xfrag:
        if batch != 1:
            raise ValueError("out_xfrag needs batch == 1")
        nb = _lib.load().amq_xfrag_bytes(S, H)
        if out is None:
            out = torch.empty(nb // 2, dtype=torch.float16, device=q.device)
        _need(out, torch.float16, "out_xf", nb // 2)
    else:
        _need(out, torch.float16, "out", batch * S * H)
    if kv_cache:
        if k.dim() != 4 or k.shape[0] != batch or k.shape[1] != n_kv_heads or k.shape[3] != 128 or v.shape != k.shape:
            raise ValueError("caches must be [batch, n_kv_heads, max_seq, 128]")
        max_seq = k.shape[2]
        if pos0 + S > max_seq:
            raise ValueError(f"keys 0..{pos0 + S - 1} do not fit the cache (max_seq={max_seq})")
        _need(k, torch.float16, "kcache")
# ... 267 lines not shown
```

include/amq_hip.h:

```cpp
#ifndef AMQ_HIP_H
#define AMQ_HIP_H

#include <stddef.h>
#include <stdint.h>

#ifdef __cplusplus
extern "C" {
#endif

#define AMQ_VERSION 521

#define AMQ_OK            0
#define AMQ_EINVAL       -1
#define AMQ_ESHAPE       -2
#define AMQ_ELAUNCH      -3
#define AMQ_EUNSUPPORTED -4

#define AMQ_MODE_HQQ 0
#define AMQ_MODE_FMA 1
#define AMQ_MODE_FMA1 2

#define AMQ_PRO_NONE     0
#define AMQ_PRO_RMSNORM  1
#define AMQ_PRO_SILU_MUL 2

#define AMQ_MAX_SEGMENTS 4

int amq_version(void);
const char* amq_last_error(void);

#define AMQ_MATH_DEFAULT    0
#define AMQ_MATH_LINEAR     1
#define AMQ_MATH_GROUPSCALE 2
#define AMQ_MATH_EXACT      3
int amq_default_gemv_math(void);

typedef struct amq_gemv_opts {
    int math;
    int waves;
    int depth;
    int rpt;
    int dot;
} amq_gemv_opts;

#define AMQ_GEMM_AUTO   0
#define AMQ_GEMM_TILED  1
#define AMQ_GEMM_SKINNY 2
#define AMQ_GEMM_RING   3
#define AMQ_GEMM_RING128 4
#define AMQ_GEMM_WS 5
#define AMQ_GEMM_DEQ 6

int amq_query(int K, int* out, int cap);

size_t amq_native_qweight_bytes(int bits, int N, int K);
float amq_fma1_scale_bound(int bits);
size_t amq_native_meta_bytes(int N, int K, int group);

int amq_repack_from_hqq(int bits, const void* W_q, const void* scale, const void* zero,
                        int N, int K, int group, void* qweight_native, void* meta_native, void* stream);
int amq_repack_from_gptq(int bits, const void* qweight, const void* scales, const void* zeros,
                         int N, int K, int group, void* qweight_native, void* meta_native, void* stream);
int amq_repack_from_awq(const void* qweight, const void* scales, const void* scaled_zeros,
                        int N, int K, int group, void* qweight_native, void* meta_native, void* stream);

int amq_dequantize_f16(int bits, int mode, const void* qweight_native, const void* meta_native,
                       int N, int K, int group, void* W_out, void* stream);
int amq_dequantize_hqq_f16(int bits, const void* W_q, const void* scale, const void* zero,
                           int N, int K, int group, void* W_out, void* stream);

int amq_gemv_f16(int bits, int mode, const void* x, const void* qweight_native, const void* meta_native,
                 const void* bias, void* y, int M, int N, int K, int group,
                 int x_stride, int y_stride, void* stream);
int amq_gemm_f16(int bits, int mode, const void* x, const void* qweight_native, const void* meta_native,
                 const void* bias, void* y, int M, int N, int K, int group,
                 int x_stride, int y_stride, void* stream);
int amq_linear_f16(int bits, int mode, const void* x, const void* qweight_native, const void* meta_native,
                   const void* bias, void* y, int M, int N, int K, int group, void* stream);

size_t amq_gemm_splitk_workspace_bytes(int M, int N, int K);
int amq_gemm_splitk_f16(int bits, int mode, const void* x, const void* qweight_native, const void* meta_native,
                        const void* bias, void* y, int M, int N, int K, int group, int x_stride, int y_stride,
                        void* workspace, size_t workspace_bytes, void* stream);

typedef struct amq_segment {
    const void* qweight_native;
    const void* meta_native;
    const void* bias;
    const void* residual;
    void* y;
    int N;
    int bits;
    int mode;
    int y_stride;
} amq_segment;

int amq_gemv_grouped_f16(const amq_segment* segments , int nseg,
                         const void* x, const void* x2, const void* gamma, float eps, int prologue,
                         int M, int K, int group, int x_stride, const amq_gemv_opts* opts ,
                         void* stream);
int amq_gemv_grouped_sums_f16(const amq_segment* segs, int nseg, const void* x, const void* gamma, float eps, const float* sums_in,
                              float* sums_out, int M, int K, int group, void* stream);


size_t amq_compat_workspace_bytes(int bits, int M, int N, int K);
int amq_vecquantmatmul_faster_old(int bits, const void* vec, const void* mat, void* mul, const void* scales,
                                  const void* zeros, int groupsize, int vec_height, int batch, int height, int width,
                                  void* workspace, size_t workspace_bytes, int workspace_valid, void* stream);
int amq_gemv_4bit(const void* x, const void* kernel, const void* scales, const void* scaled_zeros, void* y,
                  int m, int n, int k, int group_size,
                  void* workspace, size_t workspace_bytes, int workspace_valid, void* stream);
int amq_gemm_4bit(const void* x, const void* kernel, const void* scales, const void* scaled_zeros, void* y,
                  int m, int n, int k, int group_size,
                  void* workspace, size_t workspace_bytes, int workspace_valid, void* stream);

int amq_rmsnorm_f16(const void* x, const void* gamma, void* y, int M, int K, float eps, void* stream);
int amq_gemv_f16w(const void* x, const void* W, const void* bias, void* y, const void* gamma, float eps,
                  int N, int K, void* stream);
int amq_gemv_f16w_rows(const void* x, const void* W, const void* bias, void* y, const void* gamma, float eps, int M,
                       int N, int K, void* stream);
int amq_attn_decode_f16(const void* q, const void* k, const void* v, void* kcache, void* vcache, void* out,
                        const int* pos_dev, int pos, int batch, int n_heads, int n_kv_heads, int head_dim,
                        int max_seq, float rope_theta, const void* rope_table, void* stream);
int amq_rope_table_f16(void* table, int max_seq, float rope_theta, void* stream);
int amq_rope_table_freqs_f16(void* table, int max_seq, const float* inv_freq, float scale, void* stream);

int amq_attn_decode_cur_f16(const void* q, const void* k, const void* v, void* kcache, void* vcache, void* out,
                            const void* step_state, int batch, int n_heads, int n_kv_heads, int head_dim, int max_seq,
                            void* stream);

size_t amq_attn_decode_split_workspace_bytes(int batch, int n_heads, int n_splits);
int amq_attn_decode_split_f16(const void* q, const void* k, const void* v, void* kcache, void* vcache, void* out,
                              const void* step_state, const int* pos_dev, int pos, int batch, int n_heads, int n_kv_heads,
                              int head_dim, int max_seq, float rope_theta, const void* rope_table, int n_splits,
                              void* workspace, size_t workspace_bytes, void* tickets, void* stream);

int amq_decode_tail_f16(const void* logits, int vocab, const void* embed, int hidden, long long* token, int* pos, void* x,
                        const void* rope_table, void* rope_cur, int rope_rows, void* stream);
int amq_set_token_f16(const long long* token_in, int n_in, const void* embed, int vocab, int hidden, long long* token, const int* pos, void* x,
                      const void* rope_table, void* rope_cur, int rope_rows, int batch, void* stream);
int amq_decode_tail_suppress_f16(const void* logits, int vocab, const void* embed, int hidden, long long* token, int* pos, void* x,
                                 const void* rope_table, void* rope_cur, int rope_rows, int batch, const int* suppress_ids, void* stream);
int amq_decode_tail_batch_f16(const void* logits, int vocab, const void* embed, int hidden, long long* token, int* pos, void* x,
                              const void* rope_table, void* rope_cur, int rope_rows, int batch, void* stream);


int amq_gemm_res_f16(int bits, int mode, const void* x, const void* qweight_native, const void* meta_native,
                     const void* bias, const void* residual, void* y, int M, int N, int K, int group, int x_stride,
                     int y_stride, void* workspace, size_t workspace_bytes, void* stream);
int amq_gemm_res_norm_xfrag_f16(int bits, int mode, const void* x, const void* qweight_native, const void* meta_native, const void* bias,
                                const void* residual, void* y, int M, int N, int K, int group, int x_stride, void* workspace,
                                size_t workspace_bytes, const void* gamma, float eps, void* xf, void* stream);
size_t amq_gemm_route_workspace_bytes(int route, int M, int N, int K);
size_t amq_gemm_route_workspace_bytes_g(int route, int M, int N, int K, int group);
int amq_gemm_route_f16(int route, int bits, int mode, const void* x, const void* qweight_native, const void* meta_native,
                       const void* bias, const void* residual, void* y, int M, int N, int K, int group, int x_stride,
                       int y_stride, void* workspace, size_t workspace_bytes, void* stream);
int amq_gemm_f16w_f16(const void* x, const void* w_f16, const void* bias, const void* residual, const void* gate, void* y,
                      int M, int N, int K, int x_stride, int y_stride, void* stream);
int amq_gemm_gated_fused(int route, int M, int N, int K, int use_workspace);
int amq_gemm_gated_fused_g(int route, int M, int N, int K, int use_workspace, int group);
int amq_gemm_gated_f16(int route, int bits, int mode, const void* x, const void* qweight_native, const void* meta_native,
                       const void* bias, const void* gate, void* y, int M, int N, int K, int group, int x_stride,
                       void* workspace, size_t workspace_bytes, void* stream);
size_t amq_xfrag_bytes(int M, int K);
int amq_xfrag_f16(const void* src, void* xf, int M, int K, long long stride_m, long long stride_kt, void* stream);
int amq_rmsnorm_xfrag_f16(const void* x, const void* gamma, void* xf, int M, int K, float eps, void* stream);
int amq_gemm_xfrag_f16(int bits, int mode, const void* xf, const void* qweight_native, const void* meta_native,
                       const void* bias, const void* gate, const void* residual, void* y, int M, int N, int K, int group,
                       int y_stride, void* stream);
int amq_gemm_xfrag_grouped_f16(const amq_segment* segments , int nseg, const void* xf, int M, int K, int group,
                               void* stream);
#define AMQ_FEWROW_AUTO   0
#define AMQ_FEWROW_TILE   1
#define AMQ_FEWROW_STREAM 2
int amq_gemm_xfrag_grouped_form_f16(const amq_segment* segments , int nseg, const void* xf, int M, int K, int group,
                                    int form, int blocks_per_wg, void* stream);
int amq_attn_prefill_f16(const void* q, const void* k, const void* v, void* out, int batch, int S, int pos0, int n_heads,
                         int n_kv_heads, int head_dim, long long q_rstride, long long q_bstride, long long k_rstride,
                         long long k_bstride, long long k_hstride, long long v_rstride, long long v_bstride, long long v_hstride,
                         long long o_rstride, long long o_bstride, void* stream);
int amq_attn_prefill_xfrag_f16(const void* q, const void* k, const void* v, void* out_xf, int S, int pos0, int n_heads,
                               int n_kv_heads, int head_dim, long long q_rstride, long long k_rstride, long long k_hstride,
                               long long v_rstride, long long v_hstride, void* stream);

int amq_rope_cache_f16(void* q, const void* k, const void* v, void* kcache, void* vcache, const void* rope_table,
                       int rope_rows, int pos0, int S, int n_heads, int n_kv_heads, int head_dim, int max_seq, void* stream);
int amq_rope_cache_batch_f16(void* q, const void* k, const void* v, void* kcache, void* vcache, const void* rope_table,
                             int rope_rows, int pos0, int S, int batch, int n_heads, int n_kv_heads, int head_dim, int max_seq,
                             void* stream);
int amq_rope_rows_f16(void* q, void* k, const void* rope_table, int rope_rows, int pos0, int rows, int seq_len, int n_heads,
                      int n_kv_heads, int head_dim, void* stream);
int amq_silu_mul_f16(const void* gate, const void* up, void* out, size_t n, void* stream);

int amq_dequantize_bf16(int bits, const void* qweight_native, const void* meta_native_bf16, int N, int K, int group, void* W_out, void* stream);
int amq_dequantize_hqq_bf16(int bits, const void* W_q, const void* scale, const void* zero, int N, int K, int group, void* W_out, void* stream);
int amq_gemv_bf16(int bits, const void* x, const void* qweight_native, const void* meta_native_bf16, const void* bias, const void* residual, void* y,
                  int M, int N, int K, int group, int x_stride, int y_stride, void* stream);
size_t amq_gemm_bf16_workspace_bytes(int M, int N, int K);
int amq_gemm_bf16(int bits, const void* x, const void* qweight_native, const void* meta_native_bf16, const void* bias, const void* residual, void* y,
                  int M, int N, int K, int group, int x_stride, int y_stride, void* workspace, size_t workspace_bytes, void* stream);

#ifdef __cplusplus
}
#endif
#endif
```

Baseline: 756.1 tokens/s.

## Carry per-chunk sum-of-squares from residual GEMVs into next RMSNorm prologue at batch 1

For batch-1 decode, the o_proj and down_proj GEMV epilogues now write per-8-element sums of squares of their residual outputs. The following gate/up and QKV GEMVs read those partial sums instead of recomputing the full-row reduction before applying RMSNorm. When a block owns exactly the x chunks it needs, the staging path also skips a __syncthreads. The aim is to remove the per-workgroup norm reduction and a barrier from each norm-fused GEMV, in exchange for extra epilogue readlanes and stores, a lower launch-bounds occupancy target, and more constrained launch geometry.

```diff
diff --git a/amq_amd/_lib.py b/amq_amd/_lib.py
--- a/amq_amd/_lib.py
+++ b/amq_amd/_lib.py
@@ -92,6 +92,7 @@
     "amq_silu_mul_f16": (_i, [_vp, _vp, _vp, _sz, _vp]),
     "amq_gemv_grouped_f16": (_i, [ctypes.POINTER(Segment), _i, _vp, _vp, _vp, _f, _i, _i, _i, _i, _i, ctypes.POINTER(GemvOpts), _vp]),
     "amq_gemv_grouped_sums_f16": (_i, [ctypes.POINTER(Segment), _i, _vp, _vp, _f, _vp, _vp, _i, _i, _i, _vp]),
+    "amq_gemv_row_sums_f16": (_i, [ctypes.POINTER(Segment), _i, _vp, _vp, _vp, _f, _i, _vp, _vp, _i, _vp]),
     "amq_gemm_f16w_f16": (_i, [_vp, _vp, _vp, _vp, _vp, _vp, _i, _i, _i, _i, _i, _vp]),
     "amq_gemm_route_workspace_bytes": (_sz, [_i, _i, _i, _i]),
     "amq_gemm_route_workspace_bytes_g": (_sz, [_i, _i, _i, _i, _i]),
diff --git a/amq_amd/csrc/amq_capi.hip b/amq_amd/csrc/amq_capi.hip
--- a/amq_amd/csrc/amq_capi.hip
+++ b/amq_amd/csrc/amq_capi.hip
@@ -201,6 +201,43 @@
     return check_hip(amq::launch_gemv(a, (hipStream_t)stream), "gemv_sums");
 }
 
+int amq_gemv_row_sums_f16(const amq_segment* segs, int nseg, const void* x, const void* x2, const void* gamma, float eps, int prologue,
+                          const float* sums_in, float* sums_out, int K, void* stream) {
+    if (!segs || nseg < 1 || nseg > AMQ_MAX_SEGMENTS) return fail(AMQ_EINVAL, "nseg must be 1..%d (got %d)", AMQ_MAX_SEGMENTS, nseg);
+    if (!x) return fail(AMQ_EINVAL, "null x");
+    if (prologue == AMQ_PRO_RMSNORM) {
+        if (!sums_in || !gamma) return fail(AMQ_EINVAL, "AMQ_PRO_RMSNORM: sums_in (the chunk sums of squares of x) and gamma are required");
+        if (sums_out) return fail(AMQ_EINVAL, "sums_out is written by launches without a norm (o_proj, down_proj): not together with sums_in");
+        if (K < 2048 || K > 4096) return fail(AMQ_ESHAPE, "sums_in: 2048 <= K <= 4096 (the 8-wave one-row kernels; got K=%d)", K);
+    } else if (prologue == AMQ_PRO_NONE || prologue == AMQ_PRO_SILU_MUL) {
+        if (sums_in) return fail(AMQ_EINVAL, "sums_in goes with AMQ_PRO_RMSNORM");
+        if (!sums_out) return fail(AMQ_EINVAL, "neither sums_in nor sums_out: amq_gemv_grouped_f16");
+        if (nseg != 1) return fail(AMQ_EINVAL, "sums_out describes ONE output: nseg must be 1");
+        if (prologue == AMQ_PRO_SILU_MUL && !x2) return fail(AMQ_EINVAL, "AMQ_PRO_SILU_MUL: null x2");
+    } else {
+        return fail(AMQ_EINVAL, "prologue must be AMQ_PRO_NONE, AMQ_PRO_RMSNORM or AMQ_PRO_SILU_MUL (got %d)", prologue);
+    }
+    if (amq_default_gemv_math() != AMQ_MATH_EXACT) return fail(AMQ_EUNSUPPORTED, "the chunk-sum forms run the exact arithmetic only");
+    if (amq::gemv_min_lds_bytes(1, K, false) > LDS_LIMIT) return fail(AMQ_ESHAPE, "K=%d does not fit LDS for the GEMV path", K);
+    amq::GemvArgs a{};
+    for (int i = 0; i < nseg; ++i) {
+        const amq_segment& s = segs[i];
+        if (int rc = check_shape(s.bits, s.N, K, 128)) return rc;
+        if (int rc = check_mode(s.mode)) return rc;
+        if (!s.qweight_native || !s.meta_native || !s.y) return fail(AMQ_EINVAL, "segment %d: null pointer", i);
+        amq::GemvSeg& d = a.seg[i];
+        d.qweight = s.qweight_native; d.meta = s.meta_native; d.bias = s.bias; d.residual = s.residual; d.y = s.y;
+        d.N = s.N; d.bits = s.bits; d.mode = s.mode;
+        d.y_stride = s.y_stride ? s.y_stride : s.N;
+    }
+    a.nseg = nseg; a.M = 1; a.K = K; a.x_stride = K;
+    a.x = x; a.x2 = prologue == AMQ_PRO_SILU_MUL ? x2 : nullptr; a.gamma = gamma; a.eps = eps;
+    a.prologue = prologue == AMQ_PRO_RMSNORM ? amq::PRO_RMSNORM_CHUNKS : prologue;
+    a.sums_in = sums_in; a.sums_out = sums_out;
+    a.gp = 1;
+    return check_hip(amq::launch_gemv(a, (hipStream_t)stream), "gemv_row_sums");
+}
+
 int amq_gemv_f16(int bits, int mode, const void* x, const void* qn, const void* mn, const void* bias, void* y,
                  int M, int N, int K, int group, int x_stride, int y_stride, void* stream) {
     amq_segment s{};
diff --git a/amq_amd/csrc/amq_gemv.hip b/amq_amd/csrc/amq_gemv.hip
--- a/amq_amd/csrc/amq_gemv.hip
+++ b/amq_amd/csrc/amq_gemv.hip
@@ -46,6 +46,7 @@
 AMQ_GEMV_EXTERN(PRO_SILU_MUL)
 #undef AMQ_GEMV_EXTERN
 hipError_t launch_pro_sums_entry(const GemvKArgs&, int nw, int rs, int, size_t, hipStream_t);
+hipError_t launch_pro_chunks_entry(const GemvKArgs&, int, size_t, hipStream_t);
 
 #ifndef AMQ_RS128_THREE
 #define AMQ_RS128_THREE 1
@@ -101,11 +102,17 @@
     const bool lin = (a.flags & GEMV_FLAG_LINEAR) && !((a.flags & GEMV_FLAG_DOT) && a.M == 1);
     (void)lin; (void)mask;
     const size_t lds = ph2 ? gemv_lds_bytes_rows(a.M, a.K / 2, 16) : (rs128 || rs64) ? gemv_lds_bytes_rows(a.M, a.K, nw) : gemv_lds_bytes(a.M, a.K, a.M > 1 ? nw : 16);
-    if ((a.prologue == PRO_RMSNORM_SUMS || a.sums_out) && !(rs128 || rs64)) return hipErrorInvalidValue;
+    if ((a.prologue == PRO_RMSNORM_SUMS || (a.sums_out && a.M > 1)) && !(rs128 || rs64)) return hipErrorInvalidValue;
     if (a.prologue == PRO_RMSNORM_SUMS && (ph2 || !a.sums_in || (a.K >> 4) > 64 * SUMS_PER_LANE || a.x_stride != a.K)) return hipErrorInvalidValue;
-    if (a.sums_out && (a.nseg != 1 || a.prologue != PRO_NONE)) return hipErrorInvalidValue;
+    if (a.sums_out && a.M > 1 && (a.nseg != 1 || a.prologue != PRO_NONE)) return hipErrorInvalidValue;
+    const bool auto_geom = plain && !a.force_waves && a.force_rpt <= 0 && !(a.flags & GEMV_FLAG_GS);
+    if (a.sums_out && a.M == 1 && (!auto_geom || a.nseg != 1 || (a.prologue != PRO_NONE && a.prologue != PRO_SILU_MUL) || a.x_stride != a.K ||
+                                   (a.prologue == PRO_SILU_MUL && nw != 16)))
+        return hipErrorInvalidValue;
+    if (a.prologue == PRO_RMSNORM_CHUNKS &&
+        (a.M != 1 || !auto_geom || nw != 8 || (a.K >> 3) > 512 || !a.sums_in || a.sums_out || a.x_stride != a.K)) return hipErrorInvalidValue;
     GemvKArgs k{};
-    k.x = a.x; k.x2 = a.prologue == PRO_RMSNORM_SUMS ? a.sums_in : a.x2; k.gamma = a.gamma;
+    k.x = a.x; k.x2 = (a.prologue == PRO_RMSNORM_SUMS || a.prologue == PRO_RMSNORM_CHUNKS) ? a.sums_in : a.x2; k.gamma = a.gamma;
     k.sums_out = (float*)a.sums_out; k.sums_stride = a.seg[0].n_rt;
     k.M = a.M; k.K = a.K; k.x_stride = a.x_stride; k.nseg = a.nseg;
     k.eps = a.eps; k.rpt = rpt;
@@ -134,6 +141,7 @@
         }
     }
     if (a.prologue == PRO_RMSNORM_SUMS) return launch_pro_sums_entry(k, nw, rs64 ? 64 : 128, wg, lds, st);
+    if (a.prologue == PRO_RMSNORM_CHUNKS) return launch_pro_chunks_entry(k, wg, lds, st);
     switch (a.prologue) {
         case PRO_NONE: return launch_pro<PRO_NONE>(k, a.flags | (rs128 ? GEMV_FLAG_RS128 : 0) | (rs64 ? GEMV_FLAG_RS64 : 0) | (ph2 ? GEMV_FLAG_PH2 : 0), a.force_depth, nw, wg, lds, st);
         case PRO_RMSNORM: return launch_pro<PRO_RMSNORM>(k, a.flags | (rs128 ? GEMV_FLAG_RS128 : 0) | (rs64 ? GEMV_FLAG_RS64 : 0) | (ph2 ? GEMV_FLAG_PH2 : 0), a.force_depth, nw, wg, lds, st);
diff --git a/amq_amd/csrc/amq_gemv_body.cuh b/amq_amd/csrc/amq_gemv_body.cuh
--- a/amq_amd/csrc/amq_gemv_body.cuh
+++ b/amq_amd/csrc/amq_gemv_body.cuh
@@ -75,6 +75,12 @@
         : inv(__builtin_bit_cast(float, (127 - __builtin_ctz((unsigned)K)) << 23)), pow2((K & (K - 1)) == 0), k((float)K) {}
     __device__ __forceinline__ float operator()(float tot) const { return pow2 ? tot * inv : tot / k; }
 };
+
+__device__ __forceinline__ float sumsq8(float ss, const h8& v) {
+#pragma unroll
+    for (int e = 0; e < 8; ++e) { float f = (float)v[e]; ss += f * f; }
+    return ss;
+}
 
 template <int PRO, int NW, bool LIN>
 __device__ __forceinline__ void stage_x(const GemvHot& a, _Float16* xl, float* xg, float* red, int xs) {
@@ -180,25 +186,40 @@
 
 constexpr int XC_MAX = 4;
 constexpr int SUMS_PER_LANE = 8;
-struct XRegs { union { h8 v[XC_MAX]; float f[4 * XC_MAX]; }; h8 w[XC_MAX]; };
+struct XRegs { union { h8 v[XC_MAX]; float f[4 * XC_MAX]; }; h8 w[XC_MAX]; float cs[SUMS_PER_LANE]; };
 template <int NW> struct XCfg { static constexpr int XC = NW == 16 ? 2 : 1; };
 
+template <int PRO, int MATH, int XCH> struct XOwn { static constexpr bool OK = PRO == PRO_NONE && MATH != MATH_LINEAR && XCH == 1; };
+template <int NW>
+__device__ __forceinline__ int x_chunk(bool own, int i) {
+    const int tid = (int)threadIdx.x;
+    return own ? 16 * ((tid >> 6) + NW * ((tid & 63) >> 4)) + (tid & 15) : tid + i * NW * 64;
+}
+
 template <int PRO, int NW, int XCH>
-__device__ __forceinline__ void x_issue(const GemvHot& a, XRegs& xr) {
-    constexpr int THREADS = NW * 64;
+__device__ __forceinline__ void x_issue(const GemvHot& a, XRegs& xr, bool own) {
     const int last = (a.K >> 3) - 1;
 #pragma unroll
     for (int i = 0; i < XCH; ++i) {
-        int c = (int)threadIdx.x + i * THREADS;
+        int c = x_chunk<NW>(own, i);
         c = c < last ? c : last;
         xr.v[i] = *(const h8*)((const _Float16*)a.x + 8 * c);
         if (PRO == PRO_SILU_MUL) xr.w[i] = *(const h8*)((const _Float16*)a.x2 + 8 * c);
-        if (PRO == PRO_RMSNORM) xr.w[i] = *(const h8*)((const _Float16*)a.gamma + 8 * c);
+        if (PRO == PRO_RMSNORM || PRO == PRO_RMSNORM_CHUNKS) xr.w[i] = *(const h8*)((const _Float16*)a.gamma + 8 * c);
+    }
+    if constexpr (PRO == PRO_RMSNORM_CHUNKS) {
+        static_assert(NW <= SUMS_PER_LANE && XCH == 1, "chunk sums: one chunk per thread, at most 8 waves");
+        const int lane = (int)threadIdx.x & 63;
+#pragma unroll
+        for (int v = 0; v < NW; ++v) {
+            const int idx = lane + 64 * v;
+            xr.cs[v] = ((const float*)a.x2)[idx < last ? idx : last];
+        }
     }
 }
 
 template <int PRO, int NW, int XCH, bool LIN>
-__device__ __forceinline__ void x_finish(const GemvHot& a, const XRegs& xr, _Float16* xl, float* xg, float* red) {
+__device__ __forceinline__ void x_finish(const GemvHot& a, const XRegs& xr, _Float16* xl, float* xg, float* red, bool own) {
     constexpr int THREADS = NW * 64;
     const int tid = threadIdx.x;
     const int chunks = a.K >> 3;
@@ -207,10 +228,7 @@
         float ss = 0.f;
 #pragma unroll
         for (int i = 0; i < XCH; ++i) {
-            if (tid + i * THREADS < chunks) {
-#pragma unroll
-                for (int e = 0; e < 8; ++e) { float f = (float)xr.v[i][e]; ss += f * f; }
-            }
+            if (tid + i * THREADS < chunks) ss = sumsq8(ss, xr.v[i]);
         }
         ss = wave_sum(ss);
         if ((tid & 63) == 0) red[tid >> 6] = ss;
@@ -219,10 +237,19 @@
 #pragma unroll
         for (int w = 0; w < NW; ++w) tot += red[w];
         rstd = rsqrtf(MeanDiv(a.K)(tot) + a.eps);
+    } else if (PRO == PRO_RMSNORM_CHUNKS) {
+        const int lane = tid & 63;
+        float tot = 0.f;
+#pragma unroll
+        for (int v = 0; v < NW; ++v) {
+            tot += wave_sum(lane + 64 * v < chunks ? xr.cs[v] : 0.f);
+            __builtin_amdgcn_sched_barrier(0);
+        }
+        rstd = rsqrtf(MeanDiv(a.K)(tot) + a.eps);
     }
 #pragma unroll
     for (int i = 0; i < XCH; ++i) {
-        const int c = tid + i * THREADS;
+        const int c = x_chunk<NW>(own, i);
         float cs = 0.f;
         if (c < chunks) {
             h8 r;
@@ -543,10 +570,12 @@
     so.residual = (const _Float16*)blk.residual[sidx];
     so.y = (_Float16*)blk.y[sidx];
     so.y_stride = blk.y_stride[sidx];
-    so.sums = (RS != 256 && PRO == PRO_NONE) ? blk.sums_out : nullptr;
+    constexpr bool CHUNK_SUMS = RS == 256 && (PRO == PRO_NONE || (PRO == PRO_SILU_MUL && NW == 16)) && (MATH == MATH_EXACT || MATH == MATH_GS) && GP == 1 && !SC1;
+    so.sums = ((RS != 256 && PRO == PRO_NONE) || CHUNK_SUMS) ? blk.sums_out : nullptr;
     so.sums_stride = blk.sums_stride;
 #ifndef AMQ_ABL_NOSTAGE
-    if (xmode == 1) x_finish<PRO, NW, XCH, MATH == MATH_LINEAR>(a, xr, lds_x, xg, red);
+    const bool own = XOwn<PRO, MATH, XCH>::OK && xmode == 1 && G % NW == 0;
+    if (xmode == 1) x_finish<PRO, NW, XCH, MATH == MATH_LINEAR>(a, xr, lds_x, xg, red, own);
     else if (RS != 256 && xmode == 2) {
 #ifdef AMQ_ABL_NOLOAD
         x_finish_dma<PRO, NW, XCH, 0, RowsCfg<RS>::MRMAX>(a, xr, lds_x, red, xs, 0, a.K / PH);
@@ -555,8 +584,10 @@
 #endif
     }
     else stage_x<PRO, NW, MATH == MATH_LINEAR>(a, lds_x, xg, red, xs);
-#endif
+    if (!own) __syncthreads();
+#else
     __syncthreads();
+#endif
     if (wave == 0) AMQ_STAMP_AT(blk, 2);
 
     _Float16 pf_bias = (_Float16)0.f, pf_res = (_Float16)0.f;
@@ -614,6 +645,17 @@
                 if (so.sums) {                                                                   \
                     const float q_ = row16_total((float)y_ * (float)y_);                         \
                     if (e_c == 0) so.sums[(size_t)e_m * so.sums_stride + rt_] = q_;              \
+                }                                                                                \
+            }                                                                                    \
+            if constexpr (CHUNK_SUMS) {                        \
+                if (so.sums) {                                                                   \
+                    const int yb_ = (int)__builtin_bit_cast(unsigned short, y_);                 \
+                    h8 lo_, hi_;                                                                 \
+                    _Pragma("unroll") for (int e_ = 0; e_ < 8; ++e_) {                           \
+                        lo_[e_] = __builtin_bit_cast(_Float16, (unsigned short)__builtin_amdgcn_readlane(yb_, e_));     \
+                        hi_[e_] = __builtin_bit_cast(_Float16, (unsigned short)__builtin_amdgcn_readlane(yb_, 8 + e_)); \
+                    }                                                                            \
+                    if (threadIdx.x < 2) so.sums[rt_ * 2 + threadIdx.x] = sumsq8(0.f, threadIdx.x ? hi_ : lo_);         \
                 }                                                                                \
             }                                                                                    \
         }                                                                                        \
@@ -806,7 +848,7 @@
 #define AMQ_LB_WAVES_R(NW_, GP_, MATH_, XCH_, RS_) (((RS_) == 64 && (NW_) == 8) ? AMQ_RS64_WAVES : ((RS_) == 128 && (NW_) == 8) ? 4 : (RS_) == 128 ? 1 : AMQ_LB_WAVES_M(NW_, GP_, MATH_, XCH_))
 #endif
 template <int PRO, int NW, int U, int MATH, int XCH, int RS = 256, int GP = 1, int PH = 1>
-__global__ __launch_bounds__(NW * 64, AMQ_LB_WAVES_R(NW, GP, MATH, XCH, RS)) void gemv_kernel(const void* p_x, const void* p_xw, const void* p_qw0,
+__global__ __launch_bounds__(NW * 64, PRO == PRO_RMSNORM_CHUNKS ? 6 : AMQ_LB_WAVES_R(NW, GP, MATH, XCH, RS)) void gemv_kernel(const void* p_x, const void* p_xw, const void* p_qw0,
                                                                      const void* p_mt0, int p_K, int p_m_nseg, int p_rpt,
                                                                      int p_n_rt0, int p_key0, float p_eps, GemvKArgs blk) {
     extern __shared__ __attribute__((aligned(16))) unsigned char smem[];
@@ -817,6 +859,10 @@
     a.x = p_x; a.x2 = p_xw; a.gamma = p_xw;
     if (PRO == PRO_RMSNORM_SUMS) a.x2 = blk.x2;
     a.K = p_K; a.M = p_m_nseg & 0xFF; a.rpt = p_rpt; a.eps = p_eps;
+    if (PRO == PRO_RMSNORM_CHUNKS) {
+        a.x2 = (const void*)(((unsigned long long)__builtin_bit_cast(unsigned, p_eps) << 32) | (unsigned)p_rpt);
+        a.eps = blk.eps;
+    }
     const int nseg = p_m_nseg >> 16;
     const bool dense = (p_m_nseg >> 8) & 1;
     const int Kst = a.K / PH;
@@ -825,6 +871,7 @@
     if (RS != 256 && MATH != MATH_LINEAR && fits && dense && a.M >= 2 && a.M <= RowsCfg<RS>::MRMAX) xmode = 2;
     if (PH > 1 && xmode != 2) return;
     if (PRO == PRO_RMSNORM_SUMS && xmode != 2) return;
+    if (PRO == PRO_RMSNORM_CHUNKS && xmode != 1) return;
     const bool slow_x = xmode == 0;
     a.x_stride = slow_x ? blk.x_stride : a.K;
     const int xs = Kst + XPAD;
@@ -835,7 +882,7 @@
     float* red = (float*)(smem + xbytes + xgbytes);
 
     XRegs xr;
-    if (xmode == 1) x_issue<PRO, NW, XCH>(a, xr);
+    if (xmode == 1) x_issue<PRO, NW, XCH>(a, xr, XOwn<PRO, MATH, XCH>::OK && (a.K >> 7) % NW == 0);
     else if (RS != 256 && xmode == 2) x_dma_rows<PRO, NW, XCH>(a, xl, xs, xr, 0, Kst);
 
     const int bid = (int)blockIdx.x;
@@ -900,8 +947,15 @@
         if (e != hipSuccess) return e;
     }
     const void* xw = PRO == PRO_SILU_MUL ? a.x2 : a.gamma;
+    int rpt = a.rpt;
+    float eps = a.eps;
+    if (PRO == PRO_RMSNORM_CHUNKS) {
+        const unsigned long long p = (unsigned long long)(size_t)a.x2;
+        rpt = (int)(unsigned)p;
+        eps = __builtin_bit_cast(float, (unsigned)(p >> 32));
+    }
     hipLaunchKernelGGL(kern, dim3(total_wg), dim3(NW * 64), lds, st, a.x, xw, a.qweight[0], a.meta[0], a.K,
-                       a.M | ((a.x_stride == a.K ? 1 : 0) << 8) | (a.nseg << 16), a.rpt, a.n_rt[0], a.key[0], a.eps, a);
+                       a.M | ((a.x_stride == a.K ? 1 : 0) << 8) | (a.nseg << 16), rpt, a.n_rt[0], a.key[0], eps, a);
     return hipGetLastError();
 }
 
diff --git a/amq_amd/csrc/amq_gemv_pro3.hip b/amq_amd/csrc/amq_gemv_pro3.hip
--- a/amq_amd/csrc/amq_gemv_pro3.hip
+++ b/amq_amd/csrc/amq_gemv_pro3.hip
@@ -8,4 +8,7 @@
     if (nw == 16) return launch_one<PRO_RMSNORM_SUMS, 16, 2, MATH_EXACT, XCfg<16>::XC, 128>(a, total_wg, lds, st);
     return launch_one<PRO_RMSNORM_SUMS, 8, 2, MATH_EXACT, XCfg<8>::XC, 128>(a, total_wg, lds, st);
 }
+hipError_t launch_pro_chunks_entry(const GemvKArgs& a, int total_wg, size_t lds, hipStream_t st) {
+    return launch_one<PRO_RMSNORM_CHUNKS, 8, 2, MATH_EXACT, 1>(a, total_wg, lds, st);
 }
+}
diff --git a/amq_amd/csrc/amq_gemv_qkvattn.hip b/amq_amd/csrc/amq_gemv_qkvattn.hip
--- a/amq_amd/csrc/amq_gemv_qkvattn.hip
+++ b/amq_amd/csrc/amq_gemv_qkvattn.hip
@@ -224,7 +224,7 @@
     }
     const int local = bid - wgb;
     XRegs xr;
-    x_issue<PRO, NW, XCH>(a, xr);
+    x_issue<PRO, NW, XCH>(a, xr, false);
     switch (key) {
         case 4 * 4 + MODE_HQQ: gemv_body<4, MODE_HQQ, PRO, NW, U, MATH, XCH, 256, true>(a, blk, sidx, qwp, mtp, nrt, local, xl, xl, xg, red, xs, 1, xr); break;
         case 3 * 4 + MODE_HQQ: gemv_body<3, MODE_HQQ, PRO, NW, U, MATH, XCH, 256, true>(a, blk, sidx, qwp, mtp, nrt, local, xl, xl, xg, red, xs, 1, xr); break;
diff --git a/amq_amd/csrc/amq_kernels.h b/amq_amd/csrc/amq_kernels.h
--- a/amq_amd/csrc/amq_kernels.h
+++ b/amq_amd/csrc/amq_kernels.h
@@ -30,7 +30,8 @@
 };
 
 enum { PRO_NONE = 0, PRO_RMSNORM = 1, PRO_SILU_MUL = 2,
-       PRO_RMSNORM_SUMS = 3  };
+       PRO_RMSNORM_SUMS = 3 ,
+       PRO_RMSNORM_CHUNKS = 4  };
 enum { FMT_HQQ = 0, FMT_GPTQ = 1, FMT_AWQ = 2 };
 constexpr int GEMV_MAX_SEG = 4;
 
diff --git a/amq_amd/llama.py b/amq_amd/llama.py
--- a/amq_amd/llama.py
+++ b/amq_amd/llama.py
@@ -73,6 +73,7 @@
     DOWN_FUSED_ROWS = 1
     NORM_FUSED_ROWS = 4
     NORM_SUMS = True
+    ROW_SUMS = True
     FUSE_QKV_ATTN = False
     ENGINE_DEFAULT = False
     all_logits = False
@@ -181,6 +182,9 @@
         self._norm_sums = (self.NORM_SUMS and 2 <= self.B <= 8 and not self.fine and 2048 <= self.H <= 8192 and self.I >= 2048
                            and self.B <= ops.gemv_max_rows(self.H, plain=True))
         self.ss = torch.zeros(self.B, self.H // 16, dtype=torch.float32, device=dev) if self._norm_sums else None
+        self._row_sums = (self.ROW_SUMS and self.B == 1 and not self.fine and 2048 <= self.H <= 4096 and self.I > 8192 and not self.fuse_qkv_attn
+                          and ops.default_gemv_math() == ops.MATH_EXACT and ops.DEFAULT_GEMV_OPTS is None)
+        self.cs = torch.zeros(self.H // 8, dtype=torch.float32, device=dev) if self._row_sums else None
         eligible = self.B == 1 and max_seq <= self.ENGINE_MAX_SEQ and self.H == self.nh * 128 and not self.fine and not self.has_bias
         if engine and not eligible:
             raise ValueError("the decode engine needs batch 1 and max_seq <= %d" % self.ENGINE_MAX_SEQ)
@@ -278,6 +282,8 @@
                 qkv = [blk["self_attn.q_proj"].seg(self.q), blk["self_attn.k_proj"].seg(self.k), blk["self_attn.v_proj"].seg(self.v)]
                 if self._norm_sums and have_sums:
                     ops.gemv_grouped_sums(self.x, qkv, H, gamma=blk["ln1"], eps=self.eps, sums_in=self.ss)
+                elif self._row_sums and have_sums:
+                    ops.gemv_row_sums(self.x, qkv, H, prologue=ops.PRO_RMSNORM, gamma=blk["ln1"], eps=self.eps, sums_in=self.cs)
                 elif self.B > self.NORM_FUSED_ROWS:
                     ops.gemv_grouped(ops.rmsnorm(self.x, blk["ln1"], self.eps, out=self.xn), qkv, H)
                 else:
@@ -288,16 +294,24 @@
                 ops.gemv_grouped_sums(self.att, [blk["self_attn.o_proj"].seg(self.x, residual=self.x)], H, sums_out=self.ss)
                 ops.gemv_grouped_sums(self.x, [blk["mlp.gate_proj"].seg(self.gate), blk["mlp.up_proj"].seg(self.up)], H,
                                       gamma=blk["ln2"], eps=self.eps, sums_in=self.ss)
+            elif self._row_sums:
+                ops.gemv_row_sums(self.att, [blk["self_attn.o_proj"].seg(self.x, residual=self.x)], H, sums_out=self.cs)
+                ops.gemv_row_sums(self.x, [blk["mlp.gate_proj"].seg(self.gate), blk["mlp.up_proj"].seg(self.up)], H,
+                                  prologue=ops.PRO_RMSNORM, gamma=blk["ln2"], eps=self.eps, sums_in=self.cs)
             else:
                 ops.gemv_grouped(self.att, [blk["self_attn.o_proj"].seg(self.x, residual=self.x)], H)
-            if self._norm_sums:
+            if self._norm_sums or self._row_sums:
                 pass
             elif self.B > self.NORM_FUSED_ROWS:
                 ops.gemv_grouped(ops.rmsnorm(self.x, blk["ln2"], self.eps, out=self.xn), [blk["mlp.gate_proj"].seg(self.gate), blk["mlp.up_proj"].seg(self.up)], H)
             else:
                 ops.gemv_grouped(self.x, [blk["mlp.gate_proj"].seg(self.gate), blk["mlp.up_proj"].seg(self.up)], H,
                                  prologue=ops.PRO_RMSNORM, gamma=blk["ln2"], eps=self.eps)
-            if self._down_rows_fit:
+            if self._down_rows_fit and self._row_sums:
+                ops.gemv_row_sums(self.gate, [blk["mlp.down_proj"].seg(self.x, residual=self.x)], self.I,
+                                  prologue=ops.PRO_SILU_MUL, x2=self.up, sums_out=self.cs)
+                have_sums = True
+            elif self._down_rows_fit:
                 ops.gemv_grouped(self.gate, [blk["mlp.down_proj"].seg(self.x, residual=self.x)], self.I,
                                  prologue=ops.PRO_SILU_MUL, x2=self.up)
             elif self._down_rows_phased and self._norm_sums:
diff --git a/amq_amd/ops.py b/amq_amd/ops.py
--- a/amq_amd/ops.py
+++ b/amq_amd/ops.py
@@ -507,6 +507,35 @@
                                                 ctypes.byref(opts) if opts is not None else None, _lib.current_stream()))
 
 
+def gemv_row_sums(x, segments, K, prologue=PRO_NONE, x2=None, gamma=None, eps=0.0, sums_in=None, sums_out=None):
+    xx = _prep_x(x, K)
+    if xx.shape[0] != 1:
+        raise ValueError("gemv_row_sums: one row")
+    if not 1 <= len(segments) <= _lib.MAX_SEGMENTS:
+        raise ValueError(f"1..{_lib.MAX_SEGMENTS} segments")
+    arr = (Segment * len(segments))()
+    for i, s in enumerate(segments):
+        _check_shape(s["bits"], s["N"], K)
+        _check_native(s["qn"], s["mn"], s["bits"], s["N"], K)
+        _need(s["y"], torch.float16, "y", s["N"])
+        if s.get("bias") is not None:
+            _need(s["bias"], torch.float16, "bias", s["N"])
+        if s.get("residual") is not None:
+            _need(s["residual"], torch.float16, "residual", s["N"])
+        arr[i] = Segment(_lib.ptr(s["qn"]), _lib.ptr(s["mn"]), _lib.ptr(s.get("bias")), _lib.ptr(s.get("residual")),
+                         _lib.ptr(s["y"]), s["N"], s["bits"], s["mode"], 0)
+    if prologue == PRO_RMSNORM:
+        _need(gamma, torch.float16, "gamma", K)
+        _need(sums_in, torch.float32, "sums_in", K // 8)
+    if prologue == PRO_SILU_MUL:
+        x2 = _prep_x(x2, K)
+    if sums_out is not None:
+        _need(sums_out, torch.float32, "sums_out", segments[0]["N"] // 8)
+    _lib.check(_lib.load().amq_gemv_row_sums_f16(arr, len(segments), _lib.ptr(xx), _lib.ptr(x2) if prologue == PRO_SILU_MUL else None,
+                                                 _lib.ptr(gamma) if prologue == PRO_RMSNORM else None, ctypes.c_float(eps), prologue,
+                                                 _lib.ptr(sums_in), _lib.ptr(sums_out), K, _lib.current_stream()))
+
+
 def gemv_grouped_sums(x, segments, K, gamma=None, eps=0.0, sums_in=None, sums_out=None):
     xx = _prep_x(x, K)
     M = xx.shape[0]
diff --git a/include/amq_hip.h b/include/amq_hip.h
--- a/include/amq_hip.h
+++ b/include/amq_hip.h
@@ -101,6 +101,8 @@
                          void* stream);
 int amq_gemv_grouped_sums_f16(const amq_segment* segs, int nseg, const void* x, const void* gamma, float eps, const float* sums_in,
                               float* sums_out, int M, int K, int group, void* stream);
+int amq_gemv_row_sums_f16(const amq_segment* segs, int nseg, const void* x, const void* x2, const void* gamma, float eps, int prologue,
+                          const float* sums_in, float* sums_out, int K, void* stream);
 
 
 size_t amq_compat_workspace_bytes(int bits, int M, int N, int K);
```

Result: slower. 727.6 tokens/s (median of 2 runs) (-3.8%).
